# askerlee/segtran

Measured on NVIDIA H100. Metric: voxels/sec fwd+bwd Segtran3d BraTS 112^3 bs=4 hot path, higher is better.
Workload: dtype tf32

## Files before the change

include/segtran_b200.h:

```cpp
#ifndef SEGTRAN_B200_H_
#define SEGTRAN_B200_H_

#include <stddef.h>
#include <stdint.h>

#ifdef __cplusplus
extern "C" {
#endif

#define SX_VERSION 1

enum { SX_F32 = 0, SX_BF16 = 1 };
enum { SX_OP_TF32 = 0, SX_OP_BF16 = 1 };
enum { SX_MAJOR_K = 0, SX_MAJOR_MN = 1 };
enum { SX_BIAS_NONE = 0, SX_BIAS_N = 1, SX_BIAS_M = 2 };
enum { SX_ACT_NONE = 0, SX_ACT_GELU = 1,
       SX_ACT_GELU_BWD = 2  };

int sx_version(void);
const char* sx_last_error(void);
int sx_device_info(int* sm_count, int* cc_major, int* cc_minor);

typedef struct {
  const void* ptr;
  int32_t major;
  int32_t _pad;
  int64_t ld;
  int64_t stride_z0;
  int64_t stride_z1;
} sx_operand;

typedef struct {
  int32_t op_dtype;
  int32_t M, N, K, Z0, Z1;
  sx_operand A, B;
  void* C;
  int32_t c_dtype;
  int32_t round_tf32;
  int64_t ldc, c_stride_z0, c_stride_z1;
  float alpha;
  int32_t bias_mode;
  const float* bias;
  int64_t bias_stride_z0, bias_stride_z1;
  int32_t act;
  int32_t accumulate;
  void* preact;
  int32_t split_k;
  int32_t _pad2;
  float* amax;
  float drop_p;
  uint32_t _pad3;
  uint64_t drop_seed;
  const uint64_t* drop_seed_dev;
  const float* addend;
  float* part;
  int64_t part_floats;
} sx_gemm_args;

typedef struct {
  float* ct;
  int64_t ldct, ct_stride_z0, ct_stride_z1;
} sx_gemm_tout;

int sx_gemm(const sx_gemm_args* args, const sx_gemm_tout* tout, void* stream);

typedef struct {
  const float* table;
  int32_t pd, R;
  int32_t grid[3];
  float w;
} sx_posbias;

typedef struct {
  int32_t B, M, U1, U2, d;
  int32_t round_tf32;
  const float* Q;
  int64_t q_ld, q_bstride;
  const float* K;
  int64_t k_ld, k_bstride;
  float alpha, clip;
  float* P;
  float* S;
  int64_t ldp;
  float* lse;
  float* rowmax;
  float* stat;
  float* diag;
  float drop_p;
  uint32_t _pad;
  uint64_t drop_seed;
  const uint64_t* drop_seed_dev;
  sx_posbias posbias;
} sx_attn_probs_args;
int sx_attn_probs_fwd(const sx_attn_probs_args* args, void* stream);

enum { SX_CONSIST_BCE = 0, SX_CONSIST_MARGIN = 1 };
typedef struct {
  int32_t B, N, A, K;
  int32_t variant;
  int32_t round_r;
  const float* Xo;
  int64_t xo_ld, xo_bstride;
  const float* Xt;
  int64_t xt_ld, xt_bstride;
  const float* X;
  int64_t x_ld, x_bstride;
  const float* F;
  const float* mu;
  float* R;
  int64_t ldr;
  float* out;
  float* cap;
  float cap_scale;
  int32_t _pad;
  float* part;
  int64_t part_floats;
} sx_consist_args;
int sx_attn_consist_fwd(const sx_consist_args* args, void* stream);
int sx_attn_consist_bwd(const sx_consist_args* args, const float* gout, const float* G, int32_t rows, int32_t cols,
                        int64_t ldg, int64_t g_bstride, const float* vrow, const float* vcol, float* dst, int64_t ldd,
                        int64_t d_bstride, void* stream);

int sx_clamp_if(const float* S, int64_t R, int32_t L, int64_t lds, const float* amax, float clip, const float* dY,
                int64_t ldy, float* out, int64_t ldo, void* stream);

int sx_seed_derive(const uint64_t* base, uint64_t add, uint64_t* out, void* stream);
int sx_seed_advance(uint64_t* base, uint64_t inc, void* stream);


int sx_reduce_max(const float* x, int64_t n, float* out, void* stream);

int sx_pos_lsinu_fwd(const float* pos, const float* posmax, int64_t R, int32_t pd, const float* W, const float* b,
                     int32_t C, float* pe, void* stream);
int sx_pos_lsinu_bwd(const float* pos, const float* posmax, int64_t R, int32_t pd, const float* W, const float* b,
                     int32_t C, const float* dpe, float* de_scratch, float* dW, float* db, float* part, int64_t part_floats, void* stream);

int sx_prologue_fwd(const float* x, int64_t B, int32_t N, int32_t C, const float* g, const float* b, const float* pe,
                    int32_t C0, int64_t pe_bstride, float posw, const float* mask, float drop_p, uint64_t seed, const uint64_t* seed_dev, float* h,
                    int32_t round_tf32, float* stats, void* stream);
int sx_prologue_bwd(const float* dh, const float* x, int64_t B, int32_t N, int32_t C, const float* g, const float* b,
                    const float* pe, int32_t C0, int64_t pe_bstride, float posw, const float* mask, float drop_p,
                    uint64_t seed, const uint64_t* seed_dev, const float* stats, float* dx, float* dg, float* db, float* dpe,
                    float* dt_scratch , float* part, int64_t part_floats, void* stream);

int sx_softmax_fwd(const float* S, int64_t R, int32_t L, int64_t lds, const float* amax, float clip, float drop_p,
                   uint64_t seed, const uint64_t* seed_dev, float* P, int64_t ldp, int32_t round_tf32, float* lse, float* diag,
                   void* stream);
int sx_softmax_bwd(const float* dP, int64_t ldd, const float* S, int64_t lds, const float* lse, int64_t R, int32_t L,
                   const float* amax, float clip, float drop_p, uint64_t seed, const uint64_t* seed_dev, int64_t ldp_fwd, float* dS,
                   int64_t ldo, int32_t round_tf32, void* stream);
int sx_softmax_posbias_fwd(const float* S, int64_t R, int32_t L, int64_t lds, const float* amax, float clip, float drop_p,
                           uint64_t seed, const uint64_t* seed_dev, float* P, int64_t ldp, int32_t round_tf32,
                           float* lse, float* diag, const sx_posbias* posbias, void* stream);
int sx_softmax_posbias_bwd(const float* dP, int64_t ldd, const float* S, int64_t lds, const float* lse, int64_t R, int32_t L,
                           const float* amax, float clip, float drop_p, uint64_t seed, const uint64_t* seed_dev, int64_t ldp_fwd,
                           float* dS, int64_t ldo, int32_t round_tf32, const sx_posbias* posbias,
                           float* dtable, float* part, int64_t part_floats, void* stream);

int sx_layernorm_fwd(const float* x, int64_t R, int32_t C, const float* g, const float* b, float* y,
                     int32_t round_tf32, float* stats, void* stream);
int sx_layernorm_bwd(const float* dy, const float* x, int64_t R, int32_t C, const float* g, const float* stats,
                     float* dx, int32_t round_tf32, float* dg, float* db, float* part, int64_t part_floats, void* stream);

int sx_ln_softaggr_fwd(const float* Y, int32_t B, int32_t M, int32_t N, int32_t F, const float* g, const float* b,
                       const float* ws, const float* bs, float drop_p, uint64_t seed, const uint64_t* seed_dev, float* out, float* stats,
                       float* wts, void* stream);
int sx_ln_softaggr_bwd(const float* dout, const float* Y, int32_t B, int32_t M, int32_t N, int32_t F, const float* g,
                       const float* b, const float* ws, float drop_p, uint64_t seed, const uint64_t* seed_dev, const float* stats,
                       const float* wts, float* dY, int32_t round_tf32, float* dg, float* db,
                       float* dws, float* dbs, float* part, int64_t part_floats, void* stream);

int sx_softaggr_fwd(const float* x, int32_t B, int32_t M, int32_t N, int32_t F, const float* ws, const float* bs, float* out,
                    float* wts, void* stream);
int sx_softaggr_bwd(const float* dout, const float* x, int32_t B, int32_t M, int32_t N, int32_t F, const float* ws,
                    const float* wts, float* dx, float* dscore, void* stream);
int sx_gelu_bwd(const float* dG, const float* H, int64_t n, float drop_p, uint64_t seed, const uint64_t* seed_dev, float* dH,
                int32_t round_tf32, void* stream);
int sx_convert(const void* x, int32_t x_dtype, int64_t n, void* y, int32_t y_dtype, int32_t round_tf32, void* stream);
int sx_split_tf32(const float* x, int64_t n, float* hi, float* lo, void* stream);
int sx_split_tf32_cat(const float* x, int32_t Z1, int32_t Z0, int32_t R, int32_t K, int64_t sz1, int64_t sz0, int64_t sr,
                      int64_t sk, int32_t Kp, int32_t role, float* out, void* stream);
int sx_dot(const float* x, const float* y, int64_t n, float* out, float* part, int64_t part_floats, void* stream);
int sx_scale(const float* x, int64_t n, const float* alpha_dev, float alpha, float* y, void* stream);
int sx_colsum_batched(const float* X, int32_t Z1, int64_t stride_z1, int32_t Z0, int64_t stride_z0, int64_t R, int32_t C,
                      int64_t ld, float* out, float* part, int64_t part_floats, void* stream);
int sx_add(const float* a, const float* b, int64_t n, float* y, void* stream);
int sx_rowsum(const float* X, int64_t R, int64_t C, int64_t ld, int32_t out_mod, float* out, float* part, int64_t part_floats, void* stream);
int sx_transpose(const float* in, int64_t Z, int32_t R, int32_t C, int32_t ldo, float* out, void* stream);

int sx_head_contract_fwd(const float* curr, const float* W, const float* bias, int32_t B, int32_t Cf, int64_t V,
                         int32_t K, float* L, int32_t accumulate, void* stream);
int sx_head_contract_bwd_data(const float* dL, const float* W, int32_t B, int32_t Cf, int64_t V, int32_t K,
                              float* dcurr, void* stream);
int sx_head_contract_bwd_weight(const float* dL, const float* curr, int32_t B, int32_t Cf, int64_t V, int32_t K,
                                float* dW, float* part, int64_t part_floats, void* stream);
int sx_token_scores(const float* vf, const float* W, int32_t B, int32_t N, int32_t F, int32_t K, float* out,
                    void* stream);
int sx_token_scores_bwd(const float* dt, const float* W, int32_t B, int32_t N, int32_t F, int32_t K, float* dvf,
                        void* stream);
int sx_subpixel_resize_fwd(const float* S, const float* bias, int32_t B, int32_t K, int32_t D2, int32_t H2, int32_t W2,
                           int32_t H, int32_t W, int32_t D, float* out, void* stream);
int sx_subpixel_resize_bwd(const float* dout, int32_t B, int32_t K, int32_t D2, int32_t H2, int32_t W2, int32_t H,
                           int32_t W, int32_t D, float* dS, void* stream);
enum { SX_HEAD_DMAP_NONE = 0, SX_HEAD_DMAP_INTERP = 1, SX_HEAD_DMAP_UNFOLD = 2, SX_HEAD_DMAP_UNFOLD_INTERLEAVED = 3 };
enum { SX_HEAD_SRC_DEPTH_MAJOR = 0, SX_HEAD_SRC_SLICE_MAJOR = 1 };
typedef struct {
  const float* src;
  int32_t B, Fs, Ds;
  int32_t Fo;
  int64_t HW;
  int32_t Dk;
  int32_t dmap;
  int32_t K;
  int32_t src_layout;
  const float* Wc;
  const float* bc;
  float p;
  uint32_t _pad2;
  uint64_t seed;
  const uint64_t* seed_dev;
  float* part;
  int64_t part_floats;
} sx_head_dropout_args;
int sx_head_dropout_fwd(const sx_head_dropout_args* args, float* Ls, void* stream);
int sx_head_dropout_bwd(const sx_head_dropout_args* args, const float* dLs, float* dsrc, int32_t accumulate, float* dWc,
                        void* stream);
int sx_groupnorm_fwd(const float* x, int32_t B, int32_t C, int64_t V, int32_t G, const float* gamma, const float* beta,
                     float eps, double* csum, float* stats, float* y, int32_t round_tf32, void* stream);
int sx_groupnorm_bwd(const float* dy, const float* x, int32_t B, int32_t C, int64_t V, int32_t G, const float* gamma,
                     const float* stats, double* csum, float* coef, float* dx, float* dgamma, float* dbeta, void* stream);
int sx_groupnorm_slices_fwd(const float* x, int32_t B, int32_t D, int32_t C, int64_t V, int32_t G, const float* gamma,
                            const float* beta, float eps, double* csum, float* stats, float* y, int32_t round_tf32,
                            void* stream);
int sx_groupnorm_slices_bwd(const float* dy, const float* x, int32_t B, int32_t D, int32_t C, int64_t V, int32_t G,
                            const float* gamma, const float* stats, double* csum, float* coef, float* dx, float* dgamma,
                            float* dbeta, void* stream);

int sx_seg_loss_fwd(const float* logits, const float* mask, int32_t B, int32_t K, int64_t V, const float* pos_weight,
                    const float* class_w, float dice_w, double* sums, float* out3, float* coef, void* stream);
int sx_seg_loss_bwd(const float* logits, const float* mask, int32_t B, int32_t K, int64_t V, const float* pos_weight,
                    const float* coef, float ce_scale, const float* gout, float* dlogits, void* stream);
enum { SX_SCHED_WARMUP_LINEAR = 0, SX_SCHED_WARMUP_CONSTANT = 1 };
int sx_adam_step(float* p, float* p_tf32, const float* g, float* m, float* v, const int32_t* seg_param, const int64_t* seg_off,
                 const int32_t* seg_len, int32_t nseg, int32_t P, const float* lr, const float* wd, double b1, double b2,
                 double eps, float grad_clip, float max_grad_norm, float warmup, int64_t t_total, int32_t schedule,
                 int64_t* step, double* sumsq, float* coef, float* lr_eff, float* total_norm, void* stream);

int sx_resize_axis_fwd(const float* x, int64_t outer, int32_t Lin, int32_t Lout, int64_t inner, float* y,
                       int32_t accumulate, void* stream);
int sx_resize_axis_bwd(const float* dy, int64_t outer, int32_t Lin, int32_t Lout, int64_t inner, float* dx,
                       void* stream);
typedef struct {
  int32_t lin[3];
  int32_t lout[3];
  float ratio[3];
} sx_resample_grid;
int sx_resize_tokens_fwd(const float* x, int64_t bs_in, int64_t gs_in, int64_t ld_in, float* y, int64_t bs_out,
                         int64_t gs_out, int64_t ld_out, int32_t B, int32_t G, int32_t w, int32_t w_pad,
                         const sx_resample_grid* grid, int32_t round_tf32, void* stream);
int sx_resize_tokens_bwd(const float* dy, int64_t bs_out, int64_t gs_out, int64_t ld_out, float* dx, int64_t bs_in,
                         int64_t gs_in, int64_t ld_in, int32_t B, int32_t G, int32_t w, int32_t w_pad,
                         const sx_resample_grid* grid, int32_t accumulate, void* stream);
int sx_sgemm_small(const float* A, const float* B, float* C, int32_t M, int32_t N, int32_t K, int64_t sam, int64_t sak,
                   int64_t sbk, int64_t sbn, int64_t scm, int64_t scn, int32_t Z, int64_t saz, int64_t sbz, int64_t scz,
                   float alpha, int32_t accumulate, void* stream);

typedef struct {
  const float* wx;
  const float* wy;
  const float* wz;
  int32_t nx, ny, nz, _pad;
} sx_sw_weights;
int sx_sw_accumulate(const float* scores, int32_t K, int32_t dx, int32_t dy, int32_t dz, float* preds, float* cnt,
                     int32_t H, int32_t W, int32_t D, int32_t x0, int32_t y0, int32_t z0, int32_t mirror,
                     const sx_sw_weights* weights, void* stream);
int sx_sw_finalize(float* preds, const float* cnt, int32_t K, int64_t V, int32_t brats, float* hard, void* stream);
int sx_sw_gather(const float* img, int32_t B, int32_t C, int32_t H, int32_t W, int32_t D, const int32_t* origins, int32_t n,
                 int32_t dx, int32_t dy, int32_t dz, int32_t mirror, float* out, void* stream);

int sx_sw2d_accumulate(const float* scores, int32_t B, int32_t K, int32_t h, int32_t w, int32_t dx, int32_t dy, float* preds,
                       float* cnt, int32_t H2, int32_t W2, int32_t xs, int32_t ys, int32_t mirror,
                       const sx_sw_weights* weights, void* stream);
int sx_sw2d_finalize(const float* preds, const float* cnt, int32_t B, int32_t K, int32_t H2, int32_t W2, int32_t hl,
                     int32_t wl, int32_t H, int32_t W, float* soft, int32_t* hard, void* stream);
int sx_eval2d_counts(const float* pred, int32_t B, int32_t K, int32_t h, int32_t w, const float* gt, int32_t Hg, int32_t Wg,
                     int32_t* counts, void* stream);

int sx_mask_counts(const uint8_t* A, const uint8_t* B, int32_t K, int64_t V, int64_t* counts, int64_t ldc, void* stream);
int sx_surface(const uint8_t* X, int32_t K, int32_t ndim, int32_t n0, int32_t n1, int32_t n2, uint8_t* border, void* stream);
int sx_edt_sq(const uint8_t* border, int32_t K, int32_t n0, int32_t n1, int32_t n2, int32_t* dist, void* stream);
int sx_surface_hist(const uint8_t* src_border, const int32_t* dist, int32_t K, int64_t V, int32_t nbins, uint32_t* hist,
                    int64_t ldh, void* stream);
int sx_surface_stats(const uint32_t* hist, int32_t K, int32_t nbins, int64_t ldh, double* out, int64_t ldo, void* stream);

enum { SX_LABEL_U8 = 0, SX_LABEL_I16 = 1, SX_LABEL_I32 = 2, SX_LABEL_I64 = 3, SX_LABEL_F32 = 4 };
typedef struct {
  const float* x;
  int64_t stride[5];
  float* y;
  int32_t C;
  int32_t _pad;
} sx_crop_operand;
int sx_brats_map_label(const void* label, int32_t dtype, int32_t B, int64_t V, int32_t binarize, float* out, void* stream);
int sx_draw_resized_crop(const uint64_t* seed_dev, uint64_t seed, int32_t H, int32_t W, int32_t D, int32_t oh, int32_t ow,
                         int32_t od, float min_scale, float max_scale, int32_t isotropic, float* rec, void* stream);
int sx_resized_crop(const sx_crop_operand* a, const sx_crop_operand* b, int32_t B, int32_t H, int32_t W, int32_t D,
                    int32_t oh, int32_t ow, int32_t od, const float* rec, void* stream);

int sx_gemm_debug_set(const char* key, int64_t value);

#ifdef __cplusplus
}
#endif
#endif
```

segtran_b200/_lib.py:

```python
from __future__ import annotations

import ctypes as C
import os

_HERE = os.path.dirname(os.path.abspath(__file__))
LIB_PATH = os.path.join(_HERE, "libsegtran_b200.so")

SX_F32, SX_BF16 = 0, 1
SX_OP_TF32, SX_OP_BF16 = 0, 1
SX_MAJOR_K, SX_MAJOR_MN = 0, 1
SX_BIAS_NONE, SX_BIAS_N, SX_BIAS_M = 0, 1, 2
SX_ACT_NONE, SX_ACT_GELU, SX_ACT_GELU_BWD = 0, 1, 2
SX_SCHED_WARMUP_LINEAR, SX_SCHED_WARMUP_CONSTANT = 0, 1
SX_CONSIST_BCE, SX_CONSIST_MARGIN = 0, 1
SX_HEAD_DMAP_NONE, SX_HEAD_DMAP_INTERP, SX_HEAD_DMAP_UNFOLD, SX_HEAD_DMAP_UNFOLD_INTERLEAVED = 0, 1, 2, 3
SX_HEAD_SRC_DEPTH_MAJOR, SX_HEAD_SRC_SLICE_MAJOR = 0, 1
SX_LABEL_U8, SX_LABEL_I16, SX_LABEL_I32, SX_LABEL_I64, SX_LABEL_F32 = 0, 1, 2, 3, 4


class SxError(RuntimeError):
    pass


class sx_operand(C.Structure):
    _fields_ = [("ptr", C.c_void_p), ("major", C.c_int32), ("_pad", C.c_int32), ("ld", C.c_int64),
                ("stride_z0", C.c_int64), ("stride_z1", C.c_int64)]


class sx_gemm_args(C.Structure):
    _fields_ = [("op_dtype", C.c_int32), ("M", C.c_int32), ("N", C.c_int32), ("K", C.c_int32), ("Z0", C.c_int32),
                ("Z1", C.c_int32), ("A", sx_operand), ("B", sx_operand), ("C", C.c_void_p), ("c_dtype", C.c_int32),
                ("round_tf32", C.c_int32), ("ldc", C.c_int64), ("c_stride_z0", C.c_int64), ("c_stride_z1", C.c_int64),
                ("alpha", C.c_float), ("bias_mode", C.c_int32), ("bias", C.c_void_p), ("bias_stride_z0", C.c_int64),
                ("bias_stride_z1", C.c_int64), ("act", C.c_int32), ("accumulate", C.c_int32), ("preact", C.c_void_p),
                ("split_k", C.c_int32), ("_pad2", C.c_int32), ("amax", C.c_void_p), ("drop_p", C.c_float),
                ("_pad3", C.c_uint32), ("drop_seed", C.c_uint64), ("drop_seed_dev", C.c_void_p), ("addend", C.c_void_p),
                ("part", C.c_void_p), ("part_floats", C.c_int64)]


class sx_gemm_tout(C.Structure):
    _fields_ = [("ct", C.c_void_p), ("ldct", C.c_int64), ("ct_stride_z0", C.c_int64), ("ct_stride_z1", C.c_int64)]


class sx_sw_weights(C.Structure):
    _fields_ = [("wx", C.c_void_p), ("wy", C.c_void_p), ("wz", C.c_void_p), ("nx", C.c_int32), ("ny", C.c_int32),
                ("nz", C.c_int32), ("_pad", C.c_int32)]


class sx_posbias(C.Structure):
    _fields_ = [("table", C.c_void_p), ("pd", C.c_int32), ("R", C.c_int32), ("grid", C.c_int32 * 3), ("w", C.c_float)]


class sx_attn_probs_args(C.Structure):
    _fields_ = [("B", C.c_int32), ("M", C.c_int32), ("U1", C.c_int32), ("U2", C.c_int32), ("d", C.c_int32),
                ("round_tf32", C.c_int32), ("Q", C.c_void_p), ("q_ld", C.c_int64), ("q_bstride", C.c_int64),
                ("K", C.c_void_p), ("k_ld", C.c_int64), ("k_bstride", C.c_int64), ("alpha", C.c_float),
                ("clip", C.c_float), ("P", C.c_void_p), ("S", C.c_void_p), ("ldp", C.c_int64), ("lse", C.c_void_p),
                ("rowmax", C.c_void_p), ("stat", C.c_void_p), ("diag", C.c_void_p), ("drop_p", C.c_float),
                ("_pad", C.c_uint32), ("drop_seed", C.c_uint64), ("drop_seed_dev", C.c_void_p), ("posbias", sx_posbias)]


class sx_consist_args(C.Structure):
    _fields_ = [("B", C.c_int32), ("N", C.c_int32), ("A", C.c_int32), ("K", C.c_int32), ("variant", C.c_int32),
                ("round_r", C.c_int32), ("Xo", C.c_void_p), ("xo_ld", C.c_int64), ("xo_bstride", C.c_int64),
                ("Xt", C.c_void_p), ("xt_ld", C.c_int64), ("xt_bstride", C.c_int64), ("X", C.c_void_p),
                ("x_ld", C.c_int64), ("x_bstride", C.c_int64), ("F", C.c_void_p), ("mu", C.c_void_p), ("R", C.c_void_p),
                ("ldr", C.c_int64), ("out", C.c_void_p), ("cap", C.c_void_p), ("cap_scale", C.c_float),
                ("_pad", C.c_int32), ("part", C.c_void_p), ("part_floats", C.c_int64)]


class sx_head_dropout_args(C.Structure):
    _fields_ = [("src", C.c_void_p), ("B", C.c_int32), ("Fs", C.c_int32), ("Ds", C.c_int32), ("Fo", C.c_int32),
                ("HW", C.c_int64), ("Dk", C.c_int32), ("dmap", C.c_int32), ("K", C.c_int32), ("src_layout", C.c_int32),
                ("Wc", C.c_void_p), ("bc", C.c_void_p), ("p", C.c_float), ("_pad2", C.c_uint32), ("seed", C.c_uint64),
                ("seed_dev", C.c_void_p), ("part", C.c_void_p), ("part_floats", C.c_int64)]


class sx_resample_grid(C.Structure):
    _fields_ = [("lin", C.c_int32 * 3), ("lout", C.c_int32 * 3), ("ratio", C.c_float * 3)]


class sx_crop_operand(C.Structure):
    _fields_ = [("x", C.c_void_p), ("stride", C.c_int64 * 5), ("y", C.c_void_p), ("C", C.c_int32), ("_pad", C.c_int32)]


_P, _I, _L, _F, _U64, _D = C.c_void_p, C.c_int32, C.c_int64, C.c_float, C.c_uint64, C.c_double

_PROTOS = {
    "sx_gemm": [C.POINTER(sx_gemm_args), C.POINTER(sx_gemm_tout), _P],
    "sx_gemm_debug_set": [C.c_char_p, _L],
    "sx_attn_probs_fwd": [C.POINTER(sx_attn_probs_args), _P],
    "sx_attn_consist_fwd": [C.POINTER(sx_consist_args), _P],
    "sx_attn_consist_bwd": [C.POINTER(sx_consist_args), _P, _P, _I, _I, _L, _L, _P, _P, _P, _L, _L, _P],
    "sx_clamp_if": [_P, _L, _I, _L, _P, _F, _P, _L, _P, _L, _P],
    "sx_reduce_max": [_P, _L, _P, _P],
    "sx_pos_lsinu_fwd": [_P, _P, _L, _I, _P, _P, _I, _P, _P],
    "sx_pos_lsinu_bwd": [_P, _P, _L, _I, _P, _P, _I, _P, _P, _P, _P, _P, _L, _P],
    "sx_prologue_fwd": [_P, _L, _I, _I, _P, _P, _P, _I, _L, _F, _P, _F, _U64, _P, _P, _I, _P, _P],
    "sx_prologue_bwd": [_P, _P, _L, _I, _I, _P, _P, _P, _I, _L, _F, _P, _F, _U64, _P, _P, _P, _P, _P, _P, _P, _P, _L, _P],
    "sx_softmax_fwd": [_P, _L, _I, _L, _P, _F, _F, _U64, _P, _P, _L, _I, _P, _P, _P],
    "sx_softmax_bwd": [_P, _L, _P, _L, _P, _L, _I, _P, _F, _F, _U64, _P, _L, _P, _L, _I, _P],
    "sx_softmax_posbias_fwd": [_P, _L, _I, _L, _P, _F, _F, _U64, _P, _P, _L, _I, _P, _P, C.POINTER(sx_posbias), _P],
    "sx_softmax_posbias_bwd": [_P, _L, _P, _L, _P, _L, _I, _P, _F, _F, _U64, _P, _L, _P, _L, _I, C.POINTER(sx_posbias),
                               _P, _P, _L, _P],
    "sx_layernorm_fwd": [_P, _L, _I, _P, _P, _P, _I, _P, _P],
    "sx_layernorm_bwd": [_P, _P, _L, _I, _P, _P, _P, _I, _P, _P, _P, _L, _P],
    "sx_ln_softaggr_fwd": [_P, _I, _I, _I, _I, _P, _P, _P, _P, _F, _U64, _P, _P, _P, _P, _P],
    "sx_ln_softaggr_bwd": [_P, _P, _I, _I, _I, _I, _P, _P, _P, _F, _U64, _P, _P, _P, _P, _I, _P, _P, _P, _P, _P, _L, _P],
    "sx_softaggr_fwd": [_P, _I, _I, _I, _I, _P, _P, _P, _P, _P],
    "sx_softaggr_bwd": [_P, _P, _I, _I, _I, _I, _P, _P, _P, _P, _P],
    "sx_gelu_bwd": [_P, _P, _L, _F, _U64, _P, _P, _I, _P],
    "sx_seed_derive": [_P, _U64, _P, _P],
    "sx_seed_advance": [_P, _U64, _P],
    "sx_convert": [_P, _I, _L, _P, _I, _I, _P],
    "sx_sw_accumulate": [_P, _I, _I, _I, _I, _P, _P, _I, _I, _I, _I, _I, _I, _I, C.POINTER(sx_sw_weights), _P],
    "sx_sw_finalize": [_P, _P, _I, _L, _I, _P, _P],
    "sx_sw_gather": [_P, _I, _I, _I, _I, _I, _P, _I, _I, _I, _I, _I, _P, _P],
    "sx_sw2d_accumulate": [_P, _I, _I, _I, _I, _I, _I, _P, _P, _I, _I, _I, _I, _I, C.POINTER(sx_sw_weights), _P],
    "sx_sw2d_finalize": [_P, _P, _I, _I, _I, _I, _I, _I, _I, _I, _P, _P, _P],
    "sx_eval2d_counts": [_P, _I, _I, _I, _I, _P, _I, _I, _P, _P],
    "sx_mask_counts": [_P, _P, _I, _L, _P, _L, _P],
    "sx_surface": [_P, _I, _I, _I, _I, _I, _P, _P],
    "sx_edt_sq": [_P, _I, _I, _I, _I, _P, _P],
    "sx_surface_hist": [_P, _P, _I, _L, _I, _P, _L, _P],
    "sx_surface_stats": [_P, _I, _I, _L, _P, _L, _P],
    "sx_brats_map_label": [_P, _I, _I, _L, _I, _P, _P],
    "sx_draw_resized_crop": [_P, _U64, _I, _I, _I, _I, _I, _I, _F, _F, _I, _P, _P],
    "sx_resized_crop": [C.POINTER(sx_crop_operand), C.POINTER(sx_crop_operand), _I, _I, _I, _I, _I, _I, _I, _P, _P],
    "sx_split_tf32": [_P, _L, _P, _P, _P],
    "sx_split_tf32_cat": [_P, _I, _I, _I, _I, _L, _L, _L, _L, _I, _I, _P, _P],
    "sx_transpose": [_P, _L, _I, _I, _I, _P, _P],
    "sx_colsum_batched": [_P, _I, _L, _I, _L, _L, _I, _L, _P, _P, _L, _P],
    "sx_dot": [_P, _P, _L, _P, _P, _L, _P],
    "sx_add": [_P, _P, _L, _P, _P],
    "sx_rowsum": [_P, _L, _L, _L, _I, _P, _P, _L, _P],
    "sx_scale": [_P, _L, _P, _F, _P, _P],
    "sx_head_contract_fwd": [_P, _P, _P, _I, _I, _L, _I, _P, _I, _P],
    "sx_head_contract_bwd_data": [_P, _P, _I, _I, _L, _I, _P, _P],
    "sx_head_contract_bwd_weight": [_P, _P, _I, _I, _L, _I, _P, _P, _L, _P],
    "sx_head_dropout_fwd": [C.POINTER(sx_head_dropout_args), _P, _P],
    "sx_head_dropout_bwd": [C.POINTER(sx_head_dropout_args), _P, _P, _I, _P, _P],
    "sx_token_scores": [_P, _P, _I, _I, _I, _I, _P, _P],
    "sx_token_scores_bwd": [_P, _P, _I, _I, _I, _I, _P, _P],
    "sx_subpixel_resize_fwd": [_P, _P, _I, _I, _I, _I, _I, _I, _I, _I, _P, _P],
    "sx_subpixel_resize_bwd": [_P, _I, _I, _I, _I, _I, _I, _I, _I, _P, _P],
    "sx_resize_axis_fwd": [_P, _L, _I, _I, _L, _P, _I, _P],
    "sx_resize_axis_bwd": [_P, _L, _I, _I, _L, _P, _P],
    "sx_resize_tokens_fwd": [_P, _L, _L, _L, _P, _L, _L, _L, _I, _I, _I, _I, C.POINTER(sx_resample_grid), _I, _P],
    "sx_resize_tokens_bwd": [_P, _L, _L, _L, _P, _L, _L, _L, _I, _I, _I, _I, C.POINTER(sx_resample_grid), _I, _P],
    "sx_groupnorm_fwd": [_P, _I, _I, _L, _I, _P, _P, _F, _P, _P, _P, _I, _P],
    "sx_groupnorm_bwd": [_P, _P, _I, _I, _L, _I, _P, _P, _P, _P, _P, _P, _P, _P],
    "sx_groupnorm_slices_fwd": [_P, _I, _I, _I, _L, _I, _P, _P, _F, _P, _P, _P, _I, _P],
    "sx_groupnorm_slices_bwd": [_P, _P, _I, _I, _I, _L, _I, _P, _P, _P, _P, _P, _P, _P, _P],
    "sx_seg_loss_fwd": [_P, _P, _I, _I, _L, _P, _P, _F, _P, _P, _P, _P],
    "sx_seg_loss_bwd": [_P, _P, _I, _I, _L, _P, _P, _F, _P, _P, _P],
    "sx_adam_step": [_P, _P, _P, _P, _P, _P, _P, _P, _I, _I, _P, _P, _D, _D, _D, _F, _F, _F, _L, _I, _P, _P, _P, _P, _P, _P],
    "sx_sgemm_small": [_P, _P, _P, _I, _I, _I, _L, _L, _L, _L, _L, _L, _I, _L, _L, _L, _F, _I, _P],
}
EXPORTS = sorted(list(_PROTOS) + ["sx_version", "sx_last_error", "sx_device_info"])

_lib = None


def lib():
    global _lib
    if _lib is None:
        if not os.path.isfile(LIB_PATH):
            raise SxError("segtran_b200: %s is missing - run `python -c 'import __graft_entry__ as g; g.build()'` "
                          "or `make` at the repo root (there is no CPU / PyTorch fallback)" % LIB_PATH)
        l = C.CDLL(LIB_PATH)
        l.sx_version.restype = C.c_int
        l.sx_last_error.restype = C.c_char_p
        l.sx_device_info.argtypes = [C.POINTER(C.c_int)] * 3
        l.sx_device_info.restype = C.c_int
        for name, at in _PROTOS.items():
            f = getattr(l, name)
            f.argtypes = at
            f.restype = C.c_int
        _lib = l
    return _lib


def check(rc, what):
    if rc != 0:
        raise SxError("%s failed (rc=%d): %s" % (what, rc, lib().sx_last_error().decode("utf-8", "replace")))


_LAUNCHES = {"sx_pos_lsinu_bwd": 3, "sx_ln_softaggr_bwd": 2, "sx_prologue_bwd": 3, "sx_layernorm_bwd": 3, "sx_gemm_debug_set": 0,
             "sx_attn_probs_fwd": 2, "sx_colsum_batched": 2, "sx_dot": 2, "sx_head_contract_bwd_weight": 2,
             "sx_softmax_posbias_bwd": 2, "sx_attn_consist_fwd": 2, "sx_head_dropout_bwd": 2, "sx_edt_sq": 3}
launch_count = 0
_hook = None


def set_hook(h):
    global _hook
    _hook = h


def call(name, *args):
    global launch_count
    launch_count += _LAUNCHES.get(name, 1)
    if _hook is None:
        check(getattr(lib(), name)(*args), name)
    else:
        with _hook(name, args):
            check(getattr(lib(), name)(*args), name)
```

segtran_b200/csrc/sx_attn.cu:

```cuda
#include "sx_common.cuh"
#include "sx_posbias.cuh"
#include "sx_tc.cuh"

namespace {
using namespace sxtc;

constexpr int NUM_THREADS = 384;
constexpr int STAGES = 4;
constexpr int STAGE_BYTES = A_STAGE_BYTES + B_STAGE_BYTES;
constexpr int SMEM_BYTES = STAGES * STAGE_BYTES + 1024  + 256;
constexpr float LOG2E = 1.4426950408889634f, LN2 = 0.6931471805599453f;

__device__ __forceinline__ unsigned int ordered_key(float v) {
  const unsigned int b = __float_as_uint(v);
  return (b & 0x80000000u) ? ~b : (b | 0x80000000u);
}
__device__ __forceinline__ float ordered_val(unsigned int k) {
  return k == 0u ? -3.0e38f : __uint_as_float((k & 0x80000000u) ? (k & 0x7FFFFFFFu) : ~k);
}

struct AttnParams {
  int B, M, U1, U2, d;
  int tiles_m, tiles_n, num_kb, items, nsub;
  int q_bcast;
  float alpha2, clip2;
  float alpha, clip;
  float* P;
  float* S;
  float* lse;
  float* rowmax;
  float* stat;
  long long ldp;
  float drop_p;
  unsigned long long drop_seed;
  const unsigned long long* drop_seed_dev;
  int round_tf32;
  const float* pb_table;
  sxpb::Geom pb;
};

constexpr int PB_OFFSET = STAGES * STAGE_BYTES + 256;
constexpr int PB_MAX_FLOATS = 29 * 29 * 29;

template <bool HAS_BIAS>
__global__ void __launch_bounds__(NUM_THREADS, 1)
sx_attn_probs_kernel(const __grid_constant__ CUtensorMap tmQ, const __grid_constant__ CUtensorMap tmK, const AttnParams p) {
  extern __shared__ uint8_t smem_raw[];
  uint8_t* smem = reinterpret_cast<uint8_t*>((reinterpret_cast<uintptr_t>(smem_raw) + 1023) & ~uintptr_t(1023));
  uint64_t* bars = reinterpret_cast<uint64_t*>(smem + STAGES * STAGE_BYTES);
  uint64_t* full_bar = bars;
  uint64_t* empty_bar = bars + STAGES;

  const int warp = threadIdx.x >> 5;
  const int lane = threadIdx.x & 31;
  const int wg = threadIdx.x >> 7;

  if (threadIdx.x == 0) {
    sx::tma_prefetch_desc(&tmQ);
    sx::tma_prefetch_desc(&tmK);
    for (int s = 0; s < STAGES; ++s) {
      sx::mbar_init(&full_bar[s], 1);
      sx::mbar_init(&empty_bar[s], 2);
    }
    sx::fence_barrier_init();
  }
  float* ptab = nullptr;
  float* pred = nullptr;
  if constexpr (HAS_BIAS) {
    ptab = reinterpret_cast<float*>(smem + PB_OFFSET);
    pred = reinterpret_cast<float*>(smem + STAGES * STAGE_BYTES + 128);
    float bmn = 0.f, bmx = 0.f;
    for (int i = threadIdx.x; i < p.pb.T; i += NUM_THREADS) {
      const float v = p.pb.w * p.pb_table[i];
      ptab[i] = v * LOG2E;
      bmn = fminf(bmn, v);
      bmx = fmaxf(bmx, v);
    }
    bmx = sx::warp_max(bmx);
    bmn = -sx::warp_max(-bmn);
    if ((threadIdx.x & 31) == 0) { pred[2 * (threadIdx.x >> 5)] = bmn; pred[2 * (threadIdx.x >> 5) + 1] = bmx; }
  }
  __syncthreads();

  auto decode = [&](int it, int& b, int& m, int& mb) {
    mb = it % p.tiles_m; it /= p.tiles_m;
    m = it % p.M;
    b = it / p.M;
  };

  if (wg == 0) {
    asm volatile("setmaxnreg.dec.sync.aligned.u32 40;" ::: "memory");
    if (warp == 0 && sx::elect_one()) {
      int stage = 0;
      uint32_t phase = 0;
      for (int it = blockIdx.x; it < p.items; it += gridDim.x) {
        int b, m, mb;
        decode(it, b, m, mb);
        const int qb = p.q_bcast ? 0 : b;
        for (int sub = 0; sub < p.nsub; ++sub) {
          const int nb = sub % p.tiles_n;
          for (int kb = 0; kb < p.num_kb; ++kb) {
            sx::mbar_wait(&empty_bar[stage], phase ^ 1);
            sx::mbar_expect_tx(&full_bar[stage], STAGE_BYTES);
            uint8_t* sa = smem + stage * STAGE_BYTES;
            sx::tma_load_4d(sa, &tmQ, &full_bar[stage], kb * 32, mb * BM, m, qb, sx::kEvictLast);
            sx::tma_load_4d(sa + A_STAGE_BYTES, &tmK, &full_bar[stage], kb * 32, nb * BN, m, b, sx::kEvictLast);
            if (++stage == STAGES) { stage = 0; phase ^= 1; }
          }
        }
      }
    }
    return;
  }

  asm volatile("setmaxnreg.inc.sync.aligned.u32 232;" ::: "memory");
  const int cw = wg - 1;
  const int wtid = threadIdx.x & 127;
  const int wq = warp & 3;
  const int tr = lane >> 2;
  const int tc = (lane & 3) * 2;
  int stage = 0;
  uint32_t phase = 0;
  float gmax = -3.0e38f;
  int lowrows = 0;
  const uint32_t p16 = sx::drop_p16(p.drop_p);
  const float keep_scale = p.drop_p > 0.f ? 1.f / (1.f - p.drop_p) : 1.f;
  const unsigned long long dseed = p.drop_seed + (p.drop_seed_dev ? *p.drop_seed_dev : 0ull);
  const uint32_t dmul = sx::drop_mul((tc >> 1) & 1), dkey = sx::drop_key(dseed, (tc >> 1) & 1);
  float acc[64];
  float brange = 0.f;
  if constexpr (HAS_BIAS) {
    float bmn = 0.f, bmx = 0.f;
    for (int w = 0; w < NUM_THREADS / 32; ++w) { bmn = fminf(bmn, pred[2 * w]); bmx = fmaxf(bmx, pred[2 * w + 1]); }
    brange = bmx - bmn;
  }

  for (int it = blockIdx.x; it < p.items; it += gridDim.x) {
    int b, m, mb;
    decode(it, b, m, mb);
    int grow[2];
    long long rowflat[2];
    float rm[2], rl[2], rraw[2], rcp[2];
#pragma unroll
    for (int h = 0; h < 2; ++h) {
      grow[h] = mb * BM + cw * 64 + wq * 16 + 8 * h + tr;
      rowflat[h] = ((long long)b * p.M + m) * p.U1 + grow[h];
      rm[h] = -3.0e38f; rl[h] = 0.f; rraw[h] = -3.0e38f; rcp[h] = 0.f;
    }

    auto chunk_stats = [&](int nb) {
      if constexpr (HAS_BIAS) {
        int qc[2][3], kc[3];
        sxpb::coords(p.pb, grow[0], qc[0]);
        sxpb::coords(p.pb, grow[1], qc[1]);
        sxpb::coords(p.pb, nb * BN + tc, kc);
        float cm[2] = {-3.0e38f, -3.0e38f}, mb[2] = {-3.0e38f, -3.0e38f}, s[2] = {0.f, 0.f};
#pragma unroll
        for (int j = 0; j < 16; ++j)
#pragma unroll
          for (int e = 0; e < 2; ++e) {
            if (nb * BN + 8 * j + tc + e < p.U2) {
#pragma unroll
              for (int h = 0; h < 2; ++h) {
                const int o = sxpb::offset(p.pb, qc[h], kc);
                const float v = acc[4 * j + 2 * h + e];
                cm[h] = fmaxf(cm[h], v);
                const float x = fminf(v * p.alpha2, p.clip2) + (o >= 0 ? ptab[o] : 0.f);
                const float mn = fmaxf(mb[h], x);
                s[h] = s[h] * sx::ex2_approx(mb[h] - mn) + sx::ex2_approx(x - mn);
                mb[h] = mn;
              }
            }
            sxpb::step(p.pb, kc, e ? 7 : 1);
          }
#pragma unroll
        for (int h = 0; h < 2; ++h) {
#pragma unroll
          for (int o = 1; o <= 2; o <<= 1) {
            cm[h] = fmaxf(cm[h], __shfl_xor_sync(0xffffffffu, cm[h], o));
            const float mo = __shfl_xor_sync(0xffffffffu, mb[h], o), so = __shfl_xor_sync(0xffffffffu, s[h], o);
            const float mn = fmaxf(mb[h], mo);
            s[h] = s[h] * sx::ex2_approx(mb[h] - mn) + so * sx::ex2_approx(mo - mn);
            mb[h] = mn;
          }
          rraw[h] = fmaxf(rraw[h], cm[h] * p.alpha2);
          const float mn = fmaxf(rm[h], mb[h]);
          rl[h] = rl[h] * sx::ex2_approx(rm[h] - mn) + s[h] * sx::ex2_approx(mb[h] - mn);
          rm[h] = mn;
        }
      } else {
#pragma unroll
        for (int h = 0; h < 2; ++h) {
          float cm = -3.0e38f;
#pragma unroll
          for (int j = 0; j < 16; ++j)
#pragma unroll
            for (int e = 0; e < 2; ++e)
              if (nb * BN + 8 * j + tc + e < p.U2) cm = fmaxf(cm, acc[4 * j + 2 * h + e]);
          cm = fmaxf(cm, __shfl_xor_sync(0xffffffffu, cm, 1));
          cm = fmaxf(cm, __shfl_xor_sync(0xffffffffu, cm, 2));
          cm *= p.alpha2;
          rraw[h] = fmaxf(rraw[h], cm);
          const float mn = fmaxf(rm[h], fminf(cm, p.clip2));
          float s = 0.f;
#pragma unroll
          for (int j = 0; j < 16; ++j)
#pragma unroll
            for (int e = 0; e < 2; ++e)
              if (nb * BN + 8 * j + tc + e < p.U2) s += sx::ex2_approx(fminf(acc[4 * j + 2 * h + e] * p.alpha2, p.clip2) - mn);
          s += __shfl_xor_sync(0xffffffffu, s, 1);
          s += __shfl_xor_sync(0xffffffffu, s, 2);
          rl[h] = rl[h] * sx::ex2_approx(rm[h] - mn) + s;
          rm[h] = mn;
        }
      }
    };
    auto publish = [&]() {
#pragma unroll
      for (int h = 0; h < 2; ++h) {
        rcp[h] = 1.f / rl[h];
        if (grow[h] < p.U1) {
          gmax = fmaxf(gmax, rraw[h]);
          if ((lane & 3) == 0) {
            p.lse[rowflat[h]] = (rm[h] + __log2f(rl[h])) * LN2;
            if (p.rowmax) p.rowmax[rowflat[h]] = rraw[h] * LN2;
            if constexpr (HAS_BIAS) {
              if (rraw[h] * LN2 < -(p.clip - 104.f) + brange) ++lowrows;
            } else {
              if (rraw[h] * LN2 < -(p.clip - 104.f)) ++lowrows;
            }
          }
        }
      }
    };
    auto chunk_probs = [&](int nb) {
#pragma unroll
      for (int h = 0; h < 2; ++h) {
        if (grow[h] >= p.U1) continue;
        const long long roff = rowflat[h] * p.ldp;
        int qc[3], kc[3];
        if constexpr (HAS_BIAS) {
          sxpb::coords(p.pb, grow[h], qc);
          sxpb::coords(p.pb, nb * BN + tc, kc);
        }
#pragma unroll
        for (int j = 0; j < 16; ++j) {
          float b0 = 0.f, b1 = 0.f;
          if constexpr (HAS_BIAS) {
            int o = sxpb::offset(p.pb, qc, kc);
            if (o >= 0) b0 = ptab[o];
            sxpb::step(p.pb, kc, 1);
            o = sxpb::offset(p.pb, qc, kc);
            if (o >= 0) b1 = ptab[o];
            sxpb::step(p.pb, kc, 7);
          }
          const int col = nb * BN + 8 * j + tc;
          if (col >= p.U2) continue;
          const float v0 = acc[4 * j + 2 * h], v1 = acc[4 * j + 2 * h + 1];
          if (p.S) {
            if (col + 1 < p.U2) *reinterpret_cast<float2*>(p.S + roff + col) = make_float2(v0 * p.alpha, v1 * p.alpha);
            else p.S[roff + col] = v0 * p.alpha;
          }
          float f0, f1;
          if constexpr (HAS_BIAS) {
            f0 = sx::ex2_approx(fminf(v0 * p.alpha2, p.clip2) + b0 - rm[h]) * rcp[h];
            f1 = sx::ex2_approx(fminf(v1 * p.alpha2, p.clip2) + b1 - rm[h]) * rcp[h];
          } else {
            f0 = sx::ex2_approx(fminf(v0 * p.alpha2, p.clip2) - rm[h]) * rcp[h];
            f1 = sx::ex2_approx(fminf(v1 * p.alpha2, p.clip2) - rm[h]) * rcp[h];
          }
          if (p.drop_p > 0.f) {
            const uint32_t w = sx::drop_word_k(dmul, dkey, (unsigned long long)((roff + col) >> 2));
            f0 = (w & 0xFFFFu) >= p16 ? f0 * keep_scale : 0.f;
            f1 = (w >> 16) >= p16 ? f1 * keep_scale : 0.f;
          }
          if (p.round_tf32) {
            f0 = sx::round_tf32(f0);
            f1 = sx::round_tf32(f1);
          }
          if (col + 1 < p.U2) *reinterpret_cast<float2*>(p.P + roff + col) = make_float2(f0, f1);
          else p.P[roff + col] = f0;
        }
      }
    };

    for (int sub = 0; sub < p.nsub; ++sub) {
      const int nb = sub % p.tiles_n;
      for (int kb = 0; kb < p.num_kb; ++kb) {
        sx::mbar_wait(&full_bar[stage], phase);
        const uint32_t sa = sx::smem_u32(smem + stage * STAGE_BYTES);
        const uint32_t qa = sa + (uint32_t)(cw * 64 * BKB), ka = sa + A_STAGE_BYTES;
        sx::acc_fence(acc);
        sx::wgmma_fence();
#pragma unroll
        for (int kk = 0; kk < 4; ++kk)
          sx::wgmma_tf32(acc, sx::gmma_desc(qa + kk * 32, 16, 1024), sx::gmma_desc(ka + kk * 32, 16, 1024),
                         (kb > 0 || kk > 0) ? 1u : 0u);
        sx::wgmma_commit();
        sx::wgmma_wait<0>();
        sx::acc_fence(acc);
        if (wtid == 0) sx::mbar_arrive(&empty_bar[stage]);
        if (++stage == STAGES) { stage = 0; phase ^= 1; }
      }
      if (p.nsub == 1) {
        chunk_stats(nb);
        publish();
        chunk_probs(nb);
      } else if (sub < p.tiles_n) {
        chunk_stats(nb);
        if (sub == p.tiles_n - 1) publish();
      } else {
        chunk_probs(nb);
      }
    }
  }
  gmax = sx::warp_max(gmax);
  if (lane == 0 && gmax > -3.0e38f) atomicMax(reinterpret_cast<unsigned int*>(&p.stat[0]), ordered_key(gmax * LN2));
  int lr = lowrows;
#pragma unroll
  for (int o = 16; o > 0; o >>= 1) lr += __shfl_xor_sync(0xffffffffu, lr, o);
  if (lane == 0 && lr > 0) atomicAdd(&p.stat[1], (float)lr);
}

__global__ void attn_diag_kernel(float* stat, float clip, float* diag) {
  const float mx = ordered_val(__float_as_uint(stat[0]));
  stat[2] = mx;
  if (diag) {
    diag[0] = fmaxf(diag[0], mx);
    if (mx > clip) {
      diag[1] += 1.f;
      diag[2] += stat[1];
    }
  }
}

}

extern "C" int sx_attn_probs_fwd(const sx_attn_probs_args* a, void* stream) {
  SX_REQUIRE(a != nullptr, "sx_attn_probs_fwd: null args");
  SX_REQUIRE(a->B > 0 && a->M > 0 && a->U1 > 0 && a->U2 > 0 && a->d > 0, "sx_attn_probs_fwd: bad shape");
  SX_REQUIRE(a->Q && a->K && a->P && a->lse && a->stat, "sx_attn_probs_fwd: null pointer");
  SX_REQUIRE(a->d % 4 == 0 && a->ldp % 4 == 0 && a->ldp >= a->U2, "sx_attn_probs_fwd: d and ldp must be multiples of 4");
  SX_REQUIRE((reinterpret_cast<uintptr_t>(a->P) & 15) == 0 && (!a->S || (reinterpret_cast<uintptr_t>(a->S) & 15) == 0),
             "sx_attn_probs_fwd: outputs must be 16-byte aligned");
  const int sms = sm_count_cached();
  SX_REQUIRE(sms > 0, "sx_attn_probs_fwd: no CUDA device (this library has no CPU fallback)");

  AttnParams p{};
  p.B = a->B; p.M = a->M; p.U1 = a->U1; p.U2 = a->U2; p.d = a->d;
  p.tiles_m = sx_ceil_div(a->U1, BM);
  p.tiles_n = sx_ceil_div(a->U2, BN);
  p.num_kb = sx_ceil_div(a->d, 32);
  p.nsub = p.tiles_n == 1 ? 1 : 2 * p.tiles_n;
  const long long items = (long long)a->B * a->M * p.tiles_m;
  SX_REQUIRE(items < (1ll << 30), "sx_attn_probs_fwd: too many row blocks");
  p.items = (int)items;
  p.q_bcast = a->q_bstride == 0 && a->B > 1;
  p.alpha = a->alpha; p.clip = a->clip;
  p.alpha2 = a->alpha * LOG2E; p.clip2 = a->clip * LOG2E;
  p.P = reinterpret_cast<float*>(a->P); p.S = reinterpret_cast<float*>(a->S);
  p.lse = a->lse; p.rowmax = a->rowmax; p.stat = a->stat;
  p.ldp = a->ldp;
  p.drop_p = a->drop_p; p.drop_seed = a->drop_seed;
  p.drop_seed_dev = reinterpret_cast<const unsigned long long*>(a->drop_seed_dev);
  p.round_tf32 = a->round_tf32;
  const bool has_bias = a->posbias.table != nullptr;
  if (has_bias) {
    SX_REQUIRE(a->U1 == a->U2, "sx_attn_probs_fwd: positional biases need self-attention (U1 == U2)");
    const char* err = sxpb::check(&a->posbias, a->U1);
    SX_REQUIRE(err == nullptr, "sx_attn_probs_fwd: %s", err);
    p.pb_table = a->posbias.table;
    p.pb = sxpb::make_geom(a->posbias);
    SX_REQUIRE(p.pb.T <= PB_MAX_FLOATS, "sx_attn_probs_fwd: positional-bias table too large");
  }

  sx_operand oq{}, ok{};
  oq.ptr = a->Q; oq.major = SX_MAJOR_K; oq.ld = a->q_ld; oq.stride_z0 = a->d; oq.stride_z1 = p.q_bcast ? 0 : a->q_bstride;
  ok.ptr = a->K; ok.major = SX_MAJOR_K; ok.ld = a->k_ld; ok.stride_z0 = a->d; ok.stride_z1 = a->k_bstride;
  if (a->M == 1) { oq.stride_z0 = 0; ok.stride_z0 = 0; }
  if (a->B == 1) { oq.stride_z1 = 0; ok.stride_z1 = 0; }
  CUtensorMap tq, tk;
  int rc = make_map(&tq, oq, 4, a->U1, a->d, a->M, a->B, BM, "Q");
  if (rc) return rc;
  rc = make_map(&tk, ok, 4, a->U2, a->d, a->M, a->B, BN, "K");
  if (rc) return rc;

  const int grid = p.items < sms ? p.items : sms;
  cudaStream_t st = reinterpret_cast<cudaStream_t>(stream);
  if (has_bias) {
    constexpr int smem_pb = PB_OFFSET + PB_MAX_FLOATS * 4 + 1024;
    SX_CHECK_CUDA(set_max_smem_once(sx_attn_probs_kernel<true>, smem_pb));
    sx_attn_probs_kernel<true><<<grid, NUM_THREADS, PB_OFFSET + p.pb.T * 4 + 1024, st>>>(tq, tk, p);
  } else {
    SX_CHECK_CUDA(set_max_smem_once(sx_attn_probs_kernel<false>, SMEM_BYTES));
    sx_attn_probs_kernel<false><<<grid, NUM_THREADS, SMEM_BYTES, st>>>(tq, tk, p);
  }
  SX_CHECK_CUDA(cudaGetLastError());
  attn_diag_kernel<<<1, 1, 0, st>>>(a->stat, a->clip, a->diag);
  SX_CHECK_CUDA(cudaGetLastError());
  return 0;
}
```

segtran_b200/networks/segtran_shared.py:

```python
from __future__ import annotations

import copy
import math

import numpy as np
import torch
import torch.nn as nn
import torch.nn.functional as F

from .. import ops

bb2feat_dims = {
    'resnet34': [64, 64, 128, 256, 512], 'resnet50': [64, 256, 512, 1024, 2048],
    'resnet101': [64, 256, 512, 1024, 2048], 'resibn101': [64, 256, 512, 1024, 2048],
    'eff-b0': [16, 24, 40, 112, 1280], 'eff-b1': [16, 24, 40, 112, 1280], 'eff-b2': [16, 24, 48, 120, 1408],
    'eff-b3': [24, 32, 48, 136, 1536], 'eff-b4': [24, 32, 56, 160, 1792], 'effv2m': [24, 48, 80, 176, 512],
    'i3d': [64, 192, 480, 832, 1024],
}


def gen_all_indices(shape, device):
    axes = [torch.arange(int(s), device=device) for s in shape]
    return torch.stack(torch.meshgrid(*axes, indexing='ij'), dim=len(axes))


def multi_resize_shape(shape, scales):
    return [torch.Size([int(g / scale) for g in shape]) for scale in scales]


def mince_grids(shape, scales):
    grid = tuple(int(g) for g in shape)
    if len(grid) not in (2, 3):
        raise ValueError("mince transformer: a 2-D or 3-D token grid is needed (got %s)" % (grid,))
    out = []
    for scale, shp in zip(scales, multi_resize_shape(grid, scales)):
        for g, n in zip(grid, shp):
            if n < 1:
                raise ValueError("mince transformer: scale %s leaves an empty axis of the grid %s" % (scale, grid))
            if n != math.floor(g * (1.0 / scale)):
                raise ValueError("mince transformer: scale %s gives int(%d / %s) = %d cells but F.interpolate makes %d"
                                 % (scale, g, scale, n, math.floor(g * (1.0 / scale))))
        out.append(tuple(int(n) for n in shp))
    return out


def fracs_to_indices(feat_dim, mince_channel_props):
    fracs = np.array(mince_channel_props, dtype=float)
    fracs /= fracs.sum()
    n = len(fracs)
    idx = [0] * (n + 1)
    for i in range(n - 1):
        idx[i + 1] = idx[i] + int(fracs[i] * feat_dim)
    idx[-1] = feat_dim
    return idx, [idx[i + 1] - idx[i] for i in range(n)]


def _check_mince_config(config):
    if config.mince_scales is None or config.mince_channel_props is None:
        raise ValueError("mince transformer: mince_scales and mince_channel_props must be given")
    if len(config.mince_channel_props) != len(config.mince_scales):
        raise ValueError("mince transformer: %d scales but %d channel proportions"
                         % (len(config.mince_scales), len(config.mince_channel_props)))




class SegtranConfig:

    def __init__(self):
        self.feat_dim = -1
        self.in_feat_dim = -1
        self.num_modes = 4
        self.use_squeezed_transformer = True
        self.num_attractors = 256
        self.tie_qk_scheme = 'shared'
        self.mid_type = 'shared'
        self.trans_output_type = 'private'
        self.act_fun = F.gelu
        self.has_FFN = True
        self.has_FFN_in_squeeze = False
        self.pos_code_type = 'lsinu'
        self.pos_code_weight = 1.
        self.pos_bias_radius = 7
        self.qk_have_bias = True
        self.v_has_bias = False
        self.attn_clip = 500
        self.base_initializer_range = 0.02
        self.query_idbias_scale = 10
        self.feattrans_lin1_idbias_scale = 10
        self.pool_modes_feat = 'softmax'
        self.use_mince_transformer = False
        self.mince_scales = None
        self.mince_channel_props = None
        self.hidden_dropout_prob = 0.1
        self.attention_probs_dropout_prob = 0.1
        self.out_fpn_do_dropout = False
        self.eval_robustness = False
        self.ablate_multihead = False
        self.use_attn_consist_loss = False

    def try_assign(self, args, *keys):
        hit = False
        for key in keys:
            if key in args:
                self.__dict__[key] = args[key] if isinstance(args, dict) else args.__dict__[key]
                hit = True
        return hit

    def set_fpn_layers(self, config_name, fpn_settings, do_print=True):
        self.in_fpn_layers = [int(c) for c in fpn_settings.in_fpn_layers]
        self.out_fpn_layers = [int(c) for c in fpn_settings.out_fpn_layers]
        if self.out_fpn_layers[-1] > self.in_fpn_layers[-1]:
            print("in_fpn_layers=%s is not compatible with out_fpn_layers=%s" % (self.in_fpn_layers, self.out_fpn_layers))
            exit(0)
        ratios = fpn_settings.translayer_compress_ratios
        assert len(ratios) == self.num_translayers + 1, \
            "Length of {} != 1 + num_translayers {}".format(ratios, self.num_translayers)
        self.orig_in_feat_dim = self.bb_feat_dims[self.in_fpn_layers[-1]]
        self.translayer_compress_ratios = ratios
        self.translayer_dims = [int(self.orig_in_feat_dim / r) for r in np.cumprod(ratios)]
        self.trans_in_dim = self.translayer_dims[0]
        self.min_feat_dim = np.min(self.translayer_dims)
        self.trans_out_dim = self.translayer_dims[-1]
        self.in_fpn_scheme = fpn_settings.in_fpn_scheme
        self.out_fpn_scheme = fpn_settings.out_fpn_scheme
        if do_print:
            print("'%s' orig in-feat: %d, in-feat: %d, out-feat: %d, in-scheme: %s, out-scheme: %s, translayer_dims: %s"
                  % (config_name, self.orig_in_feat_dim, self.trans_in_dim, self.trans_out_dim, self.in_fpn_scheme,
                     self.out_fpn_scheme, self.translayer_dims))


def _prod(shape):
    n = 1
    for g in shape:
        n *= int(g)
    return n


def _unsupported(what):
    raise NotImplementedError("segtran_b200: %s is an ablation path this build does not implement "
                              "(use the reference module for it)" % what)


class MMSharedMid(nn.Module):

    def __init__(self, config):
        super().__init__()
        self.num_modes, self.feat_dim = config.num_modes, config.feat_dim
        self.shared_linear = nn.Linear(self.feat_dim, self.feat_dim)
        self.mid_act_fn = config.act_fun
        self.dropout = nn.Dropout(config.hidden_dropout_prob)

    def forward(self, x):
        p = self.dropout.p if self.training else 0.0
        return ops.linear(x, self.shared_linear.weight, self.shared_linear.bias, gelu=True, drop_p=p,
                          seed=ops.new_dropout_seed(x.device) if p > 0 else 0)


class MMPrivateMid(nn.Module):
    def __init__(self, config):
        super().__init__()
        _unsupported("mid_type='private'")


class MMPrivateOutput(nn.Module):

    def __init__(self, config):
        super().__init__()
        self.num_modes, self.feat_dim = config.num_modes, config.feat_dim
        fam = self.feat_dim * self.num_modes
        self.group_linear = nn.Conv1d(fam, fam, 1, groups=self.num_modes)
        self.resout_norm_layer = nn.LayerNorm(self.feat_dim, eps=1e-12, elementwise_affine=True)
        self.dropout = nn.Dropout(config.hidden_dropout_prob)

    def forward(self, x, shortcut=None):
        return ops.group_linear(x, self.group_linear.weight, self.group_linear.bias)


class MMSharedOutput(nn.Module):

    def __init__(self, config):
        super().__init__()
        self.num_modes, self.feat_dim = config.num_modes, config.feat_dim
        self.shared_linear = nn.Linear(self.feat_dim, self.feat_dim)
        self.resout_norm_layer = nn.LayerNorm(self.feat_dim, eps=1e-12, elementwise_affine=True)
        self.dropout = nn.Dropout(config.hidden_dropout_prob)

    def forward(self, x, shortcut):
        return ops.add(ops.linear(x, self.shared_linear.weight, self.shared_linear.bias), shortcut)


class LearnedSoftAggregate(nn.Module):

    def __init__(self, num_feat, group_dim, keepdim=False):
        super().__init__()
        self.group_dim = group_dim
        self.feat2score = nn.Linear(num_feat, 1)
        self.keepdim = keepdim

    def forward(self, x, score_basis=None):
        if score_basis is not None or self.group_dim != 1 or x.dim() != 4:
            _unsupported("LearnedSoftAggregate with a separate score basis / group_dim != 1")
        y = ops.soft_aggregate(x, self.feat2score.weight, self.feat2score.bias)
        return y.unsqueeze(1) if self.keepdim else y


class ExpandedFeatTrans(nn.Module):

    def __init__(self, config, name):
        super().__init__()
        self.config, self.name = config, name
        self.in_feat_dim, self.feat_dim, self.num_modes = config.in_feat_dim, config.feat_dim, config.num_modes
        self.feat_dim_allmode = self.feat_dim * self.num_modes
        self.has_FFN = config.has_FFN and not config.eval_robustness
        self.has_input_skip = getattr(config, 'has_input_skip', False)
        if self.has_input_skip:
            _unsupported("has_input_skip")
        if config.use_mince_transformer and config.mince_scales is not None:
            _check_mince_config(config)
            self.mince_scales = list(config.mince_scales)
            self.num_scales = len(self.mince_scales)
            self.mince_channel_props = config.mince_channel_props
            self.mince_channel_indices, _ = fracs_to_indices(self.feat_dim, self.mince_channel_props)
        else:
            self.num_scales = 0
            self.mince_scales = None
        self.first_linear = nn.Linear(self.in_feat_dim, self.feat_dim_allmode, bias=config.v_has_bias)
        self.first_norm_layer = nn.LayerNorm(self.feat_dim, eps=1e-12, elementwise_affine=True)
        self.base_initializer_range = config.base_initializer_range
        self.pool_modes_keepdim = False
        self.pool_modes_feat = config.pool_modes_feat
        if self.pool_modes_feat != 'softmax':
            _unsupported("pool_modes_feat=%r" % self.pool_modes_feat)
        self.feat_softaggr = LearnedSoftAggregate(self.feat_dim, group_dim=1, keepdim=False)
        self.mid_type = config.mid_type
        if self.mid_type == 'shared':
            self.intermediate = MMSharedMid(config)
        elif self.mid_type == 'private':
            self.intermediate = MMPrivateMid(config)
        else:
            _unsupported("mid_type=%r" % self.mid_type)
        if config.trans_output_type == 'shared':
            self.output = MMSharedOutput(config)
        elif config.trans_output_type == 'private':
            self.output = MMPrivateOutput(config)

    def add_identity_bias(self):
        s = self.config.feattrans_lin1_idbias_scale
        if s > 0:
            Fd = self.feat_dim
            eye = torch.eye(Fd) * self.base_initializer_range * s
            w = self.first_linear.weight.data
            w[:Fd, :Fd] = w[:Fd, :Fd] * 0.5 + eye.to(w)

    def _can_fold(self):
        return self.has_FFN and isinstance(self.output, MMPrivateOutput) and isinstance(self.intermediate, MMSharedMid) \
            and self.first_linear.bias is None and self.first_linear.weight.shape[1] % 4 == 0 and self.feat_dim % 4 == 0

    def supports_fused_attention(self):
        return self.has_FFN and isinstance(self.output, MMPrivateOutput) and isinstance(self.intermediate, MMSharedMid)

    def _value_bank(self, input_feat, tag="big"):
        M, mid = self.num_modes, self.intermediate
        B, U2 = input_feat.shape[0], input_feat.shape[1]
        if self._can_fold():
            return ops.folded_value_bank(input_feat, self.first_linear.weight, mid.shared_linear.weight, M, tag)
        v = ops.linear(input_feat, self.first_linear.weight, self.first_linear.bias, tag=tag)
        return ops.linear(v.view(B, U2, M, self.feat_dim), mid.shared_linear.weight, tag=tag).view(B, U2, M * self.feat_dim)

    def _norm_aggregate(self, y):
        p = self.output.dropout.p if self.training else 0.0
        ln = self.output.resout_norm_layer
        f2s = self.feat_softaggr.feat2score
        return ops.ln_softaggr(y, ln.weight, ln.bias, f2s.weight, f2s.bias, drop_p=p,
                               seed=ops.new_dropout_seed(y.device) if p > 0 else 0)

    def _mince_fuse(self, input_feat, probs, grid):
        M, Fd = self.num_modes, self.feat_dim
        grids = mince_grids(grid, self.mince_scales)
        if len(probs) != self.num_scales:
            raise ValueError("ExpandedFeatTrans: %d attention probabilities for %d mince scales" % (len(probs), self.num_scales))
        idx = self.mince_channel_indices
        wins = [(idx[s], idx[s + 1]) for s in range(self.num_scales)]
        if any(b <= a for a, b in wins):
            raise ValueError("ExpandedFeatTrans: an empty mince channel window %s of %d channels" % (wins, Fd))
        v = ops.linear(input_feat, self.first_linear.weight, self.first_linear.bias, round_out=False)
        ratios = [(ops.down_ratio(sc),) * len(grid) for sc in self.mince_scales]
        vs = ops.resize_tokens(v, M, grid, grids, ratios, wins)
        us = [ops.attn_pv(p, vv, M, round_out=False) for p, vv in zip(probs, vs)]
        return ops.resize_tokens_into(us, grid, grids, wins, Fd)

    def forward(self, input_feat, attention_probs, in_geoshape=None):
        M = self.num_modes
        if self.num_scales > 0:
            if in_geoshape is None:
                raise ValueError("ExpandedFeatTrans: the mince transformer needs the token grid (in_geoshape)")
            u = self._mince_fuse(input_feat, attention_probs, tuple(int(g) for g in in_geoshape))
            if not self.has_FFN:
                z = u[:, 0] if M == 1 else self.feat_softaggr(u)
                return ops.layer_norm(z, self.first_norm_layer.weight, self.first_norm_layer.bias)
            g = self.intermediate(u)
            return self._norm_aggregate(self.output(g, u))
        folded = self.supports_fused_attention()
        if not folded:
            v = ops.linear(input_feat, self.first_linear.weight, self.first_linear.bias)
        if not self.has_FFN:
            u = ops.attn_pv(attention_probs, v, M)
            z = u[:, 0] if M == 1 else self.feat_softaggr(u)
            return ops.layer_norm(z, self.first_norm_layer.weight, self.first_norm_layer.bias)
        if folded:
            mid = self.intermediate
            vp = self._value_bank(input_feat, ops.small_tag(input_feat.shape[1], attention_probs.shape[2]))
            p = mid.dropout.p if self.training else 0.0
            gl = self.output.group_linear
            y = ops.attn_pv_gelu_group_linear(attention_probs, vp, M, mid.shared_linear.bias, p,
                                              ops.new_dropout_seed(vp.device) if p > 0 else 0, gl.weight, gl.bias)
        else:
            u = ops.attn_pv(attention_probs, v, M)
            g = self.intermediate(u)
            y = self.output(g, u)
        return self._norm_aggregate(y)


class AblationMMSharedMid(nn.Module):

    def __init__(self, config):
        super().__init__()
        self.num_modes, self.feat_dim = config.num_modes, config.feat_dim
        self.shared_linear = nn.Linear(self.feat_dim, self.feat_dim)
        self.mid_act_fn = config.act_fun


class AblationMMPrivateOutput(nn.Module):

    def __init__(self, config):
        super().__init__()
        self.num_modes, self.feat_dim = config.num_modes, config.feat_dim
        fam = self.feat_dim * self.num_modes
        self.group_linear = nn.Conv1d(fam, fam, 1, groups=self.num_modes)
        self.resout_norm_layer = nn.LayerNorm(self.feat_dim, eps=1e-12, elementwise_affine=True)
        self.dropout = nn.Dropout(config.hidden_dropout_prob)


class AblationMMSharedOutput(nn.Module):

    def __init__(self, config):
        super().__init__()
        self.num_modes, self.feat_dim = config.num_modes, config.feat_dim
        self.shared_linear = nn.Linear(self.feat_dim, self.feat_dim)
        self.resout_norm_layer = nn.LayerNorm(self.feat_dim, eps=1e-12, elementwise_affine=True)
        self.dropout = nn.Dropout(config.hidden_dropout_prob)


class MultiHeadFeatTrans(nn.Module):

    def __init__(self, config, name):
        super().__init__()
        self.config, self.name = config, name
        self.in_feat_dim, self.feat_dim, self.num_modes = config.in_feat_dim, config.feat_dim, config.num_modes
        if self.feat_dim % self.num_modes:
            raise ValueError("MultiHeadFeatTrans: feat_dim %d is not divisible by %d heads" % (self.feat_dim, self.num_modes))
        if config.mid_type != 'shared':
            _unsupported("mid_type=%r with ablate_multihead" % (config.mid_type,))
        if config.trans_output_type not in ('private', 'shared'):
            _unsupported("trans_output_type=%r" % (config.trans_output_type,))
        self.feat_dim_onehead = self.feat_dim // self.num_modes
        self.feat_dim_allhead = self.feat_dim_onehead * self.num_modes
        self.first_linear = nn.Linear(self.in_feat_dim, self.feat_dim_allhead)
        config.num_modes = 1
        self.mid_type = config.mid_type
        self.intermediate = AblationMMSharedMid(config)
        if config.trans_output_type == 'shared':
            self.output = AblationMMSharedOutput(config)
        else:
            self.output = AblationMMPrivateOutput(config)

    def supports_fused_attention(self):
        return True

    def forward(self, input_feat, attention_probs):
        v = ops.linear(input_feat, self.first_linear.weight, self.first_linear.bias, tag="proj")
        u = ops.attn_pv(attention_probs, v, self.num_modes, heads=True)
        mid = self.intermediate.shared_linear
        g = ops.linear(u, mid.weight, mid.bias, gelu=True, tag="proj")
        out = self.output
        p = out.dropout.p if self.training else 0.0
        seed = ops.new_dropout_seed(u.device) if p > 0 else 0
        if isinstance(out, AblationMMSharedOutput):
            z = ops.linear(g, out.shared_linear.weight, out.shared_linear.bias, drop_p=p, seed=seed, tag="proj",
                           round_out=False, addend=u)
        else:
            z = ops.linear(g, out.group_linear.weight, out.group_linear.bias, drop_p=p, seed=seed, tag="proj",
                           round_out=False)
        ln = out.resout_norm_layer
        return ops.layer_norm(z, ln.weight, ln.bias, round_out=False)


def _new_diag(device):
    return torch.tensor([-3.0e38, 0.0, 0.0], device=device)


def _attention_probs(q, k, M, clip, drop_p, diag, *, fused, posbias=None, alpha=None, row_bias=None, tag="big",
                     kmajor_dq=False):
    seed = ops.new_dropout_seed(q.device) if drop_p > 0 else 0
    if fused:
        return ops.attn_probs(q, k, M, alpha, clip, drop_p, seed, diag, posbias, kmajor_dq=kmajor_dq), None, None
    amax = torch.full((1,), -3.0e38, device=q.device)
    S = ops.attn_scores(q, k, M, amax, row_bias, tag, alpha)
    return ops.softmax(S, amax, clip, drop_p, seed, diag, posbias), S, amax


class CrossAttFeatTrans(nn.Module):

    def __init__(self, config, name):
        super().__init__()
        self.config, self.name = config, name
        self.num_modes, self.in_feat_dim, self.feat_dim = config.num_modes, config.in_feat_dim, config.feat_dim
        self.attention_mode_dim = self.in_feat_dim // self.num_modes
        self.att_size_allmode = self.num_modes * self.attention_mode_dim
        self.query = nn.Linear(self.in_feat_dim, self.att_size_allmode, bias=config.qk_have_bias)
        self.key = nn.Linear(self.in_feat_dim, self.att_size_allmode, bias=config.qk_have_bias)
        self.base_initializer_range = config.base_initializer_range
        if config.pos_code_type == 'bias':
            if config.use_attn_consist_loss:
                raise NotImplementedError("segtran_b200: --attnconsist with --pos bias is not implemented (the attention "
                                          "scores this build keeps do not include the positional biases)")
            self.pos_code_weight = config.pos_code_weight
        else:
            self.pos_code_weight = 1
        if config.ablate_multihead:
            self.out_trans = MultiHeadFeatTrans(config, name)
        else:
            self.out_trans = ExpandedFeatTrans(config, name)
        self.att_dropout = nn.Dropout(config.attention_probs_dropout_prob)
        self.keep_attn_scores = config.use_attn_consist_loss
        self.tie_qk_scheme = config.tie_qk_scheme
        self.attn_clip = config.attn_clip
        self.attn_diag_cycles = config.__dict__.get('attn_diag_cycles', 500)
        self.call_count = 0
        self.attention_scores = None
        self._diag = None

    def tie_qk(self, tie_qk_scheme=None):
        if tie_qk_scheme is not None:
            self.tie_qk_scheme = tie_qk_scheme
        if self.tie_qk_scheme == 'shared':
            self.key.weight = self.query.weight
            if self.key.bias is not None:
                self.key.bias = self.query.bias
        elif self.tie_qk_scheme == 'loose':
            self.key.weight.data.copy_(self.query.weight)
            if self.key.bias is not None:
                self.key.bias.data.copy_(self.query.bias)

    def add_identity_bias(self):
        d = self.attention_mode_dim
        eye = torch.eye(d) * self.base_initializer_range * self.config.query_idbias_scale
        eye = eye.repeat(1, self.in_feat_dim // d)
        w = self.key.weight.data
        w[:d] = w[:d] * 0.5 + eye.to(w)

    def _diag_values(self):
        if self._diag is None:
            return 0.0, 0
        m, c = self._diag.tolist()[:2]
        return (m if m > -1e38 else 0.0), int(c)

    @property
    def lower_clamp_ambiguous_rows(self):
        return 0 if self._diag is None else int(self._diag.tolist()[2])

    @property
    def max_attn(self):
        return max(self._diag_values()[0], 0)

    @property
    def clamp_count(self):
        return self._diag_values()[1]

    def forward(self, in_query, in_key=None, pos_biases=None):
        if in_key is None:
            in_key = in_query
        pb = None
        if pos_biases is not None:
            if not isinstance(pos_biases, ops.PosBias):
                raise TypeError("CrossAttFeatTrans: pos_biases must be an ops.PosBias (SlidingPosBiases2D/3D output)")
            if self.keep_attn_scores:
                raise NotImplementedError("segtran_b200: --attnconsist with --pos bias is not implemented")
            if in_query.shape[1] != pos_biases.num_tokens or in_key.shape[1] != pos_biases.num_tokens:
                raise ValueError("CrossAttFeatTrans: positional biases over %s cells need a self-attention over as many "
                                 "tokens (got %d queries, %d keys)" % (pos_biases.grid, in_query.shape[1], in_key.shape[1]))
            pb = pos_biases.with_weight(float(self.pos_code_weight))
        M = self.num_modes
        nq, nk = in_query.shape[1], in_key.shape[1]
        tq = ops.small_tag(nq, nk) if nq < nk else "proj"
        tk = ops.small_tag(nk, nq) if nk < nq else "proj"
        q = ops.linear(in_query, self.query.weight, self.query.bias, tag=tq)
        k = ops.linear(in_key, self.key.weight, self.key.bias, tag=tk)
        dev = q.device
        if self._diag is None or self._diag.device != dev:
            self._diag = _new_diag(dev)
        p = self.att_dropout.p if self.training else 0.0
        diag_call = self.training and (self.call_count + 1) % self.attn_diag_cycles == 0
        fused = ops.attn_fusion_enabled() and not self.keep_attn_scores and not diag_call and q.is_cuda and \
            self.attention_mode_dim % 4 == 0 and self.out_trans.supports_fused_attention()
        probs, s, amax = _attention_probs(q, k, M, float(self.attn_clip), p, self._diag, fused=fused, posbias=pb,
                                          kmajor_dq=isinstance(self.out_trans, ExpandedFeatTrans))
        self.attention_scores = ops.clamp_if(s, amax, float(self.attn_clip)) if self.keep_attn_scores else None
        if self.training:
            self.call_count += 1
            if self.call_count % self.attn_diag_cycles == 0:
                with torch.no_grad():
                    avg = float(s.sum() / (s > 0).sum().clamp_min(1))
                mx, cc = self._diag_values()
                print("max-attn: {:.2f}, avg-attn: {:.2f}, clamp-count: {}".format(mx, avg, cc))
                self._diag = _new_diag(dev)
        return self.out_trans(in_key, probs)


class CrossMinceAttFeatTrans(nn.Module):

    def __init__(self, config, name):
        super().__init__()
        self.config, self.name = config, name
        self.num_modes, self.in_feat_dim, self.feat_dim = config.num_modes, config.in_feat_dim, config.feat_dim
        self.attention_mode_dim = self.in_feat_dim // self.num_modes
        self.att_size_allmode = self.num_modes * self.attention_mode_dim
        self.query = nn.Linear(self.in_feat_dim, self.att_size_allmode, bias=config.qk_have_bias)
        self.key = nn.Linear(self.in_feat_dim, self.att_size_allmode, bias=config.qk_have_bias)
        if not config.use_mince_transformer:
            raise ValueError("CrossMinceAttFeatTrans needs use_mince_transformer")
        _check_mince_config(config)
        self.mince_scales = list(config.mince_scales)
        self.num_scales = len(self.mince_scales)
        self.mince_qk_channel_indices, _ = fracs_to_indices(self.attention_mode_dim, [1] * self.num_scales)
        if any(self.mince_qk_channel_indices[s + 1] <= self.mince_qk_channel_indices[s] for s in range(self.num_scales)):
            raise ValueError("CrossMinceAttFeatTrans: %d channels per mode cannot be split between %d scales"
                             % (self.attention_mode_dim, self.num_scales))
        self.base_initializer_range = config.base_initializer_range
        self.pos_code_weight = config.pos_code_weight if config.pos_code_type == 'bias' else 1
        if config.ablate_multihead:
            _unsupported("ablate_multihead")
        if config.use_attn_consist_loss:
            raise NotImplementedError("segtran_b200: --attnconsist with --mince is not implemented (the reference "
                                      "crashes on the per-scale list of attention scores)")
        self.out_trans = ExpandedFeatTrans(config, name)
        self.att_dropout = nn.Dropout(config.attention_probs_dropout_prob)
        self.keep_attn_scores = False
        self.tie_qk_scheme = config.tie_qk_scheme
        self.attn_clip = config.attn_clip
        self.attn_diag_cycles = config.__dict__.get('attn_diag_cycles', 500)
        self.call_count = 0
        self.attention_scores = None
        self._diag = None

    tie_qk = CrossAttFeatTrans.tie_qk
    add_identity_bias = CrossAttFeatTrans.add_identity_bias

    def _diag_lists(self):
        if self._diag is None:
            return [0.0] * self.num_scales, [0] * self.num_scales, [0] * self.num_scales
        vals = [d.tolist() for d in self._diag]
        return [max(v[0], 0.0) for v in vals], [int(v[1]) for v in vals], [int(v[2]) for v in vals]

    @property
    def max_attn(self):
        return self._diag_lists()[0]

    @property
    def clamp_count(self):
        return self._diag_lists()[1]

    @property
    def lower_clamp_ambiguous_rows(self):
        return sum(self._diag_lists()[2])

    def forward(self, in_query, query_geoshape, in_key=None, key_geoshape=None, pos_biases=None):
        if in_key is None:
            in_key, key_geoshape = in_query, query_geoshape
        grid = tuple(int(g) for g in query_geoshape)
        if key_geoshape is None or tuple(int(g) for g in key_geoshape) != grid:
            raise ValueError("CrossMinceAttFeatTrans: query and key grids must agree (got %s and %s)"
                             % (grid, None if key_geoshape is None else tuple(key_geoshape)))
        grids = mince_grids(grid, self.mince_scales)
        N = _prod(grid)
        if in_query.shape[1] != N or in_key.shape[1] != N:
            raise ValueError("CrossMinceAttFeatTrans: %d / %d tokens on a grid of %d cells"
                             % (in_query.shape[1], in_key.shape[1], N))
        pbs = [None] * self.num_scales
        if pos_biases is not None:
            if len(pos_biases) != self.num_scales:
                raise ValueError("CrossMinceAttFeatTrans: %d positional biases for %d scales"
                                 % (len(pos_biases), self.num_scales))
            for s, pb in enumerate(pos_biases):
                if pb is None:
                    continue
                if not isinstance(pb, ops.PosBias):
                    raise TypeError("CrossMinceAttFeatTrans: pos_biases entries must be ops.PosBias or None")
                if pb.grid != grids[s]:
                    raise ValueError("CrossMinceAttFeatTrans: positional biases over %s at scale %s, whose grid is %s"
                                     % (pb.grid, self.mince_scales[s], grids[s]))
                pbs[s] = pb.with_weight(float(self.pos_code_weight))
        M, d = self.num_modes, self.attention_mode_dim
        q = ops.linear(in_query, self.query.weight, self.query.bias, tag="proj", round_out=False)
        k = ops.linear(in_key, self.key.weight, self.key.bias, tag="proj", round_out=False)
        idx = self.mince_qk_channel_indices
        wins = [(idx[s], idx[s + 1]) for s in range(self.num_scales)]
        ratios = [(ops.down_ratio(sc),) * len(grid) for sc in self.mince_scales]
        qs = ops.resize_tokens(q, M, grid, grids, ratios, wins)
        ks = ops.resize_tokens(k, M, grid, grids, ratios, wins)
        dev = q.device
        if self._diag is None or self._diag[0].device != dev:
            self._diag = [_new_diag(dev) for _ in range(self.num_scales)]
        p = self.att_dropout.p if self.training else 0.0
        alpha = 1.0 / math.sqrt(d)
        self.call_count += 1
        diag_call = self.training and self.call_count % self.attn_diag_cycles == 0
        fused = ops.attn_fusion_enabled() and not diag_call and q.is_cuda
        probs = []
        for s in range(self.num_scales):
            P, sc, _ = _attention_probs(qs[s], ks[s], M, float(self.attn_clip), p, self._diag[s], fused=fused,
                                        posbias=pbs[s], alpha=alpha)
            probs.append(P)
            if diag_call:
                with torch.no_grad():
                    avg = float(sc.sum() / (sc > 0).sum().clamp_min(1))
                mx, cc, _ = self._diag_lists()
                print("{} attn max: {:.2f}, avg: {:.2f}, clamp-count: {}".format(self.mince_scales[s], mx[s], avg, cc[s]))
                self._diag[s] = _new_diag(dev)
        return self.out_trans(in_key, probs, grid)


class SqueezedAttFeatTrans(nn.Module):

    def __init__(self, config, name):
        super().__init__()
        self.config, self.name = config, name
        self.in_feat_dim, self.num_attractors = config.in_feat_dim, config.num_attractors
        if config.use_mince_transformer:
            _unsupported("the mince transformer")
        if config.ablate_multihead:
            raise NotImplementedError("segtran_b200: ablate_multihead with squeezed attention is not implemented (the "
                                      "reference crashes there: MultiHeadFeatTrans reshapes the attractor-side output "
                                      "with the token count, segtran_ablation.py:239; its drivers turn --multihead into "
                                      "--nosqueeze)")
        config1 = copy.copy(config)
        config1.feat_dim = config1.in_feat_dim
        config1.num_modes = 1
        config1.has_FFN = config.has_FFN_in_squeeze
        self.in_ator_trans = CrossAttFeatTrans(config1, name + '-in-squeeze')
        self.ator_out_trans = CrossAttFeatTrans(config, name + '-squeeze-out')
        self.attractors = nn.Parameter(torch.randn(1, self.num_attractors, self.in_feat_dim))
        self.attention_scores = None

    def _in_squeeze_reassociated(self, in_feat):
        t = self.in_ator_trans
        C = self.in_feat_dim
        st = ops.small_tag(self.num_attractors, in_feat.shape[1])
        x3 = ops.rt_for(st) == 0
        q1 = ops.linear(self.attractors, t.query.weight, t.query.bias, tag=st, round_out=not x3)
        qw = ops.linear(q1, t.key.weight.t(), tag=st)
        rb = None
        if t.key.bias is not None:
            rb = ops.scale(ops.matvec(q1[0], t.key.bias), 1.0 / math.sqrt(C))
        dev = in_feat.device
        if t._diag is None or t._diag.device != dev:
            t._diag = _new_diag(dev)
        p = t.att_dropout.p if t.training else 0.0
        probs, s, amax = _attention_probs(qw, in_feat, 1, float(t.attn_clip), p, t._diag, fused=False, row_bias=rb,
                                          tag="insq")
        t.attention_scores = ops.clamp_if(s, amax, float(t.attn_clip)) if t.keep_attn_scores else None
        if t.training:
            t.call_count += 1
        u = ops.attn_pv(probs, in_feat, 1, tag="insq", round_out=not x3)
        ot = t.out_trans
        z = ops.linear(u[:, 0], ot.first_linear.weight, tag=st, round_out=False)
        return ops.layer_norm(z, ot.first_norm_layer.weight, ot.first_norm_layer.bias, consumer_tag=st)

    def forward(self, in_feat, pos_biases=None):
        if pos_biases is not None:
            _unsupported("positional biases with squeezed attention")
        t = self.in_ator_trans
        if t.num_modes == 1 and not t.out_trans.has_FFN and t.out_trans.first_linear.bias is None \
                and t.feat_dim == self.in_feat_dim:
            att = self._in_squeeze_reassociated(in_feat)
        else:
            att = t(self.attractors, in_feat)
        ops.grad_ready(att, self.ator_out_trans.parameters())
        out = self.ator_out_trans(in_feat, att)
        self.attention_scores = self.ator_out_trans.attention_scores
        return out


class LearnedSinuPosEmbedder(nn.Module):

    def __init__(self, pos_dim, pos_embed_dim, omega=1, affine=False):
        super().__init__()
        self.pos_dim, self.pos_embed_dim, self.omega = pos_dim, pos_embed_dim, omega
        if omega != 1 or affine:
            _unsupported("LearnedSinuPosEmbedder with omega != 1 or affine")
        self.pos_fc = nn.Linear(pos_dim, pos_embed_dim, bias=True)
        self.pos_mix_norm_layer = nn.LayerNorm(pos_embed_dim, eps=1e-12, elementwise_affine=affine)

    def forward(self, pos_normed):
        shp = pos_normed.shape
        pe = ops.pos_code(pos_normed.reshape(-1, shp[-1]), self.pos_fc.weight, self.pos_fc.bias, normalize=False)
        return pe.view(*shp[:-1], -1)


class NoneEmbedder(nn.Module):

    def forward(self, pos_normed):
        return None


class _SlidingPosBiases(nn.Module):

    _INDEX_BUFFERS = ()

    def __init__(self, pos_dim, pos_bias_radius, max_pos_size):
        super().__init__()
        if pos_dim != self._POS_DIM:
            raise ValueError("%s: pos_dim must be %d" % (type(self).__name__, self._POS_DIM))
        if pos_bias_radius < 1:
            raise ValueError("%s: pos_bias_radius must be >= 1 (got %d)" % (type(self).__name__, pos_bias_radius))
        self.pos_dim = pos_dim
        self.R = pos_bias_radius
        self.max_pos_size = tuple(int(m) for m in max_pos_size)
        self.biases = nn.Parameter(torch.zeros([2 * pos_bias_radius + 1] * pos_dim))

    def forward(self, feat_shape, device=None, table=None):
        grid = tuple(int(s) for s in tuple(feat_shape)[-self.pos_dim:])
        if any(g > m for g, m in zip(grid, self.max_pos_size)):
            raise ValueError("%s: feature grid %s exceeds max_pos_size %s" % (type(self).__name__, grid, self.max_pos_size))
        return ops.PosBias(self.biases if table is None else table, self.R, grid, 1.0)

    def _load_from_state_dict(self, state_dict, prefix, local_metadata, strict, missing_keys, unexpected_keys, error_msgs):
        for name in self._INDEX_BUFFERS:
            state_dict.pop(prefix + name, None)
        super()._load_from_state_dict(state_dict, prefix, local_metadata, strict, missing_keys, unexpected_keys, error_msgs)


class SlidingPosBiases2D(_SlidingPosBiases):
    _POS_DIM = 2
    _INDEX_BUFFERS = ('all_h1s', 'all_w1s', 'all_h2s', 'all_w2s')

    def __init__(self, pos_dim, pos_bias_radius=7, max_pos_size=(100, 100)):
        super().__init__(pos_dim, pos_bias_radius, max_pos_size)


class SlidingPosBiases3D(_SlidingPosBiases):
    _POS_DIM = 3
    _INDEX_BUFFERS = ('all_h1s', 'all_w1s', 'all_d1s', 'all_h2s', 'all_w2s', 'all_d2s')

    def __init__(self, pos_dim, pos_bias_radius=7, max_pos_size=(20, 20, 20)):
        super().__init__(pos_dim, pos_bias_radius, max_pos_size)


class SegtranPosEncoder(nn.Module):

    def __init__(self, config):
        super().__init__()
        self.feat_dim = config.trans_in_dim
        self.pos_embed_dim = self.feat_dim
        self.pos_code_type = config.pos_code_type
        if self.pos_code_type == 'lsinu':
            self.pos_coder = LearnedSinuPosEmbedder(config.pos_dim, self.pos_embed_dim, omega=1, affine=False)
        elif self.pos_code_type == 'none':
            self.pos_coder = NoneEmbedder()
        elif self.pos_code_type == 'bias':
            cls = {2: SlidingPosBiases2D, 3: SlidingPosBiases3D}.get(config.pos_dim)
            if cls is None:
                raise ValueError("SegtranPosEncoder: positional biases need pos_dim 2 or 3 (got %r)" % config.pos_dim)
            self.pos_coder = cls(config.pos_dim, config.pos_bias_radius, config.max_pos_size)
        else:
            _unsupported("pos_code_type=%r" % self.pos_code_type)
        self.cached_pos_code = None
        self.cached_feat_shape = None

    def forward(self, orig_feat_shape, voxels_pos):
        if self.pos_code_type == 'none':
            return None
        if self.pos_code_type == 'bias':
            key = tuple(int(s) for s in orig_feat_shape)
            if self.training or (torch.is_grad_enabled() and self.pos_coder.biases.requires_grad):
                self.cached_pos_code = self.pos_coder(key, table=self.pos_coder.biases.detach().clone())
                self.cached_feat_shape = key
                return self.pos_coder(key)
            if self.cached_pos_code is None or self.cached_feat_shape != key:
                self.cached_pos_code = self.pos_coder(key, table=self.pos_coder.biases.detach().clone())
                self.cached_feat_shape = key
            return self.cached_pos_code
        key = tuple(voxels_pos.shape)
        if not self.training and self.cached_pos_code is not None and self.cached_feat_shape == key and \
                not (torch.is_grad_enabled() and self.cached_pos_code.requires_grad):
            return self.cached_pos_code
        B, N, pd = voxels_pos.shape
        shared = B == 1 or voxels_pos.stride(0) == 0
        pos2d = voxels_pos[0] if shared else voxels_pos.reshape(B * N, pd)
        pe = ops.pos_code(pos2d, self.pos_coder.pos_fc.weight, self.pos_coder.pos_fc.bias)
        if not shared:
            pe = pe.view(B, N, -1)
        self.cached_pos_code, self.cached_feat_shape = pe, key
        return pe


class SegtranFusionEncoder(nn.Module):

    def __init__(self, config, name):
        super().__init__()
        self.name = name
        self.num_translayers = config.num_translayers
        self.pos_code_type = config.pos_code_type
        self.translayer_compress_ratios = config.translayer_compress_ratios
        self.translayer_dims = config.translayer_dims
        self.dropout = nn.Dropout(config.hidden_dropout_prob)
        self.use_squeezed_transformer = config.use_squeezed_transformer
        self.use_mince_transformer = config.use_mince_transformer
        if self.use_squeezed_transformer and self.use_mince_transformer:
            print("Squeezed transformer cannot be used with Mince transformer.")
            print("Please specify '--nosqueeze' to disable squeezed transformer.")
            exit(0)
        if self.use_squeezed_transformer and self.pos_code_type == 'bias':
            print("Squeezed transformer cannot use Positional Biases.")
            print("Please specify '--nosqueeze' to disable squeezed transformer.")
            exit(0)
        if self.pos_code_type == 'bias' and config.use_attn_consist_loss:
            raise NotImplementedError("segtran_b200: --attnconsist with --pos bias is not implemented (the attention "
                                      "scores this build keeps do not include the positional biases)")
        self.pos_code_weight = config.pos_code_weight if self.pos_code_type != 'bias' else 0
        if self.use_mince_transformer:
            _check_mince_config(config)
            if config.use_attn_consist_loss:
                raise NotImplementedError("segtran_b200: --attnconsist with --mince is not implemented (the reference "
                                          "crashes on the per-scale list of attention scores)")
            self.num_scales = len(config.mince_scales)
            self.mince_scales = list(config.mince_scales)
        else:
            self.num_scales = 0
        if self.num_scales > 0 and self.pos_code_type in ('bias', 'none'):
            self.pos_code_layers = nn.ModuleList([SegtranPosEncoder(config) for _ in range(self.num_scales)])
        else:
            self.pos_code_layer = SegtranPosEncoder(config)
        if self.use_squeezed_transformer:
            layer_cls = SqueezedAttFeatTrans
        else:
            layer_cls = CrossMinceAttFeatTrans if self.use_mince_transformer else CrossAttFeatTrans
        layers = []
        for i in range(self.num_translayers):
            cfg_i = copy.copy(config)
            cfg_i.in_feat_dim = self.translayer_dims[i]
            cfg_i.feat_dim = self.translayer_dims[i + 1]
            layers.append(layer_cls(cfg_i, '%s%d' % (name, i)))
        self.translayers = nn.ModuleList(layers)
        self.comb_norm_layers = nn.ModuleList(
            [nn.LayerNorm(d, eps=1e-12, elementwise_affine=False) for d in self.translayer_dims[:-1]])
        self.vfeat_norm_layers = nn.ModuleList(
            [nn.LayerNorm(d, eps=1e-12, elementwise_affine=True) for d in self.translayer_dims[:-1]])
        self.use_attn_consist_loss = config.use_attn_consist_loss
        if self.use_attn_consist_loss:
            if config.use_squeezed_transformer:
                self.attn_scaler = nn.ModuleList([nn.Conv2d(1, 1, 1), nn.Conv2d(config.num_modes, 1, 1)])
            else:
                self.attn_scaler = nn.Conv2d(config.num_modes, 1, 1)
        self.layers_vfeat = []
        self.layers_attn_scores = None

    def forward(self, vfeat, voxels_pos, vmask, orig_feat_shape):
        self.layers_vfeat = []
        self.layers_attn_scores = [] if self.use_attn_consist_loss else None
        B, N, _ = vfeat.shape
        mask = vmask.reshape(B * N).to(torch.float32).contiguous() if vmask is not None else None
        x = vfeat if vfeat.dtype == torch.float32 else vfeat.float()
        if self.training and x.is_cuda:
            ops.advance_seed(x.device)
        per_scale = self.num_scales > 0 and self.pos_code_type in ('bias', 'none')
        for i, layer in enumerate(self.translayers):
            if per_scale:
                grids = mince_grids(orig_feat_shape, self.mince_scales)
                pe = [self.pos_code_layers[s](grids[s], voxels_pos) for s in range(self.num_scales)]
            else:
                pe = self.pos_code_layer(orig_feat_shape, voxels_pos)
            ln = self.vfeat_norm_layers[i]
            p = self.dropout.p if (self.training and i == 0) else 0.0
            feat_pe = pe if self.pos_code_type == 'lsinu' else None
            h = ops.prologue(x, ln.weight, ln.bias, feat_pe, float(self.pos_code_weight), mask, p,
                             ops.new_dropout_seed(x.device) if p > 0 else 0)
            ops.grad_ready(h, layer.parameters())
            if self.num_scales > 0:
                x = layer(h, orig_feat_shape, pos_biases=pe if self.pos_code_type == 'bias' else None)
            else:
                x = layer(h, pos_biases=pe if self.pos_code_type == 'bias' else None)
            self.layers_vfeat.append(x)
            if self.use_attn_consist_loss:
                if self.use_squeezed_transformer:
                    self.layers_attn_scores.append([self.attn_scaler[0](layer.in_ator_trans.attention_scores),
                                                    self.attn_scaler[1](layer.ator_out_trans.attention_scores)])
                else:
                    self.layers_attn_scores.append(self.attn_scaler(layer.attention_scores))
        self.orig_feat_shape = orig_feat_shape
        return x


class SegtranInitWeights(nn.Module):

    def __init__(self, config, *inputs, **kwargs):
        super().__init__()
        self.config = config

    def init_weights(self, module):
        if isinstance(module, (nn.Linear, nn.Embedding)):
            if (np.array(module.weight.shape) < self.config.min_feat_dim).all():
                print("Skip init of Linear weight %s" % (list(module.weight.shape)))
            else:
                module.weight.data.normal_(mean=0.0, std=self.config.base_initializer_range)
        if isinstance(module, nn.Linear) and module.bias is not None:
            module.bias.data.zero_()

    def tie_qk(self, module):
        if isinstance(module, CrossAttFeatTrans) and module.tie_qk_scheme != 'none':
            module.tie_qk()

    def add_identity_bias(self, module):
        if isinstance(module, (CrossAttFeatTrans, ExpandedFeatTrans)):
            module.add_identity_bias()
```

segtran_b200/ops.py:

```python
from __future__ import annotations

import ctypes as C
import math
import os
from typing import Optional

import numpy as np
import torch

from . import _lib as L

_PRECISION = "tf32"


def set_precision(p: str):
    global _PRECISION
    if p not in ("tf32", "tf32x3", "bf16"):
        raise ValueError("unsupported precision %r (this build implements 'tf32', 'tf32x3' and 'bf16')" % (p,))
    _PRECISION = p
    _bf16_cache.clear()


def get_precision() -> str:
    return _PRECISION
# ... 155 lines not shown
def _zeros(shape, device) -> torch.Tensor:
    if isinstance(shape, int):
        shape = (shape,)
    n = 1
    for d in shape:
        n *= int(d)
    st = _arena_state(device)
    off, n_al = st["off"], (n + 63) // 64 * 64
    st["off"] = min(off + n_al, _ARENA_MAX)
    if st["buf"] is not None and off + n_al <= st["buf"].numel():
        return st["buf"][off:off + n].view(tuple(shape))
    return torch.zeros(tuple(shape), device=device, dtype=torch.float32)


def _zeros_like(t: torch.Tensor) -> torch.Tensor:
    return _zeros(tuple(t.shape), t.device)


def _operand(t: torch.Tensor, Z1: int, Z0: int, name: str) -> L.sx_operand:
    R, K = t.shape[-2], t.shape[-1]
    sr, sk = t.stride(-2), t.stride(-1)
    if sk == 1 or K == 1:
        major, ld = L.SX_MAJOR_K, sr
        if R == 1:
            ld = max(K, 4)
    elif sr == 1 or R == 1:
        major, ld = L.SX_MAJOR_MN, sk
    else:
        raise L.SxError("gemm operand %s: neither dim is contiguous (strides %s)" % (name, t.stride()))
    op = L.sx_operand()
    op.ptr = t.data_ptr()
    op.major = major
    op.ld = ld
    op.stride_z0 = t.stride(1) if t.shape[1] > 1 else 0
    op.stride_z1 = t.stride(0) if t.shape[0] > 1 else 0
    return op


def _as4(t: torch.Tensor) -> torch.Tensor:
    while t.dim() < 4:
        t = t.unsqueeze(0)
    if t.dim() != 4:
        raise L.SxError("gemm operands must have <= 4 dims")
    return t


_bf16_cache = {}
_BF16_CACHE_MAX = 96


def _bf16_view(t4: torch.Tensor) -> torch.Tensor:
    st = t4.untyped_storage()
    n_st = st.nbytes() // 4
    if n_st <= 4 * t4.numel() + 1024 and st.data_ptr() % 16 == 0:
        key = ("st", st.data_ptr(), n_st, t4._version)
        hit = _bf16_cache.get(key)
        if hit is None:
            flat = torch.empty(n_st, device=t4.device, dtype=torch.bfloat16)
            L.call("sx_convert", st.data_ptr(), L.SX_F32, n_st, flat.data_ptr(), L.SX_BF16, 0, _stream())
            if len(_bf16_cache) >= _BF16_CACHE_MAX:
                _bf16_cache.pop(next(iter(_bf16_cache)))
            hit = (t4, flat)
            _bf16_cache[key] = hit
        return torch.as_strided(hit[1], t4.size(), t4.stride(), t4.storage_offset())
    key = (t4.data_ptr(), tuple(t4.shape), tuple(t4.stride()), t4._version)
    hit = _bf16_cache.get(key)
    if hit is not None:
        return hit[1]
    dims = sorted(((s_, z_) for s_, z_ in zip(t4.stride(), t4.shape) if z_ > 1), key=lambda x: x[0])
    dense, span = True, 1
    for s_, z_ in dims:
        dense = dense and s_ == span
        span *= z_
    src = t4 if dense else t4.contiguous()
    out = torch.empty_strided(src.size(), src.stride(), device=src.device, dtype=torch.bfloat16)
    L.call("sx_convert", src.data_ptr(), L.SX_F32, src.numel(), out.data_ptr(), L.SX_BF16, 0, _stream())
    if len(_bf16_cache) >= _BF16_CACHE_MAX:
        _bf16_cache.pop(next(iter(_bf16_cache)))
    _bf16_cache[key] = (t4, out)
    return out


_PART_FLOATS = 8 << 20
_part_bufs = {}


def _part_args(device):
    key = (device.index if device.index is not None else torch.cuda.current_device(), torch.cuda.current_stream(device).cuda_stream)
    t = _part_bufs.get(key)
    if t is None:
        t = _part_bufs[key] = torch.empty(_PART_FLOATS, device=device, dtype=torch.float32)
    return t.data_ptr(), t.numel()


def _pick_split_k(M, N, K, Z, bk=32, sms=132, epi=10):
    tiles = ((M + 127) // 128) * ((N + 127) // 128) * Z
    nkb = (K + bk - 1) // bk
    if tiles >= 2 * sms or nkb < 16:
        return 1
    best, best_cost = 1, None
    for sk in range(1, max(1, nkb // 8) + 1):
        rounds = (tiles * sk + sms - 1) // sms
        cost = rounds * ((nkb + sk - 1) // sk + epi * (1 if sk == 1 else 2))
        if best_cost is None or cost < best_cost:
            best, best_cost = sk, cost
    return best


def _gemm_nt_1(a: torch.Tensor, b: torch.Tensor, *, out: Optional[torch.Tensor] = None, alpha: float = 1.0,
               bias: Optional[torch.Tensor] = None, bias_mode: int = L.SX_BIAS_N, gelu: bool = False,
               preact: Optional[torch.Tensor] = None, accumulate: bool = False, split_k: Optional[int] = None,
               amax: Optional[torch.Tensor] = None, drop_p: float = 0.0, seed: int = 0, round_out: bool = True,
               reduce_z1: bool = False, addend: Optional[torch.Tensor] = None,
               gelu_bwd: Optional[torch.Tensor] = None, ct: Optional[torch.Tensor] = None) -> torch.Tensor:
    _req_cuda(a, b, out, bias, preact, amax)
    if a.dtype != torch.float32 or b.dtype != torch.float32:
        raise L.SxError("gemm_nt: fp32 operands expected (precision policy %s)" % _PRECISION)
    a4, b4 = _as4(a), _as4(b)
    M, K = a4.shape[-2:]
    N, K2 = b4.shape[-2:]
    if K != K2:
        raise L.SxError("gemm_nt: K mismatch %d vs %d" % (K, K2))
    Z1 = max(a4.shape[0], b4.shape[0])
    Z0 = max(a4.shape[1], b4.shape[1])
    for t in (a4, b4):
        if t.shape[0] not in (1, Z1) or t.shape[1] not in (1, Z0):
            raise L.SxError("gemm_nt: batch dims do not broadcast")
    oz1 = 1 if reduce_z1 else Z1
    fresh = out is None
    linear_epi = (not gelu) and preact is None and drop_p == 0.0 and amax is None and gelu_bwd is None and ct is None
    if split_k is None:
        split_k = _pick_split_k(M, N, K, Z0 * Z1) if (linear_epi and (fresh or accumulate or reduce_z1)) else 1
    if fresh:
        if accumulate or reduce_z1 or split_k > 1:
            out = _zeros((oz1, Z0, M, N), a.device)
        else:
            out = torch.empty((oz1, Z0, M, N), device=a.device, dtype=torch.float32)
    o4 = _as4(out)
    if o4.shape[-2:] != (M, N) or o4.stride(-1) != 1:
        raise L.SxError("gemm_nt: bad output view %s %s" % (tuple(o4.shape), o4.stride()))
    g = L.sx_gemm_args()
    g.op_dtype = L.SX_OP_TF32
    if _PRECISION == "bf16":
        a4, b4 = _bf16_view(a4), _bf16_view(b4)
        g.op_dtype = L.SX_OP_BF16
    g.M, g.N, g.K, g.Z0, g.Z1 = M, N, K, Z0, Z1
    g.A = _operand(a4, Z1, Z0, "A")
    g.B = _operand(b4, Z1, Z0, "B")
    g.C = o4.data_ptr()
    g.c_dtype = L.SX_F32
    round_after = round_out and _PRECISION == "tf32" and (split_k > 1 or accumulate or reduce_z1)
    g.round_tf32 = 1 if (round_out and _PRECISION == "tf32" and not round_after) else 0
    g.ldc = o4.stride(-2)
    g.c_stride_z0 = o4.stride(1) if o4.shape[1] > 1 else 0
    g.c_stride_z1 = 0 if reduce_z1 else (o4.stride(0) if o4.shape[0] > 1 else 0)
    g.alpha = alpha
    if bias is not None:
        b4b = bias
        while b4b.dim() < 3:
            b4b = b4b.unsqueeze(0)
        g.bias = bias.data_ptr()
        g.bias_mode = bias_mode
        g.bias_stride_z0 = b4b.stride(1) if b4b.shape[1] > 1 else 0
        g.bias_stride_z1 = b4b.stride(0) if b4b.shape[0] > 1 else 0
    g.act = L.SX_ACT_GELU if gelu else L.SX_ACT_NONE
    if gelu_bwd is not None:
        if gelu or preact is not None or tuple(gelu_bwd.shape[-2:]) != (M, N) or gelu_bwd.stride() != out.stride():
            raise L.SxError("gemm_nt: gelu_bwd needs the pre-activation in the output's layout and no other activation")
        g.act = L.SX_ACT_GELU_BWD
        g.preact = gelu_bwd.data_ptr()
    g.split_k = split_k
    if split_k > 1:
        g.part, g.part_floats = _part_args(a.device)
    g.accumulate = 1 if (accumulate or reduce_z1 or split_k > 1) else 0
    if preact is not None:
        g.preact = preact.data_ptr()
    if amax is not None:
        g.amax = amax.data_ptr()
    g.drop_p = drop_p
    g.drop_seed, g.drop_seed_dev = _seed_args(seed)
    if addend is not None:
        if addend.dtype != torch.float32 or tuple(addend.shape[-2:]) != (M, N) or _as4(addend).stride() != o4.stride():
            raise L.SxError("gemm_nt: addend must be an fp32 tensor in the output's layout")
        g.addend = addend.data_ptr()
    tout = None
    if ct is not None:
        t4 = _as4(ct)
        if ct.dtype != torch.float32 or tuple(t4.shape[-2:]) != (N, M) or t4.stride(-1) != 1 or round_after:
            raise L.SxError("gemm_nt: ct must be an fp32 [..., N, M] view with m contiguous, on a single-pass product")
        t = L.sx_gemm_tout()
        t.ct = t4.data_ptr()
        t.ldct = t4.stride(-2)
        t.ct_stride_z0 = t4.stride(1) if t4.shape[1] > 1 else 0
        t.ct_stride_z1 = t4.stride(0) if t4.shape[0] > 1 else 0
        tout = C.byref(t)
    L.call("sx_gemm", C.byref(g), tout, _stream())
    if round_after and fresh:
        L.call("sx_convert", out.data_ptr(), L.SX_F32, out.numel(), out.data_ptr(), L.SX_F32, 1, _stream())
    return out


def gemm_nt(a: torch.Tensor, b: torch.Tensor, *, out: Optional[torch.Tensor] = None, alpha: float = 1.0,
            bias: Optional[torch.Tensor] = None, bias_mode: int = L.SX_BIAS_N, gelu: bool = False,
            preact: Optional[torch.Tensor] = None, accumulate: bool = False, split_k: Optional[int] = None,
            amax: Optional[torch.Tensor] = None, drop_p: float = 0.0, seed: int = 0, round_out: bool = True,
            reduce_z1: bool = False, gelu_bwd: Optional[torch.Tensor] = None,
            addend: Optional[torch.Tensor] = None, tag: str = "big", ct: Optional[torch.Tensor] = None) -> torch.Tensor:
    if not _three_pass(tag):
        return _gemm_nt_1(a, b, out=out, alpha=alpha, bias=bias, bias_mode=bias_mode, gelu=gelu, preact=preact,
                          accumulate=accumulate, split_k=split_k, amax=amax, drop_p=drop_p, seed=seed,
                          round_out=round_out, reduce_z1=reduce_z1, gelu_bwd=gelu_bwd, addend=addend, ct=ct)
    if ct is not None:
        raise L.SxError("gemm_nt: ct needs a single-pass product")
    _req_cuda(a, b)
    return _gemm_nt_1(_split_cat(a, 0), _split_cat(b, 1), out=out, alpha=alpha, bias=bias, bias_mode=bias_mode, gelu=gelu,
                      preact=preact, accumulate=accumulate, split_k=split_k, amax=amax, drop_p=drop_p, seed=seed,
                      round_out=round_out, reduce_z1=reduce_z1, gelu_bwd=gelu_bwd, addend=addend)


def _split_cat(t: torch.Tensor, role: int) -> torch.Tensor:
    t4 = _as4(t)
    Z1, Z0, R, K = t4.shape
    Kp = _pad4(K)
    out = torch.empty((Z1, Z0, R, 3 * Kp), device=t.device, dtype=torch.float32)
    L.call("sx_split_tf32_cat", t4.data_ptr(), Z1, Z0, R, K, t4.stride(0), t4.stride(1), t4.stride(2), t4.stride(3), Kp, role,
           out.data_ptr(), _stream())
    return out


def _pad4(n: int) -> int:
    return (n + 3) // 4 * 4


def _rowpad_empty(shape, device) -> torch.Tensor:
    Lr = shape[-1]
    buf = torch.empty(tuple(shape[:-1]) + (_pad4(Lr),), device=device, dtype=torch.float32)
    return buf[..., :Lr]


def _rows_ok(t: torch.Tensor) -> bool:
    if t.stride(-1) != 1 or t.stride(-2) % 4 != 0 or t.data_ptr() % 16 != 0:
        return False
    exp = t.stride(-2) * t.shape[-2]
    for d in range(t.dim() - 3, -1, -1):
        if t.shape[d] > 1 and t.stride(d) != exp:
            return False
        exp *= t.shape[d]
    return True


def _rowpad(t: torch.Tensor) -> torch.Tensor:
    if _rows_ok(t):
        return t
    o = _rowpad_empty(t.shape, t.device)
    o.copy_(t)
    return o


def round_tf32(x: torch.Tensor) -> torch.Tensor:
    _req_cuda(x)
    if _PRECISION == "tf32":
        r = getattr(x, "_sx_tf32", None)
        if r is not None and getattr(x, "_sx_tf32_version", -1) == x._version and \
                getattr(x, "_sx_tf32_ptr", None) == x.data_ptr():
            return r
    x = x.contiguous()
    if _PRECISION != "tf32":
        return x
    y = torch.empty_like(x)
    L.call("sx_convert", x.data_ptr(), L.SX_F32, x.numel(), y.data_ptr(), L.SX_F32, 1, _stream())
    return y


_KMAJOR_COPIES = os.environ.get("SEGTRAN_KMAJOR_COPIES", "1") != "0"


def set_kmajor_copies(on: bool):
    global _KMAJOR_COPIES
    _KMAJOR_COPIES = bool(on)


def _kmajor_copies(tag: str = "big") -> bool:
    return _KMAJOR_COPIES and _PRECISION == "tf32" and not _three_pass(tag)


def _transposed(x: torch.Tensor, Z: int, R: int, Cd: int) -> torch.Tensor:
    x = x.contiguous()
    y = _rowpad_empty((Z, Cd, R), x.device)
    L.call("sx_transpose", x.data_ptr(), Z, R, Cd, y.stride(1), y.data_ptr(), _stream())
    return y


def _token_kmajor(M: int, N: int, K: int, Z: int, tag: str = "big") -> bool:
    return _kmajor_copies(tag) and min(M, N) >= 512 and K >= 1024 and \
        2 * ((M + 127) // 128) * ((N + 255) // 256) * Z > 132


def _weight_t(Wr: torch.Tensor, Z: int, O: int, I: int) -> torch.Tensor:
    if _kmajor_copies():
        return _transposed(Wr, Z, O, I)
    return Wr.reshape(Z, O, I).transpose(-1, -2)


def colsum(x2d: torch.Tensor, out: Optional[torch.Tensor] = None) -> torch.Tensor:
    if out is None:
        out = _zeros((x2d.shape[1],), x2d.device)
    L.call("sx_colsum_batched", x2d.data_ptr(), 1, 0, 1, 0, x2d.shape[0], x2d.shape[1], x2d.stride(0), out.data_ptr(),
           *_part_args(x2d.device), _stream())
    return out


class _Linear(torch.autograd.Function):

    @staticmethod
    def forward(ctx, x, W, b, gelu, drop_p, seed, tag, round_y, addend):
        shp = x.shape
        x2 = x.reshape(-1, shp[-1])
        if not x2.is_contiguous():
            x2 = x2.contiguous()
        Wr = W.contiguous() if _three_pass(tag) else round_tf32(W)
        O = W.shape[0]
        y = torch.empty((x2.shape[0], O), device=x.device, dtype=torch.float32)
        h = torch.empty_like(y) if gelu else None
        a2 = None
        if addend is not None:
            a2 = addend.reshape(-1, O)
            if not a2.is_contiguous():
                a2 = a2.contiguous()
        gemm_nt(x2, Wr.view(O, -1), out=y, bias=b, gelu=gelu, preact=h, drop_p=drop_p, seed=seed, tag=tag,
                round_out=round_y, addend=a2)
        ctx.save_for_backward(x2, Wr, h)
        ctx.meta = (shp, b is not None, gelu, drop_p, seed, tag, None if addend is None else addend.shape)
        ctx.leaves = (W, b)
        return y.view(*shp[:-1], O)

    @staticmethod
    def backward(ctx, dy):
        x2, Wr, h = ctx.saved_tensors
        shp, has_b, gelu, drop_p, seed, tag, add_shape = ctx.meta
        W, b = ctx.leaves
        if _three_pass(tag) and _PRECISION == "tf32":
            Wr = round_tf32(W)
        O = W.shape[0]
        Wr2 = Wr.view(O, -1)
        dy2 = dy.reshape(-1, dy.shape[-1]).contiguous()
        if gelu or drop_p > 0:
            dh = torch.empty_like(dy2)
            L.call("sx_gelu_bwd", dy2.data_ptr(), _ptr(h), dy2.numel(), drop_p, *_seed_args(seed), dh.data_ptr(), _rt(),
                   _stream())
            dy2 = dh
        dx = dW = db = da = None
        if ctx.needs_input_grad[0]:
            dx = gemm_nt(dy2, _weight_t(Wr2, 1, *Wr2.shape)[0], round_out=False).view(shp)
        if ctx.needs_input_grad[1]:
            dW = _param_grad(W, dy2.t(), x2.t(), (O, -1))
        if has_b and ctx.needs_input_grad[2]:
            tgt = _grad_target(b)
            if tgt is not None:
                colsum(dy2, out=tgt)
            else:
                db = colsum(dy2)
        if add_shape is not None and ctx.needs_input_grad[8]:
            da = dy2.view(add_shape)
        return dx, dW, db, None, None, None, None, None, da


def linear(x, W, b=None, gelu=False, drop_p=0.0, seed=0, tag="big", round_out=True, addend=None):
    return _Linear.apply(x, W, b, gelu, drop_p, seed, tag, round_out, addend)


def _heads_aligned(dh: int, Fd: int) -> bool:
    es = 2 if _PRECISION == "bf16" else 4
    return (dh * es) % 16 == 0 and (Fd * es) % 16 == 0


def _head_rows(x: torch.Tensor, B: int, R: int, M: int, dh: int) -> torch.Tensor:
    v = x.view(B, R, M, dh).permute(0, 2, 1, 3)
    return v if _heads_aligned(dh, M * dh) else _rowpad(v)


def _head_cols(x: torch.Tensor, B: int, R: int, M: int, dh: int, kmajor: bool) -> torch.Tensor:
    if kmajor or not _heads_aligned(dh, M * dh):
        return _transposed(x, B, R, M * dh).unflatten(1, (M, dh))
    return x.view(B, R, M, dh).permute(0, 2, 3, 1)


class _AttnScores(torch.autograd.Function):

    @staticmethod
    def forward(ctx, q, k, M, amax, row_bias, tag, alpha=None):
        Bq, U1, Cq = q.shape
        B, U2 = k.shape[0], k.shape[1]
        d = Cq // M
        scale = 1.0 / math.sqrt(d) if alpha is None else float(alpha)
        qv = _head_rows(q, Bq, U1, M, d)
        kv = _head_rows(k, B, U2, M, d)
        S = _rowpad_empty((B, M, U1, U2), q.device)
        if row_bias is not None and M != 1:
            raise L.SxError("attn_scores: row_bias needs a single mode")
        rb = row_bias.contiguous().view(-1) if row_bias is not None else None
        gemm_nt(qv, kv, out=S, alpha=scale, amax=amax, round_out=False, bias=rb, bias_mode=L.SX_BIAS_M, tag=tag)
        ctx.save_for_backward(q, k)
        ctx.meta = (M, d, scale, row_bias.shape if row_bias is not None else None)
        ctx.tag = tag
        return S

    @staticmethod
    def backward(ctx, dS):
        q, k = ctx.saved_tensors
        M, d, scale, rb_shape = ctx.meta
        Bq, U1, Cq = q.shape
        B, U2 = k.shape[0], k.shape[1]
        dS = _rowpad(dS)
        dq, dk = _score_grads(dS, q, k, M, scale, ctx.needs_input_grad[0], ctx.needs_input_grad[1], ctx.tag)
        drb = None
        if rb_shape is not None and ctx.needs_input_grad[4]:
            drb = _zeros((U1,), q.device)
            L.call("sx_rowsum", dS.data_ptr(), B * U1, U2, dS.stride(-2), U1, drb.data_ptr(), *_part_args(dS.device), _stream())
            drb = drb.view(rb_shape)
        return dq, dk, None, None, drb, None, None


def _score_grads(dS, q, k, M, scale, need_q, need_k, tag="big", kmajor_k=False):
    Bq, U1, Cq = q.shape
    B, U2 = k.shape[0], k.shape[1]
    d = Cq // M
    dq = dk = None
    if need_q:
        bcast = Bq == 1 and B > 1
        dq = _zeros_like(q) if bcast else torch.empty_like(q)
        gemm_nt(dS, _head_cols(k, B, U2, M, d, kmajor_k), out=dq.view(Bq, U1, M, d).permute(0, 2, 1, 3), alpha=scale,
                round_out=False, reduce_z1=bcast, split_k=1, tag=tag)
    if need_k:
        dk = torch.empty_like(k)
        gemm_nt(dS.transpose(-1, -2), _head_cols(q, Bq, U1, M, d, False), out=dk.view(B, U2, M, d).permute(0, 2, 1, 3),
                alpha=scale, round_out=False, tag=tag)
    return dq, dk


class PosBias:
    __slots__ = ("table", "R", "grid", "w")

    def __init__(self, table, R, grid, w=1.0):
        grid = tuple(int(g) for g in grid)
        if len(grid) not in (2, 3) or table.dim() != len(grid) or any(s != 2 * R + 1 for s in table.shape):
            raise L.SxError("PosBias: table %s does not match radius %d over grid %s" % (tuple(table.shape), R, grid))
        self.table, self.R, self.grid, self.w = table, int(R), grid, float(w)

    def with_weight(self, w):
        return PosBias(self.table, self.R, self.grid, w)

    @property
    def num_tokens(self):
        n = 1
        for g in self.grid:
            n *= g
        return n


def _posbias_desc(table, R, grid, w) -> L.sx_posbias:
    d = L.sx_posbias()
    d.table = table.data_ptr()
    d.pd, d.R = len(grid), R
    for i, g in enumerate(grid):
        d.grid[i] = g
    d.w = w
    return d


def _posbias_table(pb):
    t = pb.table
    if t.dtype != torch.float32 or not t.is_contiguous():
        raise L.SxError("positional-bias table must be contiguous fp32")
    _req_cuda(t)
    return t


def attn_probs_fused(q, k, M, clip=500.0, drop_p=0.0, seed=0, diag=None, need_scores=False, round_out=True, posbias=None,
                     alpha=None):
    _req_cuda(q, k)
    if q.dtype != torch.float32 or k.dtype != torch.float32 or not q.is_contiguous() or not k.is_contiguous():
        raise L.SxError("attn_probs_fused: contiguous fp32 q/k expected")
    Bq, U1, Cq = q.shape
    B, U2, Ck = k.shape
    if Cq != Ck or Cq % M or (Cq // M) % 4 or Bq not in (1, B):
        raise L.SxError("attn_probs_fused: bad shapes q %s k %s modes %d" % (tuple(q.shape), tuple(k.shape), M))
    d = Cq // M
    P = _rowpad_empty((B, M, U1, U2), q.device)
    S = _rowpad_empty((B, M, U1, U2), q.device) if need_scores else None
    lse = torch.empty((B, M, U1), device=q.device, dtype=torch.float32)
    rowmax = torch.empty((B, M, U1), device=q.device, dtype=torch.float32)
    stat = _zeros((3,), q.device)
    a = L.sx_attn_probs_args()
    a.B, a.M, a.U1, a.U2, a.d = B, M, U1, U2, d
    a.round_tf32 = 1 if (round_out and _PRECISION == "tf32") else 0
    a.Q, a.q_ld, a.q_bstride = q.data_ptr(), Cq, (0 if Bq == 1 else U1 * Cq)
    a.K, a.k_ld, a.k_bstride = k.data_ptr(), Ck, U2 * Ck
    a.alpha, a.clip = (1.0 / math.sqrt(d) if alpha is None else float(alpha)), float(clip)
    a.P, a.S, a.ldp = P.data_ptr(), _ptr(S), P.stride(-2)
    a.lse, a.rowmax, a.stat, a.diag = lse.data_ptr(), rowmax.data_ptr(), stat.data_ptr(), _ptr(diag)
    a.drop_p = drop_p
    a.drop_seed, a.drop_seed_dev = _seed_args(seed)
    if posbias is not None:
        a.posbias = _posbias_desc(_posbias_table(posbias), posbias.R, posbias.grid, posbias.w)
    L.call("sx_attn_probs_fwd", C.byref(a), _stream())
    return P, S, lse, rowmax, stat


class _Scale(torch.autograd.Function):

    @staticmethod
    def forward(ctx, x, alpha):
        x = x.contiguous()
        y = torch.empty_like(x)
        L.call("sx_scale", x.data_ptr(), x.numel(), None, alpha, y.data_ptr(), _stream())
        ctx.alpha = alpha
        return y

    @staticmethod
    def backward(ctx, dy):
        return _Scale.apply(dy, ctx.alpha), None


def scale(x, alpha):
    return _Scale.apply(x, float(alpha))


class _Add(torch.autograd.Function):

    @staticmethod
    def forward(ctx, a, b):
        a, b = a.contiguous(), b.contiguous()
        y = torch.empty_like(a)
        L.call("sx_add", a.data_ptr(), b.data_ptr(), a.numel(), y.data_ptr(), _stream())
        return y

    @staticmethod
    def backward(ctx, dy):
        return dy, dy


def add(a, b):
    return _Add.apply(a, b)


class _MatVec(torch.autograd.Function):

    @staticmethod
    def forward(ctx, x, v):
        x = x.contiguous()
        v = v.contiguous()
        R, Cd = x.shape
        y = _sgemm(x, v, R, 1, Cd, (Cd, 1), (1, 1))[0].view(R)
        ctx.save_for_backward(x, v)
        return y

    @staticmethod
    def backward(ctx, dy):
        x, v = ctx.saved_tensors
        R, Cd = x.shape
        dy = dy.contiguous()
        dx = _sgemm(dy, v, R, Cd, 1, (1, 1), (1, 1))[0] if ctx.needs_input_grad[0] else None
        dv = _sgemm(dy, x, 1, Cd, R, (1, 1), (Cd, 1))[0].view(Cd) if ctx.needs_input_grad[1] else None
        return dx, dv


def matvec(x, v):
    return _MatVec.apply(x, v)


def softmax_posbias_backward(dP, ldd, S, lds, lse, R, Lr, amax, clip, drop_p, seed, ldp_fwd, dS, ldo, table, pb_geom,
                             table_needs_grad):
    tgt = _grad_target(table) if table_needs_grad else None
    buf = tgt if tgt is not None else _zeros((table.numel(),), table.device)
    L.call("sx_softmax_posbias_bwd", dP.data_ptr(), ldd, S.data_ptr(), lds, lse.data_ptr(), R, Lr, _ptr(amax), clip, drop_p,
           *_seed_args(seed), ldp_fwd, dS.data_ptr(), ldo, _rt(), C.byref(_posbias_desc(table, *pb_geom)), buf.data_ptr(),
           *_part_args(dS.device), _stream())
    if tgt is not None or not table_needs_grad:
        return None
    return buf.view(table.shape)


def softmax_backward(dP, S, lse, amax, clip, drop_p, seed, ldp, table=None, pb_geom=None, table_needs_grad=False):
    dP = _rowpad(dP)
    Lr = S.shape[-1]
    R = S.numel() // Lr
    dS = _rowpad_empty(S.shape, S.device)
    if table is None:
        L.call("sx_softmax_bwd", dP.data_ptr(), dP.stride(-2), S.data_ptr(), S.stride(-2), lse.data_ptr(), R, Lr,
               _ptr(amax), clip, drop_p, *_seed_args(seed), ldp, dS.data_ptr(), dS.stride(-2), _rt(), _stream())
        return dS, None
    return dS, softmax_posbias_backward(dP, dP.stride(-2), S, S.stride(-2), lse, R, Lr, amax, clip, drop_p, seed, ldp, dS,
                                        dS.stride(-2), table, pb_geom, table_needs_grad)


class _Softmax(torch.autograd.Function):

    @staticmethod
    def forward(ctx, S, amax, clip, drop_p, seed, diag, table, pb_geom):
        S = _rowpad(S)
        Lr, ld = S.shape[-1], S.stride(-2)
        R = S.numel() // Lr
        P = _rowpad_empty(S.shape, S.device)
        lse = torch.empty(R, device=S.device, dtype=torch.float32)
        args = (S.data_ptr(), R, Lr, ld, _ptr(amax), clip, drop_p, *_seed_args(seed), P.data_ptr(), P.stride(-2), _rt(),
                lse.data_ptr(), _ptr(diag))
        if table is None:
            L.call("sx_softmax_fwd", *args, _stream())
        else:
            L.call("sx_softmax_posbias_fwd", *args, C.byref(_posbias_desc(table, *pb_geom)), _stream())
        ctx.save_for_backward(S, lse, amax, table)
        ctx.meta = (clip, drop_p, seed, P.stride(-2), pb_geom)
        ctx.leaf = table
        return P

    @staticmethod
    def backward(ctx, dP):
        S, lse, amax, _table = ctx.saved_tensors
        clip, drop_p, seed, ldp, pb_geom = ctx.meta
        dS, dT = softmax_backward(dP, S, lse, amax, clip, drop_p, seed, ldp, ctx.leaf, pb_geom, ctx.needs_input_grad[6])
        return dS, None, None, None, None, None, dT, None


class _AttnPV(torch.autograd.Function):

    @staticmethod
    def forward(ctx, P, v, M, tag, round_out, heads):
        B, _, U1, U2 = P.shape
        Fd = v.shape[-1] // M
        P = _rowpad(P)
        if heads:
            U = torch.empty((B, U1, M * Fd), device=P.device, dtype=torch.float32)
            gemm_nt(P, _head_cols(v, B, U2, M, Fd, _kmajor_copies(tag)), out=U.view(B, U1, M, Fd).permute(0, 2, 1, 3),
                    tag=tag, round_out=round_out)
        else:
            vv = _head_cols(v, B, U2, M, Fd, _token_kmajor(U1, Fd, U2, B * M, tag))
            U = torch.empty((B, M, U1, Fd), device=P.device, dtype=torch.float32)
            gemm_nt(P, vv, out=U, tag=tag, round_out=round_out)
        ctx.save_for_backward(P, v)
        ctx.meta = (M, Fd, heads)
        ctx.tag = tag
        return U

    @staticmethod
    def backward(ctx, dU):
        P, v = ctx.saved_tensors
        M, Fd, heads = ctx.meta
        B, _, U1, U2 = P.shape
        dU = dU.contiguous()
        dP = dv = None
        if heads:
            if ctx.needs_input_grad[0]:
                dP = _rowpad_empty((B, M, U1, U2), P.device)
                gemm_nt(_head_rows(dU, B, U1, M, Fd), _head_rows(v, B, U2, M, Fd), out=dP, round_out=False, tag=ctx.tag)
            if ctx.needs_input_grad[1]:
                dv = torch.empty_like(v)
                gemm_nt(P.transpose(-1, -2), _head_cols(dU, B, U1, M, Fd, False),
                        out=dv.view(B, U2, M, Fd).permute(0, 2, 1, 3), round_out=False, tag=ctx.tag)
            return dP, dv, None, None, None, None
        dP, dv = _pv_grads(dU, P, v, M, Fd, ctx.needs_input_grad[0], ctx.needs_input_grad[1], ctx.tag)
        return dP, dv, None, None, None, None


def _pv_grads(dU, P, v, M, Fd, need_p, need_v, tag, dUt=None):
    B, _, U1, U2 = P.shape
    dP = dv = None
    if need_p:
        dP = _rowpad_empty((B, M, U1, U2), P.device)
        gemm_nt(dU, v.view(B, U2, M, Fd).permute(0, 2, 1, 3), out=dP, round_out=False, tag=tag)
    if need_v:
        dv = torch.empty_like(v)
        if dUt is None and _token_kmajor(U2, Fd, U1, B * M, tag):
            dUt = _transposed(dU, B * M, U1, Fd).unflatten(0, (B, M))
        if dUt is not None:
            Pt = _transposed(P, B * M, U1, U2).unflatten(0, (B, M))
            gemm_nt(Pt, dUt, out=dv.view(B, U2, M, Fd).permute(0, 2, 1, 3), round_out=False, tag=tag)
            del Pt
        else:
            gemm_nt(P.transpose(-1, -2), dU.transpose(-1, -2), out=dv.view(B, U2, M, Fd).permute(0, 2, 1, 3),
                    round_out=False, tag=tag)
    return dP, dv


class _FoldedValueBank(torch.autograd.Function):

    @staticmethod
    def forward(ctx, a, Wv, Wm, M, tag):
        B, A, Cd = a.shape
        Fd = Wm.shape[0]
        a2 = a.reshape(B * A, Cd)
        if not a2.is_contiguous():
            a2 = a2.contiguous()
        x3 = _three_pass(tag)
        Wvr = (Wv.contiguous() if x3 else round_tf32(Wv)).view(M, 1, Fd, Cd)
        Wmr = Wm.contiguous() if x3 else round_tf32(Wm)
        Wf = gemm_nt(Wmr.view(1, 1, Fd, Fd), Wvr.transpose(-1, -2), tag=tag, round_out=not x3)
        Vp = gemm_nt(a2, Wf.view(M * Fd, Cd), tag=tag)[0, 0]
        if x3 and _PRECISION == "tf32":
            Wf, Wvr, Wmr = round_tf32(Wf), round_tf32(Wv).view(M, 1, Fd, Cd), round_tf32(Wm)
        ctx.save_for_backward(a2, Wf, Wvr, Wmr)
        ctx.meta = (B, A, Cd, Fd, M)
        ctx.leaves = (Wv, Wm)
        return Vp.view(B, A, M * Fd)

    @staticmethod
    def backward(ctx, dVp):
        a2, Wf, Wvr, Wmr = ctx.saved_tensors
        B, A, Cd, Fd, M = ctx.meta
        Wv, Wm = ctx.leaves
        d2 = dVp.reshape(B * A, M * Fd)
        if not d2.is_contiguous():
            d2 = d2.contiguous()
        da = dWv = dWm = None
        if ctx.needs_input_grad[0]:
            da = gemm_nt(d2, _weight_t(Wf, 1, M * Fd, Cd)[0], round_out=False)[0, 0].view(B, A, Cd)
        if ctx.needs_input_grad[1] or ctx.needs_input_grad[2]:
            dWf = gemm_nt(d2.t(), a2.t(), round_out=False).view(M, 1, Fd, Cd)
            if ctx.needs_input_grad[2]:
                dWm = _param_grad(Wm, dWf, Wvr, (1, 1, Fd, Fd), reduce_z1=True)
            if ctx.needs_input_grad[1]:
                dWv = _param_grad(Wv, Wmr.t().view(1, 1, Fd, Fd), dWf.transpose(-1, -2), (M, 1, Fd, Cd))
        return da, dWv, dWm, None, None


def folded_value_bank(a, Wv, Wm, M, tag="small"):
    return _FoldedValueBank.apply(a, Wv, Wm, M, tag)


def _group_linear_fwd(G, Wo, bo):
    M, Fd = G.shape[1], G.shape[3]
    Wr = round_tf32(Wo).reshape(M, Fd, Fd)
    Y = torch.empty_like(G)
    gemm_nt(G, Wr.unsqueeze(0), out=Y, bias=bo.reshape(1, M, Fd), round_out=False)
    return Y, Wr


def _group_linear_param_grads(dY, G, Wo, bo, need_w, need_b, Gt=None):
    B, M, N, Fd = dY.shape
    dW = db = None
    if need_w:
        if Gt is not None:
            dYt = _transposed(dY, B * M, N, Fd).unflatten(0, (B, M))
            dW = _param_grad(Wo, dYt, Gt, (1, M, Fd, Fd), reduce_z1=True)
            del dYt
        else:
            dW = _param_grad(Wo, dY.transpose(-1, -2), G.transpose(-1, -2), (1, M, Fd, Fd), reduce_z1=True)
    if need_b:
        tgt = _grad_target(bo)
        buf = tgt if tgt is not None else _zeros((M * Fd,), dY.device)
        L.call("sx_colsum_batched", dY.data_ptr(), B, M * N * Fd, M, N * Fd, N, Fd, Fd, buf.data_ptr(),
               *_part_args(dY.device), _stream())
        db = None if tgt is not None else buf
    return dW, db


class _AttnPVGeluGroupLinear(torch.autograd.Function):

    @staticmethod
    def forward(ctx, P, v, M, bm, drop_p, seed, Wo, bo):
        B, _, U1, U2 = P.shape
        Fd = v.shape[-1] // M
        P = _rowpad(P)
        G = torch.empty((B, M, U1, Fd), device=P.device, dtype=torch.float32)
        H = torch.empty_like(G)
        kt = _token_kmajor(Fd, Fd, U1, M) and _token_kmajor(U2, Fd, U1, B * M)
        Gt = _rowpad_empty((B, M, Fd, U1), P.device) if kt else None
        gemm_nt(P, _head_cols(v, B, U2, M, Fd, _kmajor_copies()), out=G, bias=bm, gelu=True, preact=H, drop_p=drop_p,
                seed=seed, ct=Gt)
        Y, Wr = _group_linear_fwd(G, Wo, bo)
        ctx.save_for_backward(P, v, H, Gt if kt else G, Wr)
        ctx.meta = (M, Fd, drop_p, seed, kt)
        ctx.leaves = (bm, Wo, bo)
        return Y

    @staticmethod
    def backward(ctx, dY):
        P, v, H, G, Wr = ctx.saved_tensors
        M, Fd, drop_p, seed, kt = ctx.meta
        bm, Wo, bo = ctx.leaves
        dY = dY.contiguous()
        dbm_buf = dbm = None
        if bm is not None and ctx.needs_input_grad[3]:
            tgt = _grad_target(bm)
            dbm_buf = tgt if tgt is not None else _zeros((Fd,), dY.device)
            dbm = None if tgt is not None else dbm_buf
        dH = torch.empty_like(H)
        B, _, U1, _ = P.shape
        dHt = _rowpad_empty((B, M, Fd, U1), dY.device) if kt and ctx.needs_input_grad[1] else None
        gemm_nt(dY, _weight_t(Wr, M, Fd, Fd).unsqueeze(0), out=dH, gelu_bwd=H, drop_p=drop_p, seed=seed, ct=dHt)
        if dbm_buf is not None:
            colsum(dH.view(-1, Fd), out=dbm_buf)
        dW, dbo = _group_linear_param_grads(dY, None if kt else G, Wo, bo, ctx.needs_input_grad[6],
                                            ctx.needs_input_grad[7], Gt=G if kt else None)
        dP, dv = _pv_grads(dH, P, v, M, Fd, ctx.needs_input_grad[0], ctx.needs_input_grad[1], "big", dUt=dHt)
        return dP, dv, None, dbm, None, None, dW, dbo


def attn_pv_gelu_group_linear(P, v, M, bm, drop_p, seed, Wo, bo):
    return _AttnPVGeluGroupLinear.apply(P, v, M, bm, drop_p, seed, Wo, bo)


_ATTN_FUSION = True


def set_attn_fusion(on: bool):
    global _ATTN_FUSION
    _ATTN_FUSION = bool(on)


def attn_fusion_enabled() -> bool:
    return _ATTN_FUSION and _PRECISION == "tf32"


def _pb_args(posbias):
    if posbias is None:
        return None, None
    return _posbias_table(posbias), (posbias.R, posbias.grid, posbias.w)


class _LayerNorm(torch.autograd.Function):

    @staticmethod
    def forward(ctx, x, g, b, rnd, rnd_bwd):
        ctx.rnd_bwd = rnd_bwd
        x = x.contiguous()
        Cd = x.shape[-1]
        R = x.numel() // Cd
        y = torch.empty_like(x)
        stats = torch.empty((R, 2), device=x.device, dtype=torch.float32)
        L.call("sx_layernorm_fwd", x.data_ptr(), R, Cd, g.data_ptr(), b.data_ptr(), y.data_ptr(), rnd,
               stats.data_ptr(), _stream())
        ctx.save_for_backward(x, g, stats)
        ctx.leaves = (g, b)
        return y

    @staticmethod
    def backward(ctx, dy):
        x, g, stats = ctx.saved_tensors
        dy = dy.contiguous()
        Cd = x.shape[-1]
        R = x.numel() // Cd
        dx = torch.empty_like(x)
        dgb, dg = _sink_or_zeros(ctx.leaves[0])
        dbb, db = _sink_or_zeros(ctx.leaves[1])
        L.call("sx_layernorm_bwd", dy.data_ptr(), x.data_ptr(), R, Cd, g.data_ptr(), stats.data_ptr(), dx.data_ptr(),
               ctx.rnd_bwd, dgb.data_ptr(), dbb.data_ptr(), *_part_args(dy.device), _stream())
        return dx, dg, db, None, None


class _GroupLinear(torch.autograd.Function):

    @staticmethod
    def forward(ctx, G, Wo, bo):
        Y, Wr = _group_linear_fwd(G, Wo, bo)
        ctx.save_for_backward(G, Wr)
        ctx.leaves = (Wo, bo)
        return Y

    @staticmethod
    def backward(ctx, dY):
        G, Wr = ctx.saved_tensors
        B, M, N, Fd = G.shape
        dY = dY.contiguous()
        dG = None
        if ctx.needs_input_grad[0]:
            dG = gemm_nt(dY, _weight_t(Wr, M, Fd, Fd).unsqueeze(0), round_out=False)
        dW, db = _group_linear_param_grads(dY, G, *ctx.leaves, ctx.needs_input_grad[1], ctx.needs_input_grad[2])
        return dG, dW, db


class _LnSoftAggr(torch.autograd.Function):

    @staticmethod
    def forward(ctx, Y, g, b, ws, bs, drop_p, seed):
        Y = Y.contiguous()
        B, M, N, Fd = Y.shape
        out = torch.empty((B, N, Fd), device=Y.device, dtype=torch.float32)
        stats = torch.empty((B, M, N, 2), device=Y.device, dtype=torch.float32)
        wts = torch.empty((B, M, N), device=Y.device, dtype=torch.float32)
        L.call("sx_ln_softaggr_fwd", Y.data_ptr(), B, M, N, Fd, g.data_ptr(), b.data_ptr(), ws.data_ptr(),
               bs.data_ptr(), drop_p, *_seed_args(seed), out.data_ptr(), stats.data_ptr(), wts.data_ptr(), _stream())
        ctx.save_for_backward(Y, g, b, ws, stats, wts)
        ctx.meta = (drop_p, seed, bs.shape, ws.shape)
        ctx.leaves = (g, b, ws, bs)
        return out

    @staticmethod
    def backward(ctx, dout):
        Y, g, b, ws, stats, wts = ctx.saved_tensors
        drop_p, seed, bs_shape, ws_shape = ctx.meta
        B, M, N, Fd = Y.shape
        dout = dout.contiguous()
        dY = torch.empty_like(Y)
        dgb, dg = _sink_or_zeros(ctx.leaves[0])
        dbb, db = _sink_or_zeros(ctx.leaves[1])
        dwsb, dws = _sink_or_zeros(ctx.leaves[2])
        dbsb, dbs = _sink_or_zeros(ctx.leaves[3])
        L.call("sx_ln_softaggr_bwd", dout.data_ptr(), Y.data_ptr(), B, M, N, Fd, g.data_ptr(), b.data_ptr(),
               ws.data_ptr(), drop_p, *_seed_args(seed), stats.data_ptr(), wts.data_ptr(), dY.data_ptr(), _rt(), dgb.data_ptr(),
               dbb.data_ptr(), dwsb.data_ptr(), dbsb.data_ptr(), *_part_args(dout.device), _stream())
        return dY, dg, db, dws, dbs, None, None


class _SoftAggr(torch.autograd.Function):

    @staticmethod
    def forward(ctx, x, ws, bs):
        x = x.contiguous()
        B, M, N, Fd = x.shape
        wsc, bsc = ws.contiguous().view(-1), bs.contiguous().view(-1)
        out = torch.empty((B, N, Fd), device=x.device, dtype=torch.float32)
        wts = torch.empty((B, M, N), device=x.device, dtype=torch.float32)
        L.call("sx_softaggr_fwd", x.data_ptr(), B, M, N, Fd, wsc.data_ptr(), bsc.data_ptr(), out.data_ptr(), wts.data_ptr(),
               _stream())
        ctx.save_for_backward(x, wsc, wts)
        ctx.shapes = (ws.shape, bs.shape)
        return out

    @staticmethod
    def backward(ctx, dout):
        x, wsc, wts = ctx.saved_tensors
        B, M, N, Fd = x.shape
        dout = dout.contiguous()
        dx = torch.empty_like(x)
        dscore = torch.empty((B, M, N), device=x.device, dtype=torch.float32)
        L.call("sx_softaggr_bwd", dout.data_ptr(), x.data_ptr(), B, M, N, Fd, wsc.data_ptr(), wts.data_ptr(), dx.data_ptr(),
               dscore.data_ptr(), _stream())
        R = B * M * N
        dws = _sgemm(dscore, x, 1, Fd, R, (1, 1), (Fd, 1))[0].view(ctx.shapes[0])
        dbs = _zeros((1,), x.device)
        L.call("sx_rowsum", dscore.data_ptr(), 1, R, R, 1, dbs.data_ptr(), *_part_args(dscore.device), _stream())
        return dx, dws, dbs.view(ctx.shapes[1])


def soft_aggregate(x, ws, bs):
    return _SoftAggr.apply(x, ws, bs)


class _PosCode(torch.autograd.Function):

    @staticmethod
    def forward(ctx, pos2d, W, b, normalize):
        pos2d = pos2d.contiguous().float()
        R, pd = pos2d.shape
        C0 = W.shape[0]
        if normalize:
            pmax = torch.empty(1, device=pos2d.device, dtype=torch.float32)
            L.call("sx_reduce_max", pos2d.data_ptr(), pos2d.numel(), pmax.data_ptr(), _stream())
        else:
            pmax = torch.ones(1, device=pos2d.device, dtype=torch.float32)
        pe = torch.empty((R, C0), device=pos2d.device, dtype=torch.float32)
        Wc, bc = W.contiguous(), b.contiguous()
        L.call("sx_pos_lsinu_fwd", pos2d.data_ptr(), pmax.data_ptr(), R, pd, Wc.data_ptr(), bc.data_ptr(), C0,
               pe.data_ptr(), _stream())
        ctx.save_for_backward(pos2d, pmax, Wc, bc)
        ctx.leaves = (W, b)
        return pe

    @staticmethod
    def backward(ctx, dpe):
        pos2d, pmax, W, b = ctx.saved_tensors
        R, pd = pos2d.shape
        C0 = W.shape[0]
        dpe = dpe.contiguous()
        scratch = torch.empty_like(dpe)
        dWb, dW = _sink_or_zeros(ctx.leaves[0], like=W)
        dbb, db = _sink_or_zeros(ctx.leaves[1], like=b)
        L.call("sx_pos_lsinu_bwd", pos2d.data_ptr(), pmax.data_ptr(), R, pd, W.data_ptr(), b.data_ptr(), C0,
               dpe.data_ptr(), scratch.data_ptr(), dWb.data_ptr(), dbb.data_ptr(), *_part_args(pos2d.device), _stream())
        return None, dW, db, None


class _Prologue(torch.autograd.Function):

    @staticmethod
    def forward(ctx, x, g, b, pe, posw, mask, drop_p, seed):
        x = x.contiguous()
        B, N, Cd = x.shape
        if pe is not None:
            pe = pe.contiguous()
        C0 = pe.shape[-1] if pe is not None else 0
        pe_bstride = 0 if pe is None or pe.dim() == 2 else N * C0
        h = torch.empty_like(x)
        stats = torch.empty((B * N, 4), device=x.device, dtype=torch.float32)
        L.call("sx_prologue_fwd", x.data_ptr(), B, N, Cd, g.data_ptr(), b.data_ptr(), _ptr(pe), C0, pe_bstride,
               posw, _ptr(mask), drop_p, *_seed_args(seed), h.data_ptr(), _rt(), stats.data_ptr(), _stream())
        ctx.save_for_backward(x, g, b, pe, mask, stats)
        ctx.meta = (posw, drop_p, seed, pe_bstride)
        ctx.leaves = (g, b)
        return h

    @staticmethod
    def backward(ctx, dh):
        x, g, b, pe, mask, stats = ctx.saved_tensors
        posw, drop_p, seed, pe_bstride = ctx.meta
        B, N, Cd = x.shape
        C0 = pe.shape[-1] if pe is not None else 0
        dh = dh.contiguous()
        dx = torch.empty_like(x)
        dgb, dg = _sink_or_zeros(ctx.leaves[0])
        dbb, db = _sink_or_zeros(ctx.leaves[1])
        dpe = _zeros_like(pe) if pe is not None and ctx.needs_input_grad[3] else None
        scratch = torch.empty_like(x) if pe is not None else None
        L.call("sx_prologue_bwd", dh.data_ptr(), x.data_ptr(), B, N, Cd, g.data_ptr(), b.data_ptr(), _ptr(pe), C0,
               pe_bstride, posw, _ptr(mask), drop_p, *_seed_args(seed), stats.data_ptr(), dx.data_ptr(), dgb.data_ptr(), dbb.data_ptr(),
               _ptr(dpe), _ptr(scratch), *_part_args(dh.device), _stream())
        if pe is None:
            L.launch_count -= 1
        return dx, dg, db, dpe, None, None, None, None


class _Transpose(torch.autograd.Function):

    @staticmethod
    def forward(ctx, x):
        x = x.contiguous()
        Z, R, Cd = x.shape
        y = torch.empty((Z, Cd, R), device=x.device, dtype=torch.float32)
        L.call("sx_transpose", x.data_ptr(), Z, R, Cd, R, y.data_ptr(), _stream())
        return y

    @staticmethod
    def backward(ctx, dy):
        return _Transpose.apply(dy)


class _Dot(torch.autograd.Function):

    @staticmethod
    def forward(ctx, x, w):
        x = x.contiguous()
        out = _zeros((1,), x.device)
        L.call("sx_dot", x.data_ptr(), w.data_ptr(), x.numel(), out.data_ptr(), *_part_args(x.device), _stream())
        ctx.save_for_backward(w)
        ctx.shape = x.shape
        return out

    @staticmethod
    def backward(ctx, g):
        (w,) = ctx.saved_tensors
        dx = torch.empty_like(w)
        g = g.contiguous()
        L.call("sx_scale", w.data_ptr(), w.numel(), g.data_ptr(), 1.0, dx.data_ptr(), _stream())
        return dx.view(ctx.shape), None


def dot(x, w):
    return _Dot.apply(x, w.contiguous())


def attn_scores(q, k, M, amax=None, row_bias=None, tag="big", alpha=None):
    return _AttnScores.apply(q, k, M, amax, row_bias, tag, alpha)


def softmax(S, amax=None, clip=500.0, drop_p=0.0, seed=0, diag=None, posbias=None):
    if posbias is not None and (S.shape[-1] != posbias.num_tokens or S.shape[-2] != posbias.num_tokens):
        raise L.SxError("softmax: scores %s do not match the %s bias grid" % (tuple(S.shape), posbias.grid))
    return _Softmax.apply(S, amax, clip, drop_p, seed, diag, *_pb_args(posbias))


def attn_pv(P, v, M, tag="big", round_out=True, heads=False):
    return _AttnPV.apply(P, v, M, tag, round_out, bool(heads))


def layer_norm(x, g, b, consumer_tag=None, producer_tag=None, round_out=True):
    rnd = (_rt() if consumer_tag is None else rt_for(consumer_tag)) if round_out else 0
    return _LayerNorm.apply(x, g, b, rnd, _rt() if producer_tag is None else rt_for(producer_tag))


def group_linear(G, Wo, bo):
    return _GroupLinear.apply(G, Wo, bo)


def ln_softaggr(Y, g, b, ws, bs, drop_p=0.0, seed=0):
    return _LnSoftAggr.apply(Y, g, b, ws, bs, drop_p, seed)


def pos_code(pos2d, W, b, normalize=True):
    return _PosCode.apply(pos2d, W, b, bool(normalize))


def prologue(x, g, b, pe, posw, mask, drop_p=0.0, seed=0):
    return _Prologue.apply(x, g, b, pe, posw, mask, drop_p, seed)


def transpose(x):
    return _Transpose.apply(x)


def _resize_axis(x: torch.Tensor, axis: int, Lout: int, accumulate_into: Optional[torch.Tensor] = None):
    shp = list(x.shape)
    Lin = shp[axis]
    outer = 1
    for s in shp[:axis]:
        outer *= s
    inner = 1
    for s in shp[axis + 1:]:
        inner *= s
    shp[axis] = Lout
    if accumulate_into is not None:
        y = accumulate_into
        acc = 1
    else:
        y = torch.empty(shp, device=x.device, dtype=torch.float32)
        acc = 0
    L.call("sx_resize_axis_fwd", x.data_ptr(), outer, Lin, Lout, inner, y.data_ptr(), acc, _stream())
    return y


def _resize_axis_adj(dy: torch.Tensor, axis: int, Lin: int):
    shp = list(dy.shape)
    Lout = shp[axis]
    outer = 1
    for s in shp[:axis]:
        outer *= s
    inner = 1
    for s in shp[axis + 1:]:
        inner *= s
    shp[axis] = Lin
    dx = torch.empty(shp, device=dy.device, dtype=torch.float32)
    L.call("sx_resize_axis_bwd", dy.data_ptr(), outer, Lin, Lout, inner, dx.data_ptr(), _stream())
    return dx


class _Resize(torch.autograd.Function):

    @staticmethod
    def forward(ctx, x, size):
        x = x.contiguous()
        nd = len(size)
        ctx.in_sizes = tuple(x.shape[-nd:])
        y = x
        for i, s in enumerate(size):
            ax = x.dim() - nd + i
            if y.shape[ax] != s:
                y = _resize_axis(y, ax, s)
        ctx.size = tuple(size)
        return y

    @staticmethod
    def backward(ctx, dy):
        dy = dy.contiguous()
        nd = len(ctx.size)
        for i in reversed(range(nd)):
            ax = dy.dim() - nd + i
            if ctx.in_sizes[i] != ctx.size[i]:
                dy = _resize_axis_adj(dy, ax, ctx.in_sizes[i])
        return dy, None


def resize_linear(x, size):
    return _Resize.apply(x, tuple(int(s) for s in size))


def _f32(v) -> float:
    return float(np.float32(v))


def down_ratio(scale) -> float:
    return _f32(1.0 / (1.0 / float(scale)))


def size_ratio(lin, lout) -> float:
    return float(np.float32(lin) / np.float32(lout))


def _resample_grid(lin, lout, ratios) -> L.sx_resample_grid:
    if len(lin) not in (1, 2, 3) or len(lout) != len(lin) or len(ratios) != len(lin):
        raise L.SxError("resize_tokens: 1-D to 3-D grids expected (got %s -> %s)" % (tuple(lin), tuple(lout)))
    pad = 3 - len(lin)
    g = L.sx_resample_grid()
    for a in range(3):
        u = a - pad
        g.lin[a], g.lout[a], g.ratio[a] = (int(lin[u]), int(lout[u]), float(ratios[u])) if u >= 0 else (1, 1, 1.0)
    return g


def _cells(grid) -> int:
    n = 1
    for v in grid:
        n *= int(v)
    return n


def _tok_layout(t: torch.Tensor, G: int):
    B, N, C = t.shape
    return (N * C, C // G, C), C // G


def _mode_layout(t: torch.Tensor):
    B, G, N, W = t.shape
    return (G * N * W, N * W, W)


def _resize_fwd(x, xs, y, ys, B, G, w, w_pad, grid, rnd):
    L.call("sx_resize_tokens_fwd", x, *xs, y, *ys, B, G, w, w_pad, C.byref(grid), rnd, _stream())


def _resize_bwd(dy, ys, dx, xs, B, G, w, w_pad, grid, acc):
    L.call("sx_resize_tokens_bwd", dy, *ys, dx, *xs, B, G, w, w_pad, C.byref(grid), acc, _stream())


class _ResizeTokensDown(torch.autograd.Function):

    @staticmethod
    def forward(ctx, x, G, grid, grids_out, ratios, windows, w_pads, round_out):
        _req_cuda(x)
        x = x.contiguous()
        B = x.shape[0]
        xs, D = _tok_layout(x, G)
        outs = []
        for g_out, r, (c0, c1), wp in zip(grids_out, ratios, windows, w_pads):
            y = torch.empty((B, _cells(g_out), G * wp), device=x.device, dtype=torch.float32)
            _resize_fwd(x.data_ptr() + 4 * c0, xs, y.data_ptr(), _tok_layout(y, G)[0], B, G, c1 - c0, wp,
                        _resample_grid(grid, g_out, r), _rt() if round_out else 0)
            outs.append(y)
        ctx.meta = (x.shape, G, tuple(grid), [tuple(g) for g in grids_out], ratios, windows, w_pads)
        return tuple(outs)

    @staticmethod
    def backward(ctx, *dys):
        shape, G, grid, grids_out, ratios, windows, w_pads = ctx.meta
        B, N, Cx = shape
        D = Cx // G
        tiled = sorted(windows)[0][0] == 0 and sorted(windows)[-1][1] == D and \
            all(a[1] == b[0] for a, b in zip(sorted(windows), sorted(windows)[1:]))
        dx = (torch.empty if tiled else torch.zeros)(shape, device=dys[0].device, dtype=torch.float32)
        xs = (N * Cx, D, Cx)
        for dy, g_out, r, (c0, c1), wp in zip(dys, grids_out, ratios, windows, w_pads):
            dy = dy.contiguous()
            _resize_bwd(dy.data_ptr(), _tok_layout(dy, G)[0], dx.data_ptr() + 4 * c0, xs, B, G, c1 - c0, c1 - c0,
                        _resample_grid(grid, g_out, r), 0)
        return dx, None, None, None, None, None, None, None


def resize_tokens(x, G, grid, grids_out, ratios, windows, w_pads=None, round_out=True):
    if w_pads is None:
        w_pads = [((c1 - c0 + 7) // 8 * 8) if _PRECISION == "bf16" else _pad4(c1 - c0) for c0, c1 in windows]
    return _ResizeTokensDown.apply(x, int(G), tuple(int(v) for v in grid), [tuple(int(v) for v in g) for g in grids_out],
                                   [tuple(float(r) for r in rs) for rs in ratios], [(int(a), int(b)) for a, b in windows],
                                   [int(w) for w in w_pads], bool(round_out))


class _ResizeTokensUpInto(torch.autograd.Function):

    @staticmethod
    def forward(ctx, grid, grids_in, ratios, windows, Fd, round_out, *us):
        B, G = us[0].shape[0], us[0].shape[1]
        N = _cells(grid)
        U = torch.empty((B, G, N, Fd), device=us[0].device, dtype=torch.float32)
        Us = _mode_layout(U)
        for u, g_in, r, (c0, c1) in zip(us, grids_in, ratios, windows):
            u = u.contiguous()
            _resize_fwd(u.data_ptr(), _mode_layout(u), U.data_ptr() + 4 * c0, Us, B, G, c1 - c0, c1 - c0,
                        _resample_grid(g_in, grid, r), _rt() if round_out else 0)
        ctx.meta = (tuple(grid), grids_in, ratios, windows, [tuple(u.shape) for u in us])
        return U

    @staticmethod
    def backward(ctx, dU):
        grid, grids_in, ratios, windows, ushapes = ctx.meta
        dU = dU.contiguous()
        B, G = dU.shape[0], dU.shape[1]
        dUs = _mode_layout(dU)
        dus = []
        for g_in, r, (c0, c1), ush in zip(grids_in, ratios, windows, ushapes):
            du = torch.empty(ush, device=dU.device, dtype=torch.float32)
            _resize_bwd(dU.data_ptr() + 4 * c0, dUs, du.data_ptr(), _mode_layout(du), B, G, c1 - c0, ush[-1],
                        _resample_grid(g_in, grid, r), 0)
            dus.append(du)
        return (None, None, None, None, None, None) + tuple(dus)


def resize_tokens_into(us, grid, grids_in, windows, Fd, round_out=True):
    ratios = [tuple(size_ratio(a, b) for a, b in zip(g_in, grid)) for g_in in grids_in]
    return _ResizeTokensUpInto.apply(tuple(int(v) for v in grid), [tuple(int(v) for v in g) for g in grids_in], ratios,
                                     [(int(a), int(b)) for a, b in windows], int(Fd), bool(round_out), *us)


class _AttnProbs(torch.autograd.Function):

    @staticmethod
    def forward(ctx, q, k, M, alpha, clip, drop_p, seed, diag, table, pb_geom, kmajor_dq):
        pb = PosBias(table, *pb_geom) if table is not None else None
        need_bwd = any(ctx.needs_input_grad)
        P, S, lse, _rowmax, stat = attn_probs_fused(q, k, M, clip, drop_p, seed, diag, need_scores=need_bwd, posbias=pb,
                                                    alpha=alpha)
        ctx.save_for_backward(q, k, S, lse, stat)
        ctx.meta = (M, alpha, clip, drop_p, seed, P.stride(-2), pb_geom, kmajor_dq)
        ctx.leaf = table
        return P

    @staticmethod
    def backward(ctx, dP):
        q, k, S, lse, stat = ctx.saved_tensors
        M, alpha, clip, drop_p, seed, ldp, pb_geom, kmajor_dq = ctx.meta
        dS, dT = softmax_backward(dP, S, lse, stat[2:], clip, drop_p, seed, ldp, ctx.leaf, pb_geom, ctx.needs_input_grad[8])
        dq, dk = _score_grads(dS, q, k, M, alpha, ctx.needs_input_grad[0], ctx.needs_input_grad[1],
                              kmajor_k=kmajor_dq and _kmajor_copies())
        return dq, dk, None, None, None, None, None, None, dT, None, None


def attn_probs(q, k, M, alpha=None, clip=500.0, drop_p=0.0, seed=0, diag=None, posbias=None, *, kmajor_dq=False):
    if alpha is None:
        alpha = 1.0 / math.sqrt(q.shape[-1] // M)
    return _AttnProbs.apply(q.contiguous(), k.contiguous(), M, float(alpha), float(clip), drop_p, seed, diag,
                            *_pb_args(posbias), bool(kmajor_dq))


def _sgemm(A, B, M, N, K, sa, sb, out=None, alpha=1.0, accumulate=False, Z=1, zs=(0, 0, 0)):
    if out is None:
        out = torch.empty((Z, M, N), device=A.device, dtype=torch.float32)
    L.call("sx_sgemm_small", A.data_ptr(), B.data_ptr(), out.data_ptr(), M, N, K, sa[0], sa[1], sb[0], sb[1], N, 1, Z,
           zs[0], zs[1], M * N if zs[2] is None else zs[2], alpha, 1 if accumulate else 0, _stream())
    return out


class _HeadContract(torch.autograd.Function):

    @staticmethod
    def forward(ctx, curr, Wb, bb, Wc, bc, tvup):
        curr = curr.contiguous()
        B, Cf = curr.shape[:2]
        V = curr[0, 0].numel()
        K, Fd = Wc.shape
        Wb2 = Wb.reshape(Fd, Cf).contiguous() if Wb is not None else None
        Wc2 = Wc.contiguous()
        if Wb2 is not None:
            Wcb = _sgemm(Wc2, Wb2, K, Cf, Fd, (Fd, 1), (Cf, 1))[0]
            cc = bc.detach().clone().contiguous() if bc is not None else torch.zeros(K, device=curr.device)
            _sgemm(Wc2, bb.contiguous(), K, 1, Fd, (Fd, 1), (1, 1), out=cc.view(1, K, 1), accumulate=True)
        else:
            Wcb = Wc2
            cc = bc.contiguous() if bc is not None else torch.zeros(K, device=curr.device)
        Lo = tvup.contiguous().clone() if tvup is not None else torch.zeros((B, K, V), device=curr.device)
        L.call("sx_head_contract_fwd", curr.data_ptr(), Wcb.data_ptr(), cc.data_ptr(), B, Cf, V, K, Lo.data_ptr(), 1,
               _stream())
        ctx.save_for_backward(curr, Wb2, bb, Wc2, Wcb)
        ctx.meta = (Wb.shape if Wb is not None else None, tvup is not None, bc is not None)
        return Lo.view(B, K, *curr.shape[2:])

    @staticmethod
    def backward(ctx, dL):
        curr, Wb2, bb, Wc2, Wcb = ctx.saved_tensors
        wb_shape, has_tv, has_bc = ctx.meta
        B, Cf = curr.shape[:2]
        V = curr[0, 0].numel()
        K, Fd = Wc2.shape
        dL = dL.contiguous()
        dcurr = dWb = dbb = dWc = dbc = dtv = None
        if ctx.needs_input_grad[0]:
            dcurr = torch.empty_like(curr)
            L.call("sx_head_contract_bwd_data", dL.data_ptr(), Wcb.data_ptr(), B, Cf, V, K, dcurr.data_ptr(), _stream())
        need_w = any(ctx.needs_input_grad[1:5])
        if not need_w:
            return dcurr, None, None, None, None, (dL.view(B, K, V) if has_tv else None)
        if V % 4 == 0:
            dWcb = gemm_nt(dL.view(B, 1, K, V), curr.view(B, 1, Cf, V), reduce_z1=True, round_out=False).view(K, Cf)
        else:
            dWcb = _zeros((K, Cf), curr.device)
            L.call("sx_head_contract_bwd_weight", dL.data_ptr(), curr.data_ptr(), B, Cf, V, K, dWcb.data_ptr(),
                   *_part_args(dL.device), _stream())
        dcc = _zeros((K,), curr.device)
        L.call("sx_rowsum", dL.data_ptr(), B * K, V, V, K, dcc.data_ptr(), *_part_args(dL.device), _stream())
        if Wb2 is not None:
            dWc = gemm_nt(dWcb, Wb2, round_out=False).view(1, K, Fd)
            _sgemm(dcc, bb.contiguous(), K, Fd, 1, (1, 1), (1, 1), out=dWc, accumulate=True)
            dWc = dWc[0]
            dWb = _sgemm(Wc2, dWcb, Fd, Cf, K, (1, Fd), (Cf, 1))[0].reshape(wb_shape)
            dbb = _sgemm(Wc2, dcc, Fd, 1, K, (1, Fd), (1, 1))[0].reshape(Fd)
        else:
            dWc = dWcb
        if has_bc:
            dbc = dcc
        if has_tv:
            dtv = dL.view(B, K, V)
        return dcurr, dWb, dbb, dWc, dbc, dtv


class _TokenClassScores(torch.autograd.Function):

    @staticmethod
    def forward(ctx, vf, Wc):
        vf = vf.contiguous()
        Wc = Wc.contiguous()
        B, N, Fd = vf.shape
        K = Wc.shape[0]
        out = torch.empty((B, K, N), device=vf.device, dtype=torch.float32)
        L.call("sx_token_scores", vf.data_ptr(), Wc.data_ptr(), B, N, Fd, K, out.data_ptr(), _stream())
        ctx.save_for_backward(vf, Wc)
        return out

    @staticmethod
    def backward(ctx, dt):
        vf, Wc = ctx.saved_tensors
        B, N, Fd = vf.shape
        K = Wc.shape[0]
        dt = dt.contiguous()
        if Fd % 4 == 0:
            dvf = torch.empty_like(vf)
            L.call("sx_token_scores_bwd", dt.data_ptr(), Wc.data_ptr(), B, N, Fd, K, dvf.data_ptr(), _stream())
        else:
            dvf = _sgemm(dt, Wc, N, Fd, K, (1, N), (Fd, 1), Z=B, zs=(K * N, 0, N * Fd))
        if N % 4 == 0:
            dWc = gemm_nt(dt.view(B, 1, K, N), vf.transpose(1, 2).unsqueeze(1), reduce_z1=True, round_out=False)
            dWc = dWc.view(K, Fd)
        else:
            dWc = _zeros((1, K, Fd), vf.device)
            for bi in range(B):
                _sgemm(dt[bi], vf[bi], K, Fd, N, (N, 1), (Fd, 1), out=dWc, accumulate=True)
            dWc = dWc[0]
        return dvf, dWc


class _Conv1x1Add(torch.autograd.Function):

    @staticmethod
    def forward(ctx, x, W, b, addend):
        B, Cin, V = x.shape
        Cout = W.shape[0]
        xr = round_tf32(x)
        Wr = round_tf32(W).reshape(Cout, Cin)
        y = torch.empty((B, 1, Cout, V), device=x.device, dtype=torch.float32)
        ad = None if addend is None else addend.contiguous().view(B, 1, Cout, V)
        gemm_nt(Wr.view(1, 1, Cout, Cin), xr.view(B, 1, Cin, V).transpose(-1, -2), out=y, bias=b, bias_mode=L.SX_BIAS_M,
                addend=ad, round_out=False)
        ctx.save_for_backward(xr, Wr)
        ctx.meta = (b is not None, addend is not None)
        ctx.leaves = (W, b)
        return y.view(B, Cout, V)

    @staticmethod
    def backward(ctx, dy):
        xr, Wr = ctx.saved_tensors
        has_b, has_add = ctx.meta
        W, b = ctx.leaves
        B, Cin, V = xr.shape
        Cout = Wr.shape[0]
        dy = dy.contiguous()
        dx = dW = db = None
        if ctx.needs_input_grad[0]:
            dx = gemm_nt(Wr.t().view(1, 1, Cin, Cout), dy.view(B, 1, Cout, V).transpose(-1, -2), round_out=False)
            dx = dx.view(B, Cin, V)
        if ctx.needs_input_grad[1]:
            dW = _param_grad(W, dy.view(B, 1, Cout, V), xr.view(B, 1, Cin, V), (1, 1, Cout, Cin), reduce_z1=True)
        if has_b and ctx.needs_input_grad[2]:
            tgt = _grad_target(b)
            buf = tgt if tgt is not None else _zeros((Cout,), dy.device)
            L.call("sx_rowsum", dy.data_ptr(), B * Cout, V, V, Cout, buf.data_ptr(), *_part_args(dy.device), _stream())
            db = None if tgt is not None else buf
        return dx, dW, db, (dy if has_add else None)


class _GroupNorm(torch.autograd.Function):

    @staticmethod
    def forward(ctx, x, gamma, beta, G, eps, round_out, D):
        x = x.contiguous()
        BD, Cd, V = x.shape
        B = BD // D
        y = torch.empty_like(x)
        csum = torch.empty(BD * Cd * 2, device=x.device, dtype=torch.float64)
        stats = torch.empty(B * G * 2, device=x.device, dtype=torch.float32)
        rt = _rt() if round_out else 0
        if D == 1:
            L.call("sx_groupnorm_fwd", x.data_ptr(), B, Cd, V, G, _ptr(gamma), _ptr(beta), float(eps), csum.data_ptr(),
                   stats.data_ptr(), y.data_ptr(), rt, _stream())
        else:
            L.call("sx_groupnorm_slices_fwd", x.data_ptr(), B, D, Cd, V, G, _ptr(gamma), _ptr(beta), float(eps),
                   csum.data_ptr(), stats.data_ptr(), y.data_ptr(), rt, _stream())
        ctx.save_for_backward(x, gamma, stats)
        ctx.meta = (G, D)
        ctx.leaves = (gamma, beta)
        return y

    @staticmethod
    def backward(ctx, dy):
        x, gamma, stats = ctx.saved_tensors
        G, D = ctx.meta
        BD, Cd, V = x.shape
        B = BD // D
        dy = dy.contiguous()
        dx = torch.empty_like(x)
        csum = torch.empty(BD * Cd * 2, device=x.device, dtype=torch.float64)
        coef = torch.empty(B * G * 2, device=x.device, dtype=torch.float32)
        dg = db = dgb = dbb = None
        if gamma is not None:
            dgb, dg = _sink_or_zeros(ctx.leaves[0])
            dbb, db = _sink_or_zeros(ctx.leaves[1])
        if D == 1:
            L.call("sx_groupnorm_bwd", dy.data_ptr(), x.data_ptr(), B, Cd, V, G, _ptr(gamma), stats.data_ptr(),
                   csum.data_ptr(), coef.data_ptr(), dx.data_ptr(), _ptr(dgb), _ptr(dbb), _stream())
        else:
            L.call("sx_groupnorm_slices_bwd", dy.data_ptr(), x.data_ptr(), B, D, Cd, V, G, _ptr(gamma), stats.data_ptr(),
                   csum.data_ptr(), coef.data_ptr(), dx.data_ptr(), _ptr(dgb), _ptr(dbb), _stream())
        return dx, dg, db, None, None, None, None


def conv1x1_add(x, W, b=None, addend=None):
    sp = x.shape[2:]
    B, Cin = x.shape[:2]
    y = _Conv1x1Add.apply(x.reshape(B, Cin, -1), W, b, None if addend is None else addend.reshape(B, W.shape[0], -1))
    return y.view(B, W.shape[0], *sp)


def group_norm(x, gamma, beta, num_groups, eps=1e-5, round_out=False, slices=1):
    sp = x.shape
    D = int(slices)
    if sp[0] % D:
        raise ValueError("group_norm: batch %d is not a multiple of slices=%d" % (sp[0], D))
    return _GroupNorm.apply(x.reshape(sp[0], sp[1], -1), gamma, beta, int(num_groups), float(eps), round_out, D).view(sp)


_FPN_FUSION = True


def set_fpn_fusion(on: bool):
    global _FPN_FUSION
    _FPN_FUSION = bool(on)


def fpn_fusion_enabled() -> bool:
    return _FPN_FUSION


def conv1x1_ok(x, conv) -> bool:
    V = 1
    for d in x.shape[2:]:
        V *= int(d)
    k = conv.kernel_size
    return x.is_cuda and x.dtype == torch.float32 and all(int(t) == 1 for t in k) and conv.groups == 1 and \
        all(int(t) == 1 for t in conv.stride) and all(int(t) == 0 for t in conv.padding) and \
        V % 4 == 0 and conv.in_channels % 4 == 0


def fpn_stage(cur, higher, conv, norm, scheme="AN", slices=1):
    up_size = tuple(cur.shape[2:])
    hi = higher if tuple(higher.shape[2:]) == up_size else resize_linear(higher, up_size)
    if scheme == 'AN':
        y = conv1x1_add(cur, conv.weight, conv.bias, addend=hi)
        return group_norm(y, norm.weight, norm.bias, norm.num_groups, norm.eps, slices=slices)
    y = conv1x1_add(cur, conv.weight, conv.bias)
    return _Add.apply(group_norm(y, norm.weight, norm.bias, norm.num_groups, norm.eps, slices=slices), hi)


HEAD_MAXK = 8


def _head_out(Lo, out_size):
    if Lo.dim() == 5:
        B, K = Lo.shape[:2]
        H, W, D = out_size
        Lo = resize_linear(Lo, (D, H, W))
        Dd = Lo.shape[2]
        return transpose(Lo.reshape(B * K, Dd, H * W)).view(B, K, H, W, Dd)
    return resize_linear(Lo, tuple(out_size))


def _sgemm_s(A, B, C, M, N, K, sa, sb, sc, Z=1, zs=(0, 0, 0), accumulate=False):
    L.call("sx_sgemm_small", A.data_ptr(), B.data_ptr(), C.data_ptr(), M, N, K, sa[0], sa[1], sb[0], sb[1], sc[0], sc[1],
           Z, zs[0], zs[1], zs[2], 1.0, 1 if accumulate else 0, _stream())
    return C


class _FoldUnfold(torch.autograd.Function):

    @staticmethod
    def forward(ctx, Wc, bc, Wu, bu, Dk):
        K, Fo = Wc.shape
        Fd = Wu.shape[1]
        Wc = Wc.contiguous()
        Wu = Wu.reshape(Fo * Dk, Fd).contiguous()
        bu = bu.contiguous()
        Wf = torch.empty((K, Dk, Fd), device=Wc.device, dtype=torch.float32)
        _sgemm_s(Wc, Wu, Wf, K, Fd, Fo, (Fo, 1), (Dk * Fd, 1), (Dk * Fd, 1), Z=Dk, zs=(0, Fd, Fd))
        bf = bc.detach().reshape(K, 1).expand(K, Dk).contiguous()
        _sgemm_s(Wc, bu, bf, K, Dk, Fo, (Fo, 1), (Dk, 1), (Dk, 1), accumulate=True)
        ctx.save_for_backward(Wc, Wu, bu)
        ctx.Dk = Dk
        return Wf.view(K * Dk, Fd), bf.view(K * Dk)

    @staticmethod
    def backward(ctx, gW, gb):
        Wc, Wu, bu = ctx.saved_tensors
        Dk = ctx.Dk
        K, Fo = Wc.shape
        Fd = Wu.shape[1]
        dev = Wc.device
        gW = torch.zeros((K * Dk, Fd), device=dev) if gW is None else gW.contiguous()
        gb = torch.zeros((K * Dk,), device=dev) if gb is None else gb.contiguous()
        dWc = torch.empty((K, Fo), device=dev, dtype=torch.float32)
        _sgemm_s(gW, Wu, dWc, K, Fo, Dk * Fd, (Dk * Fd, 1), (1, Dk * Fd), (Fo, 1))
        _sgemm_s(gb, bu, dWc, K, Fo, Dk, (Dk, 1), (1, Dk), (Fo, 1), accumulate=True)
        dbc = _zeros((K,), dev)
        L.call("sx_rowsum", gb.data_ptr(), K, Dk, Dk, K, dbc.data_ptr(), *_part_args(dev), _stream())
        dWu = torch.empty((Fo * Dk, Fd), device=dev, dtype=torch.float32)
        _sgemm_s(Wc, gW, dWu, Fo, Fd, K, (1, Fo), (Dk * Fd, 1), (Dk * Fd, 1), Z=Dk, zs=(0, Fd, Fd))
        dbu = torch.empty((Fo * Dk,), device=dev, dtype=torch.float32)
        _sgemm_s(Wc, gb, dbu, Fo, Dk, K, (1, Fo), (Dk, 1), (Dk, 1))
        return dWc, dbc, dWu, dbu, None


def fold_unfold(Wc, bc, Wu, bu, d_pool_k):
    K = Wc.shape[0]
    return _FoldUnfold.apply(Wc.reshape(K, -1), bc, Wu.reshape(Wu.shape[0], -1), bu, int(d_pool_k))


def seg_head(curr, vfeat_fused, grid, Wb, bb, Wc, bc, out_size, d_pool_k=1, permute_dhw_to_hwd=False, d_unfold=1):
    B, N, Fd = vfeat_fused.shape
    K = Wc.shape[0]
# ... 377 lines not shown
```

Baseline: 534.6 million.

## Emit transposed attention probabilities from fused kernel and reuse token transposes in backward

The fused attention-probs kernel can now also write P^T during the forward pass. The PV-GELU backward then uses this copy instead of launching a separate transpose of P. A single token transpose is also computed once for the squeeze path and shared by the linear, score and PV ops, so their backward weight-gradient GEMMs can read K-major operands. The cost is extra strided, uncoalesced scatter writes and extra memory to keep P^T alive, in exchange for removing transpose kernels from the backward pass.

Result: faster. 552.0 million (median of 6 runs) (+3.2%).

```diff
diff --git a/include/segtran_b200.h b/include/segtran_b200.h
--- a/include/segtran_b200.h
+++ b/include/segtran_b200.h
@@ -92,7 +92,12 @@
   const uint64_t* drop_seed_dev;
   sx_posbias posbias;
 } sx_attn_probs_args;
-int sx_attn_probs_fwd(const sx_attn_probs_args* args, void* stream);
+
+typedef struct {
+  float* pt;
+  int64_t ldpt;
+} sx_attn_probs_tout;
+int sx_attn_probs_fwd(const sx_attn_probs_args* args, const sx_attn_probs_tout* tout, void* stream);
 
 enum { SX_CONSIST_BCE = 0, SX_CONSIST_MARGIN = 1 };
 typedef struct {
diff --git a/segtran_b200/_lib.py b/segtran_b200/_lib.py
--- a/segtran_b200/_lib.py
+++ b/segtran_b200/_lib.py
@@ -60,6 +60,10 @@
                 ("_pad", C.c_uint32), ("drop_seed", C.c_uint64), ("drop_seed_dev", C.c_void_p), ("posbias", sx_posbias)]
 
 
+class sx_attn_probs_tout(C.Structure):
+    _fields_ = [("pt", C.c_void_p), ("ldpt", C.c_int64)]
+
+
 class sx_consist_args(C.Structure):
     _fields_ = [("B", C.c_int32), ("N", C.c_int32), ("A", C.c_int32), ("K", C.c_int32), ("variant", C.c_int32),
                 ("round_r", C.c_int32), ("Xo", C.c_void_p), ("xo_ld", C.c_int64), ("xo_bstride", C.c_int64),
@@ -89,7 +93,7 @@
 _PROTOS = {
     "sx_gemm": [C.POINTER(sx_gemm_args), C.POINTER(sx_gemm_tout), _P],
     "sx_gemm_debug_set": [C.c_char_p, _L],
-    "sx_attn_probs_fwd": [C.POINTER(sx_attn_probs_args), _P],
+    "sx_attn_probs_fwd": [C.POINTER(sx_attn_probs_args), C.POINTER(sx_attn_probs_tout), _P],
     "sx_attn_consist_fwd": [C.POINTER(sx_consist_args), _P],
     "sx_attn_consist_bwd": [C.POINTER(sx_consist_args), _P, _P, _I, _I, _L, _L, _P, _P, _P, _L, _L, _P],
     "sx_clamp_if": [_P, _L, _I, _L, _P, _F, _P, _L, _P, _L, _P],
diff --git a/segtran_b200/csrc/sx_attn.cu b/segtran_b200/csrc/sx_attn.cu
--- a/segtran_b200/csrc/sx_attn.cu
+++ b/segtran_b200/csrc/sx_attn.cu
@@ -37,12 +37,14 @@
   int round_tf32;
   const float* pb_table;
   sxpb::Geom pb;
+  float* pt;
+  int ldpt;
 };
 
 constexpr int PB_OFFSET = STAGES * STAGE_BYTES + 256;
 constexpr int PB_MAX_FLOATS = 29 * 29 * 29;
 
-template <bool HAS_BIAS>
+template <bool HAS_BIAS, bool PT>
 __global__ void __launch_bounds__(NUM_THREADS, 1)
 sx_attn_probs_kernel(const __grid_constant__ CUtensorMap tmQ, const __grid_constant__ CUtensorMap tmK, const AttnParams p) {
   extern __shared__ uint8_t smem_raw[];
@@ -280,6 +282,11 @@
           }
           if (col + 1 < p.U2) *reinterpret_cast<float2*>(p.P + roff + col) = make_float2(f0, f1);
           else p.P[roff + col] = f0;
+          if constexpr (PT) {
+            float* pt = p.pt + ((long long)b * p.M + m) * p.U2 * p.ldpt;
+            pt[col * p.ldpt + grow[h]] = f0;
+            if (col + 1 < p.U2) pt[(col + 1) * p.ldpt + grow[h]] = f1;
+          }
         }
       }
     };
@@ -334,9 +341,23 @@
   }
 }
 
-}
-
-extern "C" int sx_attn_probs_fwd(const sx_attn_probs_args* a, void* stream) {
+template <bool HAS_BIAS>
+int launch_probs(const CUtensorMap& tq, const CUtensorMap& tk, const AttnParams& p, int grid, cudaStream_t st) {
+  const int smem = HAS_BIAS ? PB_OFFSET + p.pb.T * 4 + 1024 : SMEM_BYTES;
+  constexpr int smem_max = HAS_BIAS ? PB_OFFSET + PB_MAX_FLOATS * 4 + 1024 : SMEM_BYTES;
+  if (p.pt) {
+    SX_CHECK_CUDA(set_max_smem_once(sx_attn_probs_kernel<HAS_BIAS, true>, smem_max));
+    sx_attn_probs_kernel<HAS_BIAS, true><<<grid, NUM_THREADS, smem, st>>>(tq, tk, p);
+  } else {
+    SX_CHECK_CUDA(set_max_smem_once(sx_attn_probs_kernel<HAS_BIAS, false>, smem_max));
+    sx_attn_probs_kernel<HAS_BIAS, false><<<grid, NUM_THREADS, smem, st>>>(tq, tk, p);
+  }
+  return 0;
+}
+
+}
+
+extern "C" int sx_attn_probs_fwd(const sx_attn_probs_args* a, const sx_attn_probs_tout* tout, void* stream) {
   SX_REQUIRE(a != nullptr, "sx_attn_probs_fwd: null args");
   SX_REQUIRE(a->B > 0 && a->M > 0 && a->U1 > 0 && a->U2 > 0 && a->d > 0, "sx_attn_probs_fwd: bad shape");
   SX_REQUIRE(a->Q && a->K && a->P && a->lse && a->stat, "sx_attn_probs_fwd: null pointer");
@@ -364,6 +385,13 @@
   p.drop_p = a->drop_p; p.drop_seed = a->drop_seed;
   p.drop_seed_dev = reinterpret_cast<const unsigned long long*>(a->drop_seed_dev);
   p.round_tf32 = a->round_tf32;
+  if (tout) {
+    SX_REQUIRE(tout->pt != nullptr, "sx_attn_probs_fwd: null pt");
+    SX_REQUIRE(tout->ldpt >= a->U1 && (long long)a->U2 * tout->ldpt < (1ll << 31),
+               "sx_attn_probs_fwd: ldpt must be at least U1, and U2 * ldpt below 2^31");
+    p.pt = tout->pt;
+    p.ldpt = (int)tout->ldpt;
+  }
   const bool has_bias = a->posbias.table != nullptr;
   if (has_bias) {
     SX_REQUIRE(a->U1 == a->U2, "sx_attn_probs_fwd: positional biases need self-attention (U1 == U2)");
@@ -387,14 +415,8 @@
 
   const int grid = p.items < sms ? p.items : sms;
   cudaStream_t st = reinterpret_cast<cudaStream_t>(stream);
-  if (has_bias) {
-    constexpr int smem_pb = PB_OFFSET + PB_MAX_FLOATS * 4 + 1024;
-    SX_CHECK_CUDA(set_max_smem_once(sx_attn_probs_kernel<true>, smem_pb));
-    sx_attn_probs_kernel<true><<<grid, NUM_THREADS, PB_OFFSET + p.pb.T * 4 + 1024, st>>>(tq, tk, p);
-  } else {
-    SX_CHECK_CUDA(set_max_smem_once(sx_attn_probs_kernel<false>, SMEM_BYTES));
-    sx_attn_probs_kernel<false><<<grid, NUM_THREADS, SMEM_BYTES, st>>>(tq, tk, p);
-  }
+  rc = has_bias ? launch_probs<true>(tq, tk, p, grid, st) : launch_probs<false>(tq, tk, p, grid, st);
+  if (rc) return rc;
   SX_CHECK_CUDA(cudaGetLastError());
   attn_diag_kernel<<<1, 1, 0, st>>>(a->stat, a->clip, a->diag);
   SX_CHECK_CUDA(cudaGetLastError());
diff --git a/segtran_b200/networks/segtran_shared.py b/segtran_b200/networks/segtran_shared.py
--- a/segtran_b200/networks/segtran_shared.py
+++ b/segtran_b200/networks/segtran_shared.py
@@ -290,7 +290,11 @@
         us = [ops.attn_pv(p, vv, M, round_out=False) for p, vv in zip(probs, vs)]
         return ops.resize_tokens_into(us, grid, grids, wins, Fd)
 
-    def forward(self, input_feat, attention_probs, in_geoshape=None):
+    def reads_transposed_probs(self, B, U1, U2):
+        return self.supports_fused_attention() and self.num_scales == 0 and \
+            ops.pv_gelu_kmajor(B, self.num_modes, U1, U2, self.feat_dim)
+
+    def forward(self, input_feat, attention_probs, in_geoshape=None, probs_t=None):
         M = self.num_modes
         if self.num_scales > 0:
             if in_geoshape is None:
@@ -314,7 +318,8 @@
             p = mid.dropout.p if self.training else 0.0
             gl = self.output.group_linear
             y = ops.attn_pv_gelu_group_linear(attention_probs, vp, M, mid.shared_linear.bias, p,
-                                              ops.new_dropout_seed(vp.device) if p > 0 else 0, gl.weight, gl.bias)
+                                              ops.new_dropout_seed(vp.device) if p > 0 else 0, gl.weight, gl.bias,
+                                              probs_t)
         else:
             u = ops.attn_pv(attention_probs, v, M)
             g = self.intermediate(u)
@@ -401,13 +406,16 @@
 
 
 def _attention_probs(q, k, M, clip, drop_p, diag, *, fused, posbias=None, alpha=None, row_bias=None, tag="big",
-                     kmajor_dq=False):
+                     kmajor_dq=False, transposed=False, key_t=None):
     seed = ops.new_dropout_seed(q.device) if drop_p > 0 else 0
     if fused:
-        return ops.attn_probs(q, k, M, alpha, clip, drop_p, seed, diag, posbias, kmajor_dq=kmajor_dq), None, None
+        if transposed and torch.is_grad_enabled():
+            P, Pt = ops.attn_probs(q, k, M, alpha, clip, drop_p, seed, diag, posbias, kmajor_dq=kmajor_dq, transposed=True)
+            return P, None, None, Pt
+        return ops.attn_probs(q, k, M, alpha, clip, drop_p, seed, diag, posbias, kmajor_dq=kmajor_dq), None, None, None
     amax = torch.full((1,), -3.0e38, device=q.device)
-    S = ops.attn_scores(q, k, M, amax, row_bias, tag, alpha)
-    return ops.softmax(S, amax, clip, drop_p, seed, diag, posbias), S, amax
+    S = ops.attn_scores(q, k, M, amax, row_bias, tag, alpha, kt=key_t)
+    return ops.softmax(S, amax, clip, drop_p, seed, diag, posbias), S, amax, None
 
 
 class CrossAttFeatTrans(nn.Module):
@@ -478,7 +486,7 @@
     def clamp_count(self):
         return self._diag_values()[1]
 
-    def forward(self, in_query, in_key=None, pos_biases=None):
+    def forward(self, in_query, in_key=None, pos_biases=None, query_t=None):
         if in_key is None:
             in_key = in_query
         pb = None
@@ -495,7 +503,7 @@
         nq, nk = in_query.shape[1], in_key.shape[1]
         tq = ops.small_tag(nq, nk) if nq < nk else "proj"
         tk = ops.small_tag(nk, nq) if nk < nq else "proj"
-        q = ops.linear(in_query, self.query.weight, self.query.bias, tag=tq)
+        q = ops.linear(in_query, self.query.weight, self.query.bias, tag=tq, xt=query_t)
         k = ops.linear(in_key, self.key.weight, self.key.bias, tag=tk)
         dev = q.device
         if self._diag is None or self._diag.device != dev:
@@ -504,8 +512,10 @@
         diag_call = self.training and (self.call_count + 1) % self.attn_diag_cycles == 0
         fused = ops.attn_fusion_enabled() and not self.keep_attn_scores and not diag_call and q.is_cuda and \
             self.attention_mode_dim % 4 == 0 and self.out_trans.supports_fused_attention()
-        probs, s, amax = _attention_probs(q, k, M, float(self.attn_clip), p, self._diag, fused=fused, posbias=pb,
-                                          kmajor_dq=isinstance(self.out_trans, ExpandedFeatTrans))
+        expanded = isinstance(self.out_trans, ExpandedFeatTrans)
+        transposed = fused and expanded and self.out_trans.reads_transposed_probs(k.shape[0], nq, nk)
+        probs, s, amax, probs_t = _attention_probs(q, k, M, float(self.attn_clip), p, self._diag, fused=fused,
+                                                   posbias=pb, kmajor_dq=expanded, transposed=transposed)
         self.attention_scores = ops.clamp_if(s, amax, float(self.attn_clip)) if self.keep_attn_scores else None
         if self.training:
             self.call_count += 1
@@ -515,6 +525,8 @@
                 mx, cc = self._diag_values()
                 print("max-attn: {:.2f}, avg-attn: {:.2f}, clamp-count: {}".format(mx, avg, cc))
                 self._diag = _new_diag(dev)
+        if probs_t is not None:
+            return self.out_trans(in_key, probs, probs_t=probs_t)
         return self.out_trans(in_key, probs)
 
 
@@ -619,7 +631,7 @@
         fused = ops.attn_fusion_enabled() and not diag_call and q.is_cuda
         probs = []
         for s in range(self.num_scales):
-            P, sc, _ = _attention_probs(qs[s], ks[s], M, float(self.attn_clip), p, self._diag[s], fused=fused,
+            P, sc, _, _ = _attention_probs(qs[s], ks[s], M, float(self.attn_clip), p, self._diag[s], fused=fused,
                                         posbias=pbs[s], alpha=alpha)
             probs.append(P)
             if diag_call:
@@ -653,7 +665,7 @@
         self.attractors = nn.Parameter(torch.randn(1, self.num_attractors, self.in_feat_dim))
         self.attention_scores = None
 
-    def _in_squeeze_reassociated(self, in_feat):
+    def _in_squeeze_reassociated(self, in_feat, ht):
         t = self.in_ator_trans
         C = self.in_feat_dim
         st = ops.small_tag(self.num_attractors, in_feat.shape[1])
@@ -667,12 +679,12 @@
         if t._diag is None or t._diag.device != dev:
             t._diag = _new_diag(dev)
         p = t.att_dropout.p if t.training else 0.0
-        probs, s, amax = _attention_probs(qw, in_feat, 1, float(t.attn_clip), p, t._diag, fused=False, row_bias=rb,
-                                          tag="insq")
+        probs, s, amax, _ = _attention_probs(qw, in_feat, 1, float(t.attn_clip), p, t._diag, fused=False, row_bias=rb,
+                                             tag="insq", key_t=ht)
         t.attention_scores = ops.clamp_if(s, amax, float(t.attn_clip)) if t.keep_attn_scores else None
         if t.training:
             t.call_count += 1
-        u = ops.attn_pv(probs, in_feat, 1, tag="insq", round_out=not x3)
+        u = ops.attn_pv(probs, in_feat, 1, tag="insq", round_out=not x3, vt=ht)
         ot = t.out_trans
         z = ops.linear(u[:, 0], ot.first_linear.weight, tag=st, round_out=False)
         return ops.layer_norm(z, ot.first_norm_layer.weight, ot.first_norm_layer.bias, consumer_tag=st)
@@ -681,13 +693,15 @@
         if pos_biases is not None:
             _unsupported("positional biases with squeezed attention")
         t = self.in_ator_trans
+        ht = None
         if t.num_modes == 1 and not t.out_trans.has_FFN and t.out_trans.first_linear.bias is None \
                 and t.feat_dim == self.in_feat_dim:
-            att = self._in_squeeze_reassociated(in_feat)
+            ht = ops.tokens_t(in_feat, self.num_attractors, "insq")
+            att = self._in_squeeze_reassociated(in_feat, ht)
         else:
             att = t(self.attractors, in_feat)
         ops.grad_ready(att, self.ator_out_trans.parameters())
-        out = self.ator_out_trans(in_feat, att)
+        out = self.ator_out_trans(in_feat, att, query_t=ht)
         self.attention_scores = self.ator_out_trans.attention_scores
         return out
 
diff --git a/segtran_b200/ops.py b/segtran_b200/ops.py
--- a/segtran_b200/ops.py
+++ b/segtran_b200/ops.py
@@ -481,6 +481,19 @@
     return Wr.reshape(Z, O, I).transpose(-1, -2)
 
 
+def tokens_t(x: torch.Tensor, rows: int, tag: str = "big") -> Optional[torch.Tensor]:
+    B, N, C = x.shape
+    if N % 4 or not _token_kmajor(rows, C, N, B, tag):
+        return None
+    with torch.no_grad():
+        return _transposed(x, 1, B * N, C)[0]
+
+
+def tokens_t_heads(xt: torch.Tensor, B: int, M: int) -> torch.Tensor:
+    C = xt.shape[0]
+    return xt.view(M, C // M, B, xt.shape[1] // B).permute(2, 0, 1, 3)
+
+
 def colsum(x2d: torch.Tensor, out: Optional[torch.Tensor] = None) -> torch.Tensor:
     if out is None:
         out = _zeros((x2d.shape[1],), x2d.device)
@@ -492,7 +505,7 @@
 class _Linear(torch.autograd.Function):
 
     @staticmethod
-    def forward(ctx, x, W, b, gelu, drop_p, seed, tag, round_y, addend):
+    def forward(ctx, x, W, b, gelu, drop_p, seed, tag, round_y, addend, xt):
         shp = x.shape
         x2 = x.reshape(-1, shp[-1])
         if not x2.is_contiguous():
@@ -508,15 +521,17 @@
                 a2 = a2.contiguous()
         gemm_nt(x2, Wr.view(O, -1), out=y, bias=b, gelu=gelu, preact=h, drop_p=drop_p, seed=seed, tag=tag,
                 round_out=round_y, addend=a2)
-        ctx.save_for_backward(x2, Wr, h)
-        ctx.meta = (shp, b is not None, gelu, drop_p, seed, tag, None if addend is None else addend.shape)
+        if xt is not None and tuple(xt.shape) != (x2.shape[1], x2.shape[0]):
+            raise L.SxError("linear: xt must be x^T [%d, %d]" % (x2.shape[1], x2.shape[0]))
+        ctx.save_for_backward(x2 if xt is None else xt, Wr, h)
+        ctx.meta = (shp, b is not None, gelu, drop_p, seed, tag, None if addend is None else addend.shape, xt is not None)
         ctx.leaves = (W, b)
         return y.view(*shp[:-1], O)
 
     @staticmethod
     def backward(ctx, dy):
         x2, Wr, h = ctx.saved_tensors
-        shp, has_b, gelu, drop_p, seed, tag, add_shape = ctx.meta
+        shp, has_b, gelu, drop_p, seed, tag, add_shape, transposed = ctx.meta
         W, b = ctx.leaves
         if _three_pass(tag) and _PRECISION == "tf32":
             Wr = round_tf32(W)
@@ -532,7 +547,12 @@
         if ctx.needs_input_grad[0]:
             dx = gemm_nt(dy2, _weight_t(Wr2, 1, *Wr2.shape)[0], round_out=False).view(shp)
         if ctx.needs_input_grad[1]:
-            dW = _param_grad(W, dy2.t(), x2.t(), (O, -1))
+            if transposed:
+                dy2t = _transposed(dy2, 1, dy2.shape[0], O)[0]
+                dW = _param_grad(W, dy2t, x2, (O, -1))
+                del dy2t
+            else:
+                dW = _param_grad(W, dy2.t(), x2.t(), (O, -1))
         if has_b and ctx.needs_input_grad[2]:
             tgt = _grad_target(b)
             if tgt is not None:
@@ -541,11 +561,11 @@
                 db = colsum(dy2)
         if add_shape is not None and ctx.needs_input_grad[8]:
             da = dy2.view(add_shape)
-        return dx, dW, db, None, None, None, None, None, da
-
-
-def linear(x, W, b=None, gelu=False, drop_p=0.0, seed=0, tag="big", round_out=True, addend=None):
-    return _Linear.apply(x, W, b, gelu, drop_p, seed, tag, round_out, addend)
+        return dx, dW, db, None, None, None, None, None, da, None
+
+
+def linear(x, W, b=None, gelu=False, drop_p=0.0, seed=0, tag="big", round_out=True, addend=None, xt=None):
+    return _Linear.apply(x, W, b, gelu, drop_p, seed, tag, round_out, addend, xt)
 
 
 def _heads_aligned(dh: int, Fd: int) -> bool:
@@ -567,7 +587,7 @@
 class _AttnScores(torch.autograd.Function):
 
     @staticmethod
-    def forward(ctx, q, k, M, amax, row_bias, tag, alpha=None):
+    def forward(ctx, q, k, M, amax, row_bias, tag, alpha=None, kt=None):
         Bq, U1, Cq = q.shape
         B, U2 = k.shape[0], k.shape[1]
         d = Cq // M
@@ -579,28 +599,28 @@
             raise L.SxError("attn_scores: row_bias needs a single mode")
         rb = row_bias.contiguous().view(-1) if row_bias is not None else None
         gemm_nt(qv, kv, out=S, alpha=scale, amax=amax, round_out=False, bias=rb, bias_mode=L.SX_BIAS_M, tag=tag)
-        ctx.save_for_backward(q, k)
+        ctx.save_for_backward(q, k, kt)
         ctx.meta = (M, d, scale, row_bias.shape if row_bias is not None else None)
         ctx.tag = tag
         return S
 
     @staticmethod
     def backward(ctx, dS):
-        q, k = ctx.saved_tensors
+        q, k, kt = ctx.saved_tensors
         M, d, scale, rb_shape = ctx.meta
         Bq, U1, Cq = q.shape
         B, U2 = k.shape[0], k.shape[1]
         dS = _rowpad(dS)
-        dq, dk = _score_grads(dS, q, k, M, scale, ctx.needs_input_grad[0], ctx.needs_input_grad[1], ctx.tag)
+        dq, dk = _score_grads(dS, q, k, M, scale, ctx.needs_input_grad[0], ctx.needs_input_grad[1], ctx.tag, kt=kt)
         drb = None
         if rb_shape is not None and ctx.needs_input_grad[4]:
             drb = _zeros((U1,), q.device)
             L.call("sx_rowsum", dS.data_ptr(), B * U1, U2, dS.stride(-2), U1, drb.data_ptr(), *_part_args(dS.device), _stream())
             drb = drb.view(rb_shape)
-        return dq, dk, None, None, drb, None, None
-
-
-def _score_grads(dS, q, k, M, scale, need_q, need_k, tag="big", kmajor_k=False):
+        return dq, dk, None, None, drb, None, None, None
+
+
+def _score_grads(dS, q, k, M, scale, need_q, need_k, tag="big", kmajor_k=False, kt=None):
     Bq, U1, Cq = q.shape
     B, U2 = k.shape[0], k.shape[1]
     d = Cq // M
@@ -608,12 +628,19 @@
     if need_q:
         bcast = Bq == 1 and B > 1
         dq = _zeros_like(q) if bcast else torch.empty_like(q)
-        gemm_nt(dS, _head_cols(k, B, U2, M, d, kmajor_k), out=dq.view(Bq, U1, M, d).permute(0, 2, 1, 3), alpha=scale,
-                round_out=False, reduce_z1=bcast, split_k=1, tag=tag)
+        gemm_nt(dS, _head_cols(k, B, U2, M, d, kmajor_k or _token_kmajor(U1, d, U2, B * M, tag)) if kt is None else
+                tokens_t_heads(kt, B, M), out=dq.view(Bq, U1, M, d).permute(0, 2, 1, 3), alpha=scale, round_out=False,
+                reduce_z1=bcast, split_k=1, tag=tag)
     if need_k:
         dk = torch.empty_like(k)
-        gemm_nt(dS.transpose(-1, -2), _head_cols(q, Bq, U1, M, d, False), out=dk.view(B, U2, M, d).permute(0, 2, 1, 3),
-                alpha=scale, round_out=False, tag=tag)
+        if _token_kmajor(U2, d, U1, B * M, tag):
+            dSt = _transposed(dS, B * M, U1, U2).unflatten(0, (B, M))
+            gemm_nt(dSt, _head_cols(q, Bq, U1, M, d, True), out=dk.view(B, U2, M, d).permute(0, 2, 1, 3), alpha=scale,
+                    round_out=False, tag=tag)
+            del dSt
+        else:
+            gemm_nt(dS.transpose(-1, -2), _head_cols(q, Bq, U1, M, d, False),
+                    out=dk.view(B, U2, M, d).permute(0, 2, 1, 3), alpha=scale, round_out=False, tag=tag)
     return dq, dk
 
 
@@ -656,7 +683,7 @@
 
 
 def attn_probs_fused(q, k, M, clip=500.0, drop_p=0.0, seed=0, diag=None, need_scores=False, round_out=True, posbias=None,
-                     alpha=None):
+                     alpha=None, pt=None):
     _req_cuda(q, k)
     if q.dtype != torch.float32 or k.dtype != torch.float32 or not q.is_contiguous() or not k.is_contiguous():
         raise L.SxError("attn_probs_fused: contiguous fp32 q/k expected")
@@ -682,7 +709,14 @@
     a.drop_seed, a.drop_seed_dev = _seed_args(seed)
     if posbias is not None:
         a.posbias = _posbias_desc(_posbias_table(posbias), posbias.R, posbias.grid, posbias.w)
-    L.call("sx_attn_probs_fwd", C.byref(a), _stream())
+    tout = None
+    if pt is not None:
+        if tuple(pt.shape) != (B, M, U2, U1) or not _rows_ok(pt):
+            raise L.SxError("attn_probs_fused: pt must be a [B,M,U2,U1] view with dense 16-byte-pitched rows")
+        t = L.sx_attn_probs_tout()
+        t.pt, t.ldpt = pt.data_ptr(), pt.stride(-2)
+        tout = C.byref(t)
+    L.call("sx_attn_probs_fwd", C.byref(a), tout, _stream())
     return P, S, lse, rowmax, stat
 
 
@@ -804,7 +838,7 @@
 class _AttnPV(torch.autograd.Function):
 
     @staticmethod
-    def forward(ctx, P, v, M, tag, round_out, heads):
+    def forward(ctx, P, v, M, tag, round_out, heads, vt):
         B, _, U1, U2 = P.shape
         Fd = v.shape[-1] // M
         P = _rowpad(P)
@@ -813,7 +847,10 @@
             gemm_nt(P, _head_cols(v, B, U2, M, Fd, _kmajor_copies(tag)), out=U.view(B, U1, M, Fd).permute(0, 2, 1, 3),
                     tag=tag, round_out=round_out)
         else:
-            vv = _head_cols(v, B, U2, M, Fd, _token_kmajor(U1, Fd, U2, B * M, tag))
+            if vt is not None:
+                vv = tokens_t_heads(vt, B, M)
+            else:
+                vv = _head_cols(v, B, U2, M, Fd, _token_kmajor(U1, Fd, U2, B * M, tag))
             U = torch.empty((B, M, U1, Fd), device=P.device, dtype=torch.float32)
             gemm_nt(P, vv, out=U, tag=tag, round_out=round_out)
         ctx.save_for_backward(P, v)
@@ -836,23 +873,27 @@
                 dv = torch.empty_like(v)
                 gemm_nt(P.transpose(-1, -2), _head_cols(dU, B, U1, M, Fd, False),
                         out=dv.view(B, U2, M, Fd).permute(0, 2, 1, 3), round_out=False, tag=ctx.tag)
-            return dP, dv, None, None, None, None
+            return dP, dv, None, None, None, None, None
         dP, dv = _pv_grads(dU, P, v, M, Fd, ctx.needs_input_grad[0], ctx.needs_input_grad[1], ctx.tag)
-        return dP, dv, None, None, None, None
-
-
-def _pv_grads(dU, P, v, M, Fd, need_p, need_v, tag, dUt=None):
-    B, _, U1, U2 = P.shape
+        return dP, dv, None, None, None, None, None
+
+
+def _pv_grads(dU, P, v, M, Fd, need_p, need_v, tag, dUt=None, Pt=None):
+    if Pt is not None:
+        B, _, U2, U1 = Pt.shape
+    else:
+        B, _, U1, U2 = P.shape
     dP = dv = None
     if need_p:
-        dP = _rowpad_empty((B, M, U1, U2), P.device)
+        dP = _rowpad_empty((B, M, U1, U2), dU.device)
         gemm_nt(dU, v.view(B, U2, M, Fd).permute(0, 2, 1, 3), out=dP, round_out=False, tag=tag)
     if need_v:
         dv = torch.empty_like(v)
         if dUt is None and _token_kmajor(U2, Fd, U1, B * M, tag):
             dUt = _transposed(dU, B * M, U1, Fd).unflatten(0, (B, M))
         if dUt is not None:
-            Pt = _transposed(P, B * M, U1, U2).unflatten(0, (B, M))
+            if Pt is None:
+                Pt = _transposed(P, B * M, U1, U2).unflatten(0, (B, M))
             gemm_nt(Pt, dUt, out=dv.view(B, U2, M, Fd).permute(0, 2, 1, 3), round_out=False, tag=tag)
             del Pt
         else:
@@ -894,11 +935,23 @@
         if ctx.needs_input_grad[0]:
             da = gemm_nt(d2, _weight_t(Wf, 1, M * Fd, Cd)[0], round_out=False)[0, 0].view(B, A, Cd)
         if ctx.needs_input_grad[1] or ctx.needs_input_grad[2]:
-            dWf = gemm_nt(d2.t(), a2.t(), round_out=False).view(M, 1, Fd, Cd)
+            dWft = None
+            if _token_kmajor(M * Fd, Cd, B * A, 1):
+                if ctx.needs_input_grad[1] and _token_kmajor(Fd, Cd, Fd, M):
+                    dWft = _rowpad_empty((Cd, M * Fd), d2.device)
+                dWf = gemm_nt(_transposed(d2, 1, B * A, M * Fd)[0], _transposed(a2, 1, B * A, Cd)[0], round_out=False,
+                              ct=dWft)
+            else:
+                dWf = gemm_nt(d2.t(), a2.t(), round_out=False)
+            dWf = dWf.view(M, 1, Fd, Cd)
             if ctx.needs_input_grad[2]:
                 dWm = _param_grad(Wm, dWf, Wvr, (1, 1, Fd, Fd), reduce_z1=True)
             if ctx.needs_input_grad[1]:
-                dWv = _param_grad(Wv, Wmr.t().view(1, 1, Fd, Fd), dWf.transpose(-1, -2), (M, 1, Fd, Cd))
+                if dWft is not None:
+                    dWv = _param_grad(Wv, _transposed(Wmr, 1, Fd, Fd).view(1, 1, Fd, Fd),
+                                      dWft.view(Cd, M, Fd).permute(1, 0, 2).unsqueeze(1), (M, 1, Fd, Cd))
+                else:
+                    dWv = _param_grad(Wv, Wmr.t().view(1, 1, Fd, Fd), dWf.transpose(-1, -2), (M, 1, Fd, Cd))
         return da, dWv, dWm, None, None
 
 
@@ -936,26 +989,31 @@
 class _AttnPVGeluGroupLinear(torch.autograd.Function):
 
     @staticmethod
-    def forward(ctx, P, v, M, bm, drop_p, seed, Wo, bo):
+    def forward(ctx, P, v, M, bm, drop_p, seed, Wo, bo, Pt):
         B, _, U1, U2 = P.shape
         Fd = v.shape[-1] // M
         P = _rowpad(P)
         G = torch.empty((B, M, U1, Fd), device=P.device, dtype=torch.float32)
         H = torch.empty_like(G)
-        kt = _token_kmajor(Fd, Fd, U1, M) and _token_kmajor(U2, Fd, U1, B * M)
+        kt = pv_gelu_kmajor(B, M, U1, U2, Fd)
+        if Pt is not None and not kt:
+            raise L.SxError("attn_pv_gelu_group_linear: P^T given for a product that reads P MN-major")
         Gt = _rowpad_empty((B, M, Fd, U1), P.device) if kt else None
         gemm_nt(P, _head_cols(v, B, U2, M, Fd, _kmajor_copies()), out=G, bias=bm, gelu=True, preact=H, drop_p=drop_p,
                 seed=seed, ct=Gt)
         Y, Wr = _group_linear_fwd(G, Wo, bo)
-        ctx.save_for_backward(P, v, H, Gt if kt else G, Wr)
-        ctx.meta = (M, Fd, drop_p, seed, kt)
+        ctx.save_for_backward(P if Pt is None else Pt, v, H, Gt if kt else G, Wr)
+        ctx.meta = (M, Fd, drop_p, seed, kt, Pt is not None)
         ctx.leaves = (bm, Wo, bo)
         return Y
 
     @staticmethod
     def backward(ctx, dY):
         P, v, H, G, Wr = ctx.saved_tensors
-        M, Fd, drop_p, seed, kt = ctx.meta
+        M, Fd, drop_p, seed, kt, transposed = ctx.meta
+        Pt = P if transposed else None
+        if transposed:
+            P = None
         bm, Wo, bo = ctx.leaves
         dY = dY.contiguous()
         dbm_buf = dbm = None
@@ -964,19 +1022,23 @@
             dbm_buf = tgt if tgt is not None else _zeros((Fd,), dY.device)
             dbm = None if tgt is not None else dbm_buf
         dH = torch.empty_like(H)
-        B, _, U1, _ = P.shape
+        B, U1 = H.shape[0], H.shape[2]
         dHt = _rowpad_empty((B, M, Fd, U1), dY.device) if kt and ctx.needs_input_grad[1] else None
         gemm_nt(dY, _weight_t(Wr, M, Fd, Fd).unsqueeze(0), out=dH, gelu_bwd=H, drop_p=drop_p, seed=seed, ct=dHt)
         if dbm_buf is not None:
             colsum(dH.view(-1, Fd), out=dbm_buf)
         dW, dbo = _group_linear_param_grads(dY, None if kt else G, Wo, bo, ctx.needs_input_grad[6],
                                             ctx.needs_input_grad[7], Gt=G if kt else None)
-        dP, dv = _pv_grads(dH, P, v, M, Fd, ctx.needs_input_grad[0], ctx.needs_input_grad[1], "big", dUt=dHt)
-        return dP, dv, None, dbm, None, None, dW, dbo
-
-
-def attn_pv_gelu_group_linear(P, v, M, bm, drop_p, seed, Wo, bo):
-    return _AttnPVGeluGroupLinear.apply(P, v, M, bm, drop_p, seed, Wo, bo)
+        dP, dv = _pv_grads(dH, P, v, M, Fd, ctx.needs_input_grad[0], ctx.needs_input_grad[1], "big", dUt=dHt, Pt=Pt)
+        return dP, dv, None, dbm, None, None, dW, dbo, None
+
+
+def pv_gelu_kmajor(B, M, U1, U2, Fd) -> bool:
+    return _token_kmajor(Fd, Fd, U1, M) and _token_kmajor(U2, Fd, U1, B * M)
+
+
+def attn_pv_gelu_group_linear(P, v, M, bm, drop_p, seed, Wo, bo, Pt=None):
+    return _AttnPVGeluGroupLinear.apply(P, v, M, bm, drop_p, seed, Wo, bo, Pt)
 
 
 _ATTN_FUSION = True
@@ -1228,8 +1290,8 @@
     return _Dot.apply(x, w.contiguous())
 
 
-def attn_scores(q, k, M, amax=None, row_bias=None, tag="big", alpha=None):
-    return _AttnScores.apply(q, k, M, amax, row_bias, tag, alpha)
+def attn_scores(q, k, M, amax=None, row_bias=None, tag="big", alpha=None, kt=None):
+    return _AttnScores.apply(q, k, M, amax, row_bias, tag, alpha, kt)
 
 
 def softmax(S, amax=None, clip=500.0, drop_p=0.0, seed=0, diag=None, posbias=None):
@@ -1238,8 +1300,8 @@
     return _Softmax.apply(S, amax, clip, drop_p, seed, diag, *_pb_args(posbias))
 
 
-def attn_pv(P, v, M, tag="big", round_out=True, heads=False):
-    return _AttnPV.apply(P, v, M, tag, round_out, bool(heads))
+def attn_pv(P, v, M, tag="big", round_out=True, heads=False, vt=None):
+    return _AttnPV.apply(P, v, M, tag, round_out, bool(heads), vt)
 
 
 def layer_norm(x, g, b, consumer_tag=None, producer_tag=None, round_out=True):
@@ -1460,31 +1522,36 @@
 class _AttnProbs(torch.autograd.Function):
 
     @staticmethod
-    def forward(ctx, q, k, M, alpha, clip, drop_p, seed, diag, table, pb_geom, kmajor_dq):
+    def forward(ctx, q, k, M, alpha, clip, drop_p, seed, diag, table, pb_geom, kmajor_dq, transposed):
         pb = PosBias(table, *pb_geom) if table is not None else None
         need_bwd = any(ctx.needs_input_grad)
+        Pt = _rowpad_empty((k.shape[0], M, k.shape[1], q.shape[1]), q.device) if transposed else None
         P, S, lse, _rowmax, stat = attn_probs_fused(q, k, M, clip, drop_p, seed, diag, need_scores=need_bwd, posbias=pb,
-                                                    alpha=alpha)
+                                                    alpha=alpha, pt=Pt)
         ctx.save_for_backward(q, k, S, lse, stat)
         ctx.meta = (M, alpha, clip, drop_p, seed, P.stride(-2), pb_geom, kmajor_dq)
         ctx.leaf = table
-        return P
-
-    @staticmethod
-    def backward(ctx, dP):
+        if Pt is None:
+            return P
+        ctx.mark_non_differentiable(Pt)
+        return P, Pt
+
+    @staticmethod
+    def backward(ctx, dP, *_dPt):
         q, k, S, lse, stat = ctx.saved_tensors
         M, alpha, clip, drop_p, seed, ldp, pb_geom, kmajor_dq = ctx.meta
         dS, dT = softmax_backward(dP, S, lse, stat[2:], clip, drop_p, seed, ldp, ctx.leaf, pb_geom, ctx.needs_input_grad[8])
         dq, dk = _score_grads(dS, q, k, M, alpha, ctx.needs_input_grad[0], ctx.needs_input_grad[1],
                               kmajor_k=kmajor_dq and _kmajor_copies())
-        return dq, dk, None, None, None, None, None, None, dT, None, None
-
-
-def attn_probs(q, k, M, alpha=None, clip=500.0, drop_p=0.0, seed=0, diag=None, posbias=None, *, kmajor_dq=False):
+        return dq, dk, None, None, None, None, None, None, dT, None, None, None
+
+
+def attn_probs(q, k, M, alpha=None, clip=500.0, drop_p=0.0, seed=0, diag=None, posbias=None, *, kmajor_dq=False,
+               transposed=False):
     if alpha is None:
         alpha = 1.0 / math.sqrt(q.shape[-1] // M)
     return _AttnProbs.apply(q.contiguous(), k.contiguous(), M, float(alpha), float(clip), drop_p, seed, diag,
-                            *_pb_args(posbias), bool(kmajor_dq))
+                            *_pb_args(posbias), bool(kmajor_dq), bool(transposed))
 
 
 def _sgemm(A, B, M, N, K, sa, sb, out=None, alpha=1.0, accumulate=False, Z=1, zs=(0, 0, 0)):
```
